# stevenrobertson/cuburn

Measured on AMD Instinct MI355X. Metric: Msamples/s into 1920x1080 histogram + DE-filter GB/s vs HBM roofline, higher is better.
Workload: dtype f32; 1 GPU; BASELINE configs[1]: 1920x1080 still, 3 xforms (linear+spherical+swirl), 2^28 samples/frame, filters yuv+bilateral+logscale+colorclip, rgba8 out; walker_waves=4, walker_slots=1024, temporal_samples=1024, samples_per_frame=268435456, accum=binned, fuse=256, nslots=1024, frames_queued_ahead=2, frames_per_gpu=1121, parallelism=frame-sharded x1, RCCL gather of device frames, 4 frames per collective

## Files before the change

### cuburn_amd/_lib.py

```python
import ctypes as C
import os

_HERE = os.path.dirname(os.path.abspath(__file__))
LIB_PATH = os.path.join(_HERE, '_lib', 'libflame_hip.so')
LIB_PATH = os.environ.get('FLAME_HIP_LIB', LIB_PATH)

(FL_OK, FL_E_INVAL, FL_E_NOMEM, FL_E_HIP, FL_E_NODEV, FL_E_UNSUPPORTED) = (0, -1, -2, -3, -4, -5)

FILT = dict(yuv=0, bilateral=1, logscale=2, colorclip=3, smearclip=4, haloclip=5, plainclip=6, logencode=7, de=8)
BUF = dict(front=0, back=1, params=2, palette=3, points=4, seeds=5, atom=6, hot=7, side=8, log=9, dir=10)
ACCUM_ATOMIC, ACCUM_BINNED = 0, 1
FL_OP_CHAOS_CDF = 11
FL_OP_OPACITY = 10
JPEG_HEADER_BYTES = 629
JPEG_SAMPLING = {'444': 0, '420': 1}
JPEG_OPTIMIZE = 1
PNG_HEADER_BYTES = 33
PNG_ADAPTIVE = 1
PNG_FILTERS = {'paeth': 0, 'adaptive': PNG_ADAPTIVE}
APNG_IDAT = 0xffffffff
EXR_PIXELS = {'half': 1, 'float': 2}
GIF_HEADER_BYTES = 779
GIF_DITHER = {'none': 0, 'ordered': 8}
WEBP_PB, WEBP_EB = 4, 6
OUT = dict(rgba8=0, rgba16=1, yuv444p=2, yuv444p10=3, yuv420p10=4, yuv444p12=5)


class fl_dim(C.Structure):
    _fields_ = [(n, C.c_uint32) for n in ('w', 'h', 'aw', 'ah', 'astride')]


_SIGS = {
    'fl_abi_version': (C.c_int, []),
    'fl_last_error': (C.c_char_p, []),
    'fl_calc_dim': (None, [C.c_uint32, C.c_uint32, C.POINTER(fl_dim)]),
    'fl_ctx_create': (C.c_int, [C.c_int, C.c_void_p, C.c_void_p, C.c_uint32, C.c_uint32, C.POINTER(C.c_void_p)]),
    'fl_ctx_destroy': (None, [C.c_void_p]),
    'fl_ctx_sync': (C.c_int, [C.c_void_p]),
    'fl_genome_create': (C.c_int, [C.c_void_p, C.c_void_p, C.c_uint32, C.c_void_p, C.c_uint32, C.c_uint32,
                                   C.POINTER(C.c_void_p)]),
    'fl_genome_destroy': (None, [C.c_void_p]),
    'fl_genome_upload': (C.c_int, [C.c_void_p, C.c_void_p, C.c_void_p, C.c_void_p, C.c_void_p, C.c_void_p, C.c_uint32]),
    'fl_interp': (C.c_int, [C.c_void_p, C.c_void_p, C.c_uint32, C.c_uint32, C.c_float, C.c_float]),
    'fl_iterate': (C.c_int, [C.c_void_p, C.c_void_p, C.c_uint32, C.c_uint32, C.c_double, C.c_uint32, C.c_int,
                             C.POINTER(C.c_uint64)]),
    'fl_filter': (C.c_int, [C.c_void_p, C.c_int, C.c_uint32, C.c_uint32, C.c_void_p, C.c_uint32]),
    'fl_resample': (C.c_int, [C.c_void_p, C.c_uint32, C.c_uint32, C.c_uint32, C.c_void_p, C.c_uint32]),
    'fl_output': (C.c_int, [C.c_void_p, C.c_uint32, C.c_uint32, C.c_int, C.c_void_p, C.c_uint64]),
    'fl_output_bytes': (C.c_size_t, [C.c_uint32, C.c_uint32, C.c_int]),
    'fl_jpeg_bound': (C.c_size_t, [C.c_uint32, C.c_uint32]),
    'fl_jpeg_encode': (C.c_int, [C.c_void_p, C.c_uint32, C.c_uint32, C.c_uint64, C.c_int, C.c_void_p, C.c_uint64, C.c_size_t]),
    'fl_output_jpeg': (C.c_int, [C.c_void_p, C.c_uint32, C.c_uint32, C.c_int, C.c_void_p, C.c_uint64, C.c_size_t]),
    'fl_jpeg_bound_s': (C.c_size_t, [C.c_uint32, C.c_uint32, C.c_int]),
    'fl_jpeg_encode_s': (C.c_int, [C.c_void_p, C.c_uint32, C.c_uint32, C.c_uint64, C.c_int, C.c_int, C.c_void_p, C.c_uint64, C.c_size_t]),
    'fl_output_jpeg_s': (C.c_int, [C.c_void_p, C.c_uint32, C.c_uint32, C.c_int, C.c_int, C.c_void_p, C.c_uint64, C.c_size_t]),
    'fl_jpeg_bound_f': (C.c_size_t, [C.c_uint32, C.c_uint32, C.c_int, C.c_uint]),
    'fl_jpeg_encode_f': (C.c_int, [C.c_void_p, C.c_uint32, C.c_uint32, C.c_uint64, C.c_int, C.c_int, C.c_uint, C.c_void_p, C.c_uint64, C.c_size_t]),
    'fl_output_jpeg_f': (C.c_int, [C.c_void_p, C.c_uint32, C.c_uint32, C.c_int, C.c_int, C.c_uint, C.c_void_p, C.c_uint64, C.c_size_t]),
    'fl_png_bound': (C.c_size_t, [C.c_uint32, C.c_uint32, C.c_int]),
    'fl_png_encode': (C.c_int, [C.c_void_p, C.c_uint32, C.c_uint32, C.c_uint64, C.c_int, C.c_void_p, C.c_uint64, C.c_size_t]),
    'fl_output_png': (C.c_int, [C.c_void_p, C.c_uint32, C.c_uint32, C.c_int, C.c_void_p, C.c_uint64, C.c_size_t]),
    'fl_png_bound_f': (C.c_size_t, [C.c_uint32, C.c_uint32, C.c_int, C.c_int, C.c_uint]),
    'fl_png_encode_f': (C.c_int, [C.c_void_p, C.c_uint32, C.c_uint32, C.c_uint64, C.c_int, C.c_int, C.c_uint, C.c_void_p, C.c_uint64, C.c_size_t]),
    'fl_output_png_f': (C.c_int, [C.c_void_p, C.c_uint32, C.c_uint32, C.c_int, C.c_int, C.c_uint, C.c_void_p, C.c_uint64, C.c_size_t]),
    'fl_apng_chunks': (C.c_uint32, [C.c_uint32, C.c_uint32, C.c_int, C.c_int]),
    'fl_apng_bound': (C.c_size_t, [C.c_uint32, C.c_uint32, C.c_int, C.c_int, C.c_uint]),
    'fl_apng_encode': (C.c_int, [C.c_void_p, C.c_uint32, C.c_uint32, C.c_uint64, C.c_int, C.c_int, C.c_uint, C.c_uint32, C.c_void_p, C.c_uint64, C.c_size_t]),
    'fl_output_apng': (C.c_int, [C.c_void_p, C.c_uint32, C.c_uint32, C.c_int, C.c_int, C.c_uint, C.c_uint32, C.c_void_p, C.c_uint64, C.c_size_t]),
    'fl_tiff_bound': (C.c_size_t, [C.c_uint32, C.c_uint32, C.c_int, C.c_int]),
    'fl_tiff_encode': (C.c_int, [C.c_void_p, C.c_uint32, C.c_uint32, C.c_uint64, C.c_int, C.c_int, C.c_void_p, C.c_uint64, C.c_size_t]),
    'fl_output_tiff': (C.c_int, [C.c_void_p, C.c_uint32, C.c_uint32, C.c_int, C.c_int, C.c_void_p, C.c_uint64, C.c_size_t]),
    'fl_exr_bound': (C.c_size_t, [C.c_uint32, C.c_uint32, C.c_int, C.c_int]),
    'fl_exr_encode': (C.c_int, [C.c_void_p, C.c_uint32, C.c_uint32, C.c_uint64, C.c_uint32, C.c_int, C.c_int, C.c_void_p, C.c_uint64, C.c_size_t]),
    'fl_output_exr': (C.c_int, [C.c_void_p, C.c_uint32, C.c_uint32, C.c_int, C.c_int, C.c_void_p, C.c_uint64, C.c_size_t]),
    'fl_gif_bound': (C.c_size_t, [C.c_uint32, C.c_uint32]),
    'fl_gif_encode': (C.c_int, [C.c_void_p, C.c_uint32, C.c_uint32, C.c_uint64, C.c_int, C.c_int, C.c_void_p, C.c_uint64, C.c_size_t]),
    'fl_output_gif': (C.c_int, [C.c_void_p, C.c_uint32, C.c_uint32, C.c_int, C.c_int, C.c_void_p, C.c_uint64, C.c_size_t]),
    'fl_webp_bound': (C.c_size_t, [C.c_uint32, C.c_uint32, C.c_int]),
    'fl_webp_encode': (C.c_int, [C.c_void_p, C.c_uint32, C.c_uint32, C.c_uint64, C.c_int, C.c_void_p, C.c_uint64, C.c_size_t]),
    'fl_output_webp': (C.c_int, [C.c_void_p, C.c_uint32, C.c_uint32, C.c_int, C.c_void_p, C.c_uint64, C.c_size_t]),
    'fl_sort_u32': (C.c_int, [C.c_void_p, C.c_uint64, C.c_uint64, C.c_uint32, C.c_uint32, C.c_uint32, C.c_int, C.c_void_p]),
    'fl_frame_begin': (C.c_int, [C.c_void_p, C.POINTER(C.c_uint32)]),
    'fl_frame_ms': (C.c_int, [C.c_void_p, C.c_uint32, C.POINTER(C.c_float)]),
    'fl_frame_query': (C.c_int, [C.c_void_p, C.c_uint32]),
    'fl_host_alloc': (C.c_void_p, [C.c_size_t]),
    'fl_host_free': (None, [C.c_void_p]),
    'fl_timings_reset': (C.c_int, [C.c_void_p]),
    'fl_timings': (C.c_int, [C.c_void_p, C.POINTER(C.c_float), C.POINTER(C.c_float), C.POINTER(C.c_float),
                             C.POINTER(C.c_uint32)]),
    'fl_timings_detail': (C.c_int, [C.c_void_p, C.POINTER(C.c_float * 6)]),
    'fl_launch_stats': (C.c_int, [C.c_void_p, C.POINTER(C.c_uint32 * 4)]),
    'fl_measure_copy': (C.c_int, [C.c_int, C.c_size_t, C.c_int, C.POINTER(C.c_float)]),
    'fl_read_buffer': (C.c_int, [C.c_void_p, C.c_void_p, C.c_int, C.c_void_p, C.c_size_t]),
    'fl_write_buffer': (C.c_int, [C.c_void_p, C.c_void_p, C.c_int, C.c_void_p, C.c_size_t]),
    'fl_buffer_ptr': (C.c_int, [C.c_void_p, C.c_void_p, C.c_int, C.POINTER(C.c_void_p), C.POINTER(C.c_size_t)]),
    'fl_buffer_ptr_async': (C.c_int, [C.c_void_p, C.c_void_p, C.c_int, C.POINTER(C.c_void_p), C.POINTER(C.c_size_t)]),
    'fl_stream_dependency': (C.c_int, [C.c_void_p, C.c_void_p, C.c_int]),
    'fl_reserve': (C.c_int, [C.c_void_p, C.c_uint32, C.c_uint32]),
    'fl_debug_iter_launch': (C.c_int, [C.c_void_p, C.c_void_p, C.c_uint32, C.c_uint32, C.c_uint32, C.c_uint32,
                                       C.c_uint32, C.c_int]),
    'fl_debug_flush': (C.c_int, [C.c_void_p, C.c_uint32, C.c_uint32]),
    'fl_debug_clear': (C.c_int, [C.c_void_p, C.c_uint32, C.c_uint32, C.c_int]),
    'fl_debug_clear_hot': (C.c_int, [C.c_void_p, C.c_uint32, C.c_uint32]),
    'fl_debug_accum': (C.c_int, [C.c_void_p, C.c_uint32, C.c_uint32, C.c_void_p, C.c_size_t, C.c_void_p, C.c_size_t,
                                 C.c_uint32, C.c_uint32, C.c_uint32, C.c_uint32, C.c_int]),
    'fl_debug_accum_check': (C.c_int, [C.c_uint32, C.c_uint32, C.c_void_p, C.c_size_t, C.c_void_p, C.c_size_t,
                                       C.c_uint32, C.c_uint32, C.c_uint32, C.c_uint32, C.c_int]),
    'fl_debug_shuffle': (C.c_int, [C.c_void_p, C.c_uint32, C.c_void_p]),
    'fl_debug_counters': (C.c_int, [C.c_void_p, C.c_void_p]),
    'fl_rtc_compile_check': (C.c_int, [C.c_void_p, C.c_uint32, C.c_void_p, C.c_uint32, C.c_int, C.c_int, C.c_int, C.c_char_p, C.c_size_t]),
    'fl_genome_prepare': (C.c_int, [C.c_void_p, C.c_void_p, C.c_uint32, C.c_uint32, C.c_int]),
    'fl_rtc_wait': (C.c_int, [C.c_void_p, C.c_void_p]),
    'fl_rtc_stats': (C.c_int, [C.POINTER(C.c_uint64 * 8)]),
    'fl_debug_rtc_hold': (C.c_int, [C.c_int]),
    'fl_debug_apply_xf': (C.c_int, [C.c_void_p, C.c_void_p, C.c_uint32, C.c_int, C.c_uint32, C.c_void_p, C.c_void_p]),
    'fl_debug_math': (C.c_int, [C.c_void_p, C.c_int, C.c_uint32, C.c_void_p, C.c_void_p, C.c_void_p]),
    'fl_debug_place': (C.c_int, [C.c_void_p, C.c_void_p, C.c_uint32, C.c_uint64, C.c_void_p, C.c_void_p]),
    'fl_debug_de_dir': (C.c_int, [C.c_void_p, C.c_uint32, C.c_uint32, C.c_int, C.c_void_p, C.c_int, C.c_int]),
}
MATH = dict((n, i) for i, n in enumerate(
    'rcp div sqrt exp2 log2 exp log pow sin cos tan atan2 sinh cosh fmod fmod_pi trunca hw_sin hw_cos'.split()))
EXPORTS = sorted(_SIGS)

_lib = None


class FlameError(RuntimeError):
    pass


def load():
    global _lib
    if _lib is not None:
        return _lib
    if not os.path.isfile(LIB_PATH):
        raise FlameError('%s not found: build it with `python __graft_entry__.py` '
                         '(make -C cuburn_amd/csrc); the HIP library is required' % LIB_PATH)
    try:
        import torch
    except Exception:
        pass
    lib = C.CDLL(LIB_PATH, mode=C.RTLD_GLOBAL)
    for name, (res, args) in _SIGS.items():
        fn = getattr(lib, name)
        fn.restype, fn.argtypes = res, args
    if lib.fl_abi_version() != 1:
        raise FlameError('libflame_hip ABI mismatch')
    _lib = lib
    return lib


def check(rc):
    if rc == FL_OK:
        return
    msg = load().fl_last_error().decode('utf-8', 'replace')
    if rc == FL_E_NOMEM:
        raise MemoryError(msg)
    if rc in (FL_E_INVAL, FL_E_UNSUPPORTED):
        raise ValueError(msg)
    raise FlameError(msg)
```

### cuburn_amd/csrc/binned.hip

```cpp
#include "flame_device.h"
#include "kernels.h"
#include <cstdlib>

__device__ __forceinline__ void spill_cell(u64 cur, uint32_t gi, float *__restrict__ out4)
{
    float yf, uf, vf, df;
    unpack_cell(cur, yf, uf, vf, df);
    float *o = out4 + 4 * (size_t)gi;
    __hip_atomic_fetch_add(o + 0, yf * FL_INV255, __ATOMIC_RELAXED, __HIP_MEMORY_SCOPE_AGENT);
    __hip_atomic_fetch_add(o + 1, uf * FL_INV255, __ATOMIC_RELAXED, __HIP_MEMORY_SCOPE_AGENT);
    __hip_atomic_fetch_add(o + 2, vf * FL_INV255, __ATOMIC_RELAXED, __HIP_MEMORY_SCOPE_AGENT);
    __hip_atomic_fetch_add(o + 3, df, __ATOMIC_RELAXED, __HIP_MEMORY_SCOPE_AGENT);
}

__device__ __forceinline__ void hot_group(u64 v, unsigned long long grp, uint32_t gi, float *__restrict__ out4)
{
#pragma unroll
    for (int sh = 1; sh < 64; sh <<= 1) {
        const uint32_t lo = (uint32_t)__shfl_xor((int)(uint32_t)v, sh), hi = (uint32_t)__shfl_xor((int)(uint32_t)(v >> 32), sh);
        v += ((u64)hi << 32) | lo;
    }
    if ((threadIdx.x & 63u) == (uint32_t)__builtin_ctzll(grp)) spill_cell(v, gi, out4);
}

__device__ __forceinline__ void hot_group_sw(u64 v, unsigned long long grp, uint32_t gi, float *__restrict__ out4)
{
#define HOT_XOR(sh) do { const uint32_t lo = (uint32_t)__builtin_amdgcn_ds_swizzle((int)(uint32_t)v, 0x1f | ((sh) << 10)), \
                                         hi = (uint32_t)__builtin_amdgcn_ds_swizzle((int)(uint32_t)(v >> 32), 0x1f | ((sh) << 10)); \
                         v += ((u64)hi << 32) | lo; } while (0)
    HOT_XOR(1); HOT_XOR(2); HOT_XOR(4); HOT_XOR(8); HOT_XOR(16);
#undef HOT_XOR
    {
        const uint32_t lo = (uint32_t)__shfl_xor((int)(uint32_t)v, 32), hi = (uint32_t)__shfl_xor((int)(uint32_t)(v >> 32), 32);
        v += ((u64)hi << 32) | lo;
    }
    if ((threadIdx.x & 63u) == (uint32_t)__builtin_ctzll(grp)) spill_cell(v, gi, out4);
}

__device__ __forceinline__ uint32_t wave_incl_scan_b(uint32_t v, uint32_t) {
    v += (uint32_t)__builtin_amdgcn_update_dpp(0, (int)v, 0x111, 0xf, 0xf, false);
    v += (uint32_t)__builtin_amdgcn_update_dpp(0, (int)v, 0x112, 0xf, 0xf, false);
    v += (uint32_t)__builtin_amdgcn_update_dpp(0, (int)v, 0x114, 0xf, 0xf, false);
    v += (uint32_t)__builtin_amdgcn_update_dpp(0, (int)v, 0x118, 0xf, 0xf, false);
    v += (uint32_t)__builtin_amdgcn_update_dpp(0, (int)v, 0x142, 0xa, 0xf, false);
    v += (uint32_t)__builtin_amdgcn_update_dpp(0, (int)v, 0x143, 0xc, 0xf, false);
    return v;
}

__device__ __forceinline__ void wave_sync() {
    __builtin_amdgcn_fence(__ATOMIC_RELEASE, "wavefront");
    __builtin_amdgcn_wave_barrier();
    __builtin_amdgcn_fence(__ATOMIC_ACQUIRE, "wavefront");
}

__device__ __forceinline__ uint32_t wave_incl_maxscan(uint32_t v) {
    v = max(v, (uint32_t)__builtin_amdgcn_update_dpp(0, (int)v, 0x111, 0xf, 0xf, false));
    v = max(v, (uint32_t)__builtin_amdgcn_update_dpp(0, (int)v, 0x112, 0xf, 0xf, false));
    v = max(v, (uint32_t)__builtin_amdgcn_update_dpp(0, (int)v, 0x114, 0xf, 0xf, false));
    v = max(v, (uint32_t)__builtin_amdgcn_update_dpp(0, (int)v, 0x118, 0xf, 0xf, false));
    v = max(v, (uint32_t)__builtin_amdgcn_update_dpp(0, (int)v, 0x142, 0xa, 0xf, false));
    v = max(v, (uint32_t)__builtin_amdgcn_update_dpp(0, (int)v, 0x143, 0xc, 0xf, false));
    return v;
}

constexpr int ACC_GATHER_AHEAD = 4;
constexpr int ACC_ADD_ILP = 8;
constexpr int ACC_ROWS_MAX = 5;
constexpr int ACC_THREADS = 1024;

template <uint32_t TWL>
__device__ __forceinline__ void add_tile_to_cells(const u64 *tile, u64 *__restrict__ atom, float *__restrict__ out4,
                                                  uint32_t tx, uint32_t ty, uint32_t astride, uint32_t aheight, uint32_t big_thr)
{
    constexpr uint32_t TW = 1u << TWL, CELLS = TW * FL_TILE_H;
    const uint32_t tid = threadIdx.x;
    for (uint32_t i0 = tid; i0 < CELLS; i0 += blockDim.x * ACC_ADD_ILP) {
        u64 old[ACC_ADD_ILP];
        uint32_t big = 0;
#pragma unroll
        for (uint32_t k = 0; k < ACC_ADD_ILP; ++k) {
            const uint32_t i = i0 + k * blockDim.x;
            old[k] = 0ull;
            if (i < CELLS) {
                const u64 v = tile[i];
                const uint32_t px = tx * TW + (i & (TW - 1u)), py = ty * FL_TILE_H + (i >> TWL);
                if (v != 0ull && px < astride && py < aheight) {
                    if ((uint32_t)(v >> 54) >= big_thr) big |= 1u << k;
                    else
                        asm volatile("global_atomic_add_x2 %0, %1, %2, off sc0" : "+v"(old[k]) : "v"(atom + py * astride + px), "v"(v) : "memory");
                }
            }
        }
        static_assert(ACC_ADD_ILP == 8 || ACC_ADD_ILP == 4, "the wait below names every result");
        if constexpr (ACC_ADD_ILP == 8)
            asm volatile("s_waitcnt vmcnt(0)" : "+v"(old[0]), "+v"(old[1]), "+v"(old[2]), "+v"(old[3]), "+v"(old[4]), "+v"(old[5]), "+v"(old[6]), "+v"(old[7]) :: "memory");
        else
            asm volatile("s_waitcnt vmcnt(0)" : "+v"(old[0]), "+v"(old[1]), "+v"(old[2]), "+v"(old[3]) :: "memory");
#pragma unroll
        for (uint32_t k = 0; k < ACC_ADD_ILP; ++k) {
            const bool full = (uint32_t)(old[k] >> 32) >= (256u << 23);
            if (full || ((big >> k) & 1u)) {
                const uint32_t i = i0 + k * blockDim.x;
                const uint32_t gi = (ty * FL_TILE_H + (i >> TWL)) * astride + tx * TW + (i & (TW - 1u));
                if (full) {
                    const u64 cur = __hip_atomic_exchange(atom + gi, 0ull, __ATOMIC_RELAXED, __HIP_MEMORY_SCOPE_AGENT);
                    if ((uint32_t)(cur >> 32) != 0u) spill_cell(cur, gi, out4);
                } else
                    spill_cell(tile[i], gi, out4);
            }
        }
    }
}

template <uint32_t TWL>
__global__ void __launch_bounds__(TWL == 7u ? ACC_THREADS : 1024, TWL == 7u ? 8 : 4) __attribute__((amdgpu_num_sgpr(80)))
k_accum_tiles(const uint32_t *__restrict__ log, const uint32_t *__restrict__ dir,
              const u64 *__restrict__ palette, u64 *__restrict__ atom, float *__restrict__ out4,
              uint32_t tiles_x, uint32_t nparts, uint32_t nbatch_total, uint32_t batch_records,
              uint32_t nslots, uint32_t astride, uint32_t aheight, uint32_t rows_cap, uint32_t big_thr, uint32_t gang, uint32_t nbins)
{
    extern __shared__ __attribute__((aligned(16))) unsigned char smem[];
    constexpr uint32_t TW = 1u << TWL, CELLS = TW * FL_TILE_H;
    constexpr int ILP = TWL == 7u ? 3 : 4;
    static_assert(FL_PAL_W == 256, "the palette column is the record's low byte, the row the mark's");
    u64 *pal = reinterpret_cast<u64 *>(smem);
    uint32_t *mk = reinterpret_cast<uint32_t *>(smem + rows_cap * FL_PAL_W * 8) + (threadIdx.x >> 6) * 64;
    u64 *tile = reinterpret_cast<u64 *>(smem + rows_cap * FL_PAL_W * 8 + blockDim.x * 4);
    const uint32_t tid = threadIdx.x, lane = tid & 63, wv = tid >> 6, nwaves = blockDim.x >> 6;
    uint32_t bin, part;
    if (gang == 0u) { bin = blockIdx.x / nparts; part = blockIdx.x % nparts; }
    else {
        const uint32_t loc = blockIdx.x >> 3, gq = (loc / gang) * 8u + (blockIdx.x & 7u);
        bin = (gq / nparts) * gang + loc % gang; part = gq % nparts;
        if (bin >= nbins) return;
    }
    const uint32_t tx = bin % tiles_x, ty = bin / tiles_x;

    const uint32_t b_lo = (uint32_t)((u64)nbatch_total * part / nparts);
    const uint32_t b_hi = (uint32_t)((u64)nbatch_total * (part + 1) / nparts);
    const uint32_t *drow = dir + (size_t)bin * nbatch_total;
    const uint32_t per_slot = nbatch_total / nslots;
    const uint32_t spr = nslots / FL_PAL_H;
    const float inv_spr = __int_as_float(__builtin_amdgcn_readfirstlane(__float_as_int(1.0f / (float)spr)));
    const float inv_ps = __int_as_float(__builtin_amdgcn_readfirstlane(__float_as_int(1.0f / (float)per_slot)));
    const uint32_t chunk_slots = (rows_cap - 1u) * spr;

    if (b_lo >= b_hi) return;
    for (uint32_t cb = b_lo; cb < b_hi;) {
    const uint32_t cs_lo = cb / per_slot;
    const uint32_t ce = min(b_hi, (cs_lo + chunk_slots) * per_slot);
    const uint32_t row_lo = cs_lo / spr, nrows = min(rows_cap, (uint32_t)FL_PAL_H - row_lo);
    u64 stagev[3];
#pragma unroll
    for (int q = 0; q < 3; ++q) {
        const uint32_t i = tid + q * blockDim.x;
        stagev[q] = i < nrows * FL_PAL_W ? palette[row_lo * FL_PAL_W + i] : 0ull;
    }
    uint32_t e_next = cb + wv * 64 + lane < ce ? drow[cb + wv * 64 + lane] : 0u;
    if (cb == b_lo) {
        for (uint32_t i = tid; i < CELLS; i += blockDim.x) tile[i] = 0ull;
        mk[lane] = 0u;
    }
    __syncthreads();
#pragma unroll
    for (int q = 0; q < 3; ++q) {
        const uint32_t i = tid + q * blockDim.x;
        if (i < nrows * FL_PAL_W) pal[i] = stagev[q];
    }
    __syncthreads();
    for (uint32_t g0v = cb + wv * 64; g0v < ce; g0v += nwaves * 64) {
        const uint32_t g0 = (uint32_t)__builtin_amdgcn_readfirstlane((int)g0v);
        const uint32_t s0 = g0 / per_slot, rem0 = g0 - s0 * per_slot;
        const uint32_t batch = g0 + lane;
        const uint32_t e = e_next;
        e_next = batch + nwaves * 64 < ce ? drow[batch + nwaves * 64] : 0u;
        const uint32_t c = e & 0xffffu, first = e >> 16;
        const uint32_t incl = wave_incl_scan_b(c, lane);
        const uint32_t excl = incl - c;
        const uint32_t total = __shfl(incl, 63);
        const uint32_t rslot_l = s0 + (uint32_t)(((float)(rem0 + lane) + 0.5f) * inv_ps);
        const uint32_t row_l = (uint32_t)(((float)rslot_l + 0.5f) * inv_spr) - row_lo;
        const uint32_t mark_l = ((lane * batch_records + first - excl + 1u) << 8) | (row_l & 255u);
        const unsigned char *gbase = reinterpret_cast<const unsigned char *>(log + (size_t)g0 * batch_records) - 4;
        uint32_t carry = 0;
        static_assert(ILP >= 2 && ILP <= 4, "up to four rows to a word");
        auto fetch = [&](const uint32_t v0, uint32_t (&rec)[ILP], uint32_t &rows) __attribute__((always_inline)) {
            unsigned char *mk8 = reinterpret_cast<unsigned char *>(mk);
            const bool starts = c != 0u && excl - v0 < 64u * ILP;
            if (starts) mk8[excl - v0] = (unsigned char)(lane + 1u);
            wave_sync();
            uint32_t mm[ILP];
#pragma unroll
            for (int k = 0; k < ILP; ++k) mm[k] = mk8[k * 64 + lane];
            wave_sync();
            if (starts) mk8[excl - v0] = 0;
#pragma unroll
            for (int k = 0; k < ILP; ++k) mm[k] = wave_incl_maxscan(mm[k]);
#pragma unroll
            for (int k = 0; k < ILP; ++k) {
                mm[k] = max(mm[k], carry);
                carry = (uint32_t)__builtin_amdgcn_readlane((int)mm[k], 63);
                mm[k] = (uint32_t)__builtin_amdgcn_ds_bpermute((int)((mm[k] - 1u) << 2), (int)mark_l);
            }
#pragma unroll
            for (int k = 0; k < ILP; ++k) {
                const uint32_t lo = v0 + k * 64, v = lo + lane;
                const uint32_t m = mm[k];
                rows = __builtin_amdgcn_perm(m, rows, k == 0 ? 0x03020104u : k == 1 ? 0x03020400u : k == 2 ? 0x03040100u : 0x04020100u);
                const uint32_t voff = v < total ? ((m >> 8) + v) << 2 : 4u;
                asm volatile("global_load_dword %0, %1, %2" : "=v"(rec[k]) : "v"(voff), "s"(gbase) : "memory");
            }
        };
        auto process = [&](const uint32_t v0, uint32_t (&rec)[ILP], const uint32_t rows) __attribute__((always_inline)) {
            bool live[ILP];
            u64 val[ILP];
            auto gather = [&](const int k) __attribute__((always_inline)) {
                val[k] = pal[__builtin_amdgcn_perm(rows, rec[k], 0x0c0c0000u | ((4u + k) << 8))];
            };
#pragma unroll
            for (int k = 0; k < ILP; ++k) {
                live[k] = v0 + k * 64 + lane < total;
                if (k < ACC_GATHER_AHEAD) gather(k);
            }
            {
                const uint32_t o0 = rec[0] >> 8;
                if (__builtin_expect(__popcll(__ballot(live[0] && o0 == (uint32_t)__builtin_amdgcn_readfirstlane((int)o0))) >= 48, 0)) {
#pragma unroll
                    for (int k = ACC_GATHER_AHEAD; k < ILP; ++k) gather(k);
#pragma unroll
                    for (int k = 0; k < ILP; ++k) {
                        const uint32_t off = rec[k] >> 8;
                        const uint32_t off0 = (uint32_t)__builtin_amdgcn_readfirstlane((int)off);
                        const bool mine = live[k] && off == off0;
                        const unsigned long long grp = __ballot(mine);
                        if (__popcll(grp) >= 16) {
                            hot_group(mine ? val[k] : 0ull, grp, (ty * FL_TILE_H + (off0 >> TWL)) * astride + tx * TW + (off0 & (TW - 1u)), out4);
                            live[k] = live[k] && !mine;
                        }
                    }
                }
            }
#pragma unroll
            for (int k = 0; k < ILP; ++k) {
                const uint32_t off = rec[k] >> 8;
                if (k + ACC_GATHER_AHEAD < ILP) gather(k + ACC_GATHER_AHEAD);
                if (!live[k]) continue;
                const u64 old = __hip_atomic_fetch_add(tile + off, val[k], __ATOMIC_RELAXED, __HIP_MEMORY_SCOPE_WORKGROUP);
                if ((uint32_t)(old >> 32) >= (128u << 23)) {
                    const u64 cur = __hip_atomic_exchange(tile + off, 0ull, __ATOMIC_RELAXED, __HIP_MEMORY_SCOPE_WORKGROUP);
                    if ((uint32_t)(cur >> 32) != 0u) {
                        const uint32_t px = tx * TW + (off & (TW - 1u)), py = ty * FL_TILE_H + (off >> TWL);
                        spill_cell(cur, py * astride + px, out4);
                    }
                }
            }
        };
#define ACC_WAIT(n, r) do { if constexpr (ILP == 4) asm volatile("s_waitcnt vmcnt(" #n ")" : "+v"(r[0]), "+v"(r[1]), "+v"(r[ILP - 2]), "+v"(r[ILP - 1]) :: "memory"); \
                            else if constexpr (ILP == 3) asm volatile("s_waitcnt vmcnt(" #n ")" : "+v"(r[0]), "+v"(r[1]), "+v"(r[ILP - 1]) :: "memory"); \
                            else asm volatile("s_waitcnt vmcnt(" #n ")" : "+v"(r[0]), "+v"(r[1]) :: "memory"); } while (0)
#define ACC_WAIT_NEWER(r) do { if constexpr (ILP == 4) ACC_WAIT(4, r); else if constexpr (ILP == 3) ACC_WAIT(3, r); else ACC_WAIT(2, r); } while (0)
        constexpr uint32_t STEP = 64 * ILP;
        uint32_t recA[ILP] = {}, recB[ILP] = {}, rowsA = 0u, rowsB = 0u;
        for (uint32_t v0 = 0; v0 < total; v0 += 2 * STEP) {
            fetch(v0, recA, rowsA);
            if (v0 != 0u) { asm volatile("; acc-guarded-block"); ACC_WAIT_NEWER(recB); process(v0 - STEP, recB, rowsB); }
            if (v0 + STEP < total) { fetch(v0 + STEP, recB, rowsB); ACC_WAIT_NEWER(recA); } else ACC_WAIT(0, recA);
            process(v0, recA, rowsA);
        }
        if (((total + STEP - 1u) / STEP & 1u) == 0u && total != 0u) {
            ACC_WAIT(0, recB);
            process((total - 1u) / STEP * STEP, recB, rowsB);
        }
#undef ACC_WAIT
#undef ACC_WAIT_NEWER
    }
    cb = ce;
    }
    __syncthreads();

    for (uint32_t i0 = tid; i0 < CELLS; i0 += blockDim.x * ACC_ADD_ILP) {
        u64 old[ACC_ADD_ILP];
        uint32_t big = 0;
#pragma unroll
        for (uint32_t k = 0; k < ACC_ADD_ILP; ++k) {
            const uint32_t i = i0 + k * blockDim.x;
            old[k] = 0ull;
            if (i < CELLS) {
                const u64 v = tile[i];
                const uint32_t px = tx * TW + (i & (TW - 1u)), py = ty * FL_TILE_H + (i >> TWL);
                if (v != 0ull && px < astride && py < aheight) {
                    if ((uint32_t)(v >> 54) >= big_thr) big |= 1u << k;
                    else
                        asm volatile("global_atomic_add_x2 %0, %1, %2, off sc0" : "+v"(old[k]) : "v"(atom + py * astride + px), "v"(v) : "memory");
                }
            }
        }
        static_assert(ACC_ADD_ILP == 8 || ACC_ADD_ILP == 4, "the wait below names every result");
        if constexpr (ACC_ADD_ILP == 8)
            asm volatile("s_waitcnt vmcnt(0)" : "+v"(old[0]), "+v"(old[1]), "+v"(old[2]), "+v"(old[3]), "+v"(old[4]), "+v"(old[5]), "+v"(old[6]), "+v"(old[7]) :: "memory");
        else
            asm volatile("s_waitcnt vmcnt(0)" : "+v"(old[0]), "+v"(old[1]), "+v"(old[2]), "+v"(old[3]) :: "memory");
#pragma unroll
        for (uint32_t k = 0; k < ACC_ADD_ILP; ++k) {
            const bool full = (uint32_t)(old[k] >> 32) >= (256u << 23);
            if (full || ((big >> k) & 1u)) {
                const uint32_t i = i0 + k * blockDim.x;
                const uint32_t gi = (ty * FL_TILE_H + (i >> TWL)) * astride + tx * TW + (i & (TW - 1u));
                if (full) {
                    const u64 cur = __hip_atomic_exchange(atom + gi, 0ull, __ATOMIC_RELAXED, __HIP_MEMORY_SCOPE_AGENT);
                    if ((uint32_t)(cur >> 32) != 0u) spill_cell(cur, gi, out4);
                } else
                    spill_cell(tile[i], gi, out4);
            }
        }
    }
}

typedef uint32_t u32x2_t __attribute__((ext_vector_type(2)));
typedef __attribute__((address_space(3))) u64 lds_u64_t;
typedef __attribute__((address_space(3))) unsigned char lds_u8_t;
__device__ __forceinline__ lds_u64_t *lds64(uint32_t byte) { return (lds_u64_t *)(uintptr_t)byte; }
__device__ __forceinline__ lds_u8_t *lds8(uint32_t byte) { return (lds_u8_t *)(uintptr_t)byte; }
constexpr uint32_t P3_MARKS = 64u, P3_PAL = 2048u, P3_TILE = P3_PAL + ACC_ROWS_MAX * FL_PAL_W * 8u, P3_LDS = P3_TILE + FL_TILE_CELLS * 8u;
static_assert(P3_MARKS + (ACC_THREADS / 64) * 64 <= P3_PAL && P3_PAL == FL_PAL_W * 8u && ACC_ROWS_MAX < 15, "marks below the rows; row + 1 is a nibble");
__global__ void __launch_bounds__(ACC_THREADS, 8) __attribute__((amdgpu_num_sgpr(80)))
k_accum_tiles_p3(const uint32_t *__restrict__ log, const uint32_t *__restrict__ dir,
                 const u64 *__restrict__ palette, u64 *__restrict__ atom, float *__restrict__ out4,
                 uint32_t tiles_x, uint32_t nparts, uint32_t nbatch_total, uint32_t batch_words,
                 uint32_t nslots, uint32_t astride, uint32_t aheight, uint32_t rows_cap, uint32_t big_thr, uint32_t gang, uint32_t nbins)
{
    extern __shared__ __attribute__((aligned(16))) unsigned char smem[];
    constexpr uint32_t TWL = 7u, TW = 1u << TWL, CELLS = TW * FL_TILE_H;
    static_assert(FL_PAL_W == 256 && FL_REC_BITS == 21, "8-bit palette column, 13-bit cell offset");
    if ((uint32_t)(uintptr_t)(lds_u8_t *)smem != 0u) __builtin_trap();
    const uint32_t tid = threadIdx.x, lane = tid & 63, wv = tid >> 6, nwaves = blockDim.x >> 6;
    uint32_t bin, part;
    if (gang == 0u) { bin = blockIdx.x / nparts; part = blockIdx.x % nparts; }
    else {
        const uint32_t loc = blockIdx.x >> 3, gq = (loc / gang) * 8u + (blockIdx.x & 7u);
        bin = (gq / nparts) * gang + loc % gang; part = gq % nparts;
        if (bin >= nbins) return;
    }
    const uint32_t tx = bin % tiles_x, ty = bin / tiles_x;
    const uint32_t b_lo = (uint32_t)((u64)nbatch_total * part / nparts);
    const uint32_t b_hi = (uint32_t)((u64)nbatch_total * (part + 1) / nparts);
    const uint32_t *drow = dir + (size_t)bin * nbatch_total;
    const uint32_t per_slot = nbatch_total / nslots;
    const uint32_t spr = nslots / FL_PAL_H;
    const float inv_spr = __int_as_float(__builtin_amdgcn_readfirstlane(__float_as_int(1.0f / (float)spr)));
    const float inv_ps = __int_as_float(__builtin_amdgcn_readfirstlane(__float_as_int(1.0f / (float)per_slot)));
    const uint32_t chunk_slots = (rows_cap - 1u) * spr;
    if (b_lo >= b_hi) return;
    const uint32_t mk8 = P3_MARKS + wv * 64u;
    const uint32_t lane8 = (lane + 1u) << 3;
    u32x2_t wA = {}, wB = {}, wC = {};
    uint32_t mA = 0u, mB = 0u, mC = 0u;

    for (uint32_t cb = b_lo; cb < b_hi;) {
    const uint32_t cs_lo = cb / per_slot;
    const uint32_t ce = min(b_hi, (cs_lo + chunk_slots) * per_slot);
    const uint32_t row_lo = cs_lo / spr, nrows = min(rows_cap, (uint32_t)FL_PAL_H - row_lo);
    u64 stagev[3];
    uint32_t tid_c = tid;
    asm volatile("" : "+v"(tid_c));
#pragma unroll
    for (int q = 0; q < 3; ++q) {
        const uint32_t i = tid_c + q * blockDim.x;
        stagev[q] = i < nrows * FL_PAL_W ? palette[row_lo * FL_PAL_W + i] : 0ull;
    }
    uint32_t e_next = cb + wv * 64 + lane < ce ? drow[cb + wv * 64 + lane] : 0u;
    if (cb == b_lo) {
        for (uint32_t i = tid; i < CELLS; i += blockDim.x) *lds64(P3_TILE + i * 8u) = 0ull;
        *lds8(mk8 + lane) = 0;
        if (tid < 2u) *lds64(tid * 8u) = 0ull;
    }
    __syncthreads();
#pragma unroll
    for (int q = 0; q < 3; ++q) {
        const uint32_t i = tid_c + q * blockDim.x;
        if (i < nrows * FL_PAL_W) *lds64(P3_PAL + i * 8u) = stagev[q];
    }
    __syncthreads();
    for (uint32_t g0v = cb + wv * 64; g0v < ce; g0v += nwaves * 64) {
        const uint32_t g0 = (uint32_t)__builtin_amdgcn_readfirstlane((int)g0v);
        const uint32_t s0 = g0 / per_slot, rem0 = g0 - s0 * per_slot;
        const uint32_t batch = g0 + lane;
        const uint32_t e = e_next;
        e_next = batch + nwaves * 64 < ce ? drow[batch + nwaves * 64] : 0u;
        const uint32_t cnt = e & 0xffffu, rfirst = e >> 16, rlast = rfirst + cnt - 1u;
        const uint32_t fw = __umul24(rfirst, 43691u) >> 17, lw = __umul24(rlast, 43691u) >> 17;
        const uint32_t c = cnt ? lw - fw + 1u : 0u;
        const uint32_t lo_mask = (7u << (rfirst - 3u * fw)) & 7u, hi_mask = 7u >> (2u - (rlast - 3u * lw));
        const uint32_t incl = wave_incl_scan_b(c, lane);
        const uint32_t excl = incl - c;
        const uint32_t total = (uint32_t)__builtin_amdgcn_readlane((int)incl, 63);
        const uint32_t rslot_l = s0 + (uint32_t)(((float)(rem0 + lane) + 0.5f) * inv_ps);
        const uint32_t row_l = (uint32_t)(((float)rslot_l + 0.5f) * inv_spr) - row_lo;
        const uint32_t w1_l = lane * batch_words + fw - excl + 1u;
        const uint32_t w2_l = ((incl - 1u) << 10) | ((row_l + 1u) << 6) | (hi_mask << 3) | lo_mask;
        const unsigned char *gbase = reinterpret_cast<const unsigned char *>(log) + (size_t)g0 * batch_words * 8u - 8u;
        uint32_t carry = 0;
        auto fetch = [&](const uint32_t v0, u32x2_t &w, uint32_t &meta) __attribute__((always_inline)) {
            uint32_t voff = 8u;
            meta = 0u;
            if (v0 < total) {
                const bool starts = cnt != 0u && excl - v0 < 64u;
                if (starts) *lds8(mk8 + excl - v0) = (unsigned char)(lane + 1u);
                wave_sync();
                const uint32_t raw = *lds8(mk8 + lane);
                wave_sync();
                if (starts) *lds8(mk8 + excl - v0) = 0;
                uint32_t mm = max(wave_incl_maxscan(raw), carry);
                carry = (uint32_t)__builtin_amdgcn_readlane((int)mm, 63);
                const int src = (int)(mm << 2) - 4;
                const uint32_t m1 = (uint32_t)__builtin_amdgcn_ds_bpermute(src, (int)w1_l);
                const uint32_t m2 = (uint32_t)__builtin_amdgcn_ds_bpermute(src, (int)w2_l);
                const uint32_t v = v0 + lane;
                const bool inside = v < total;
                const uint32_t lm = raw != 0u ? m2 : 7u, hm = (m2 >> 10) == v ? __builtin_amdgcn_ubfe(m2, 3, 3) : 7u;
                meta = (m2 & 0x3c0u) | (inside ? lm & hm : 0u);
                voff = inside ? (m1 + v) << 3 : lane8;
            }
            asm volatile("global_load_dwordx2 %0, %1, %2" : "=v"(w) : "v"(voff), "s"(gbase) : "memory");
        };
        auto process = [&](const u32x2_t w, const uint32_t meta) __attribute__((always_inline)) {
            const uint32_t wl = w.x, wh = w.y;
            const uint32_t rowbase = (meta & 0x3c0u) << 5;
            const uint32_t col8[3] = {(wl << 3) & 0x7f8u, (wl >> 18) & 0x7f8u, (wh >> 7) & 0x7f8u};
            const uint32_t cell8[3] = {(wl >> 5) & 0xfff8u, __builtin_amdgcn_alignbit(wh, wl, 26) & 0xfff8u, (wh >> 15) & 0xfff8u};
            u64 val[3];
#pragma unroll
            for (int j = 0; j < 3; ++j) {
                const uint32_t live = (uint32_t)__builtin_amdgcn_sbfe((int)meta, j, 1);
                val[j] = *lds64((col8[j] | rowbase) & live);
            }
            if (__builtin_expect((uint32_t)__popcll(__ballot(cell8[0] == (uint32_t)__builtin_amdgcn_readfirstlane((int)cell8[0]))) >= 48u, 0)) {
#pragma unroll
                for (int j = 0; j < 3; ++j) {
                    const bool live = (meta >> j & 1u) != 0u;
                    const unsigned long long lv = __ballot(live);
                    if (lv == 0ull) continue;
                    const uint32_t off0 = (uint32_t)__builtin_amdgcn_readlane((int)cell8[j], (int)__builtin_ctzll(lv)) >> 3;
                    const bool mine = live && cell8[j] >> 3 == off0;
                    const unsigned long long grp = __ballot(mine);
                    if (__popcll(grp) >= 16) {
                        hot_group_sw(mine ? val[j] : 0ull, grp, (ty * FL_TILE_H + (off0 >> TWL)) * astride + tx * TW + (off0 & (TW - 1u)), out4);
                        if (mine) val[j] = 0ull;
                    }
                }
            }
#pragma unroll
            for (int j = 0; j < 3; ++j) {
                lds_u64_t *cp = lds64(P3_TILE + cell8[j]);
                const u64 old = __hip_atomic_fetch_add(cp, val[j], __ATOMIC_RELAXED, __HIP_MEMORY_SCOPE_WORKGROUP);
                if (__builtin_expect(__ballot((uint32_t)(old >> 32) >= (128u << 23)) != 0ull, 0)) {
                    if ((uint32_t)(old >> 32) >= (128u << 23)) {
                        const u64 cur = __hip_atomic_exchange(cp, 0ull, __ATOMIC_RELAXED, __HIP_MEMORY_SCOPE_WORKGROUP);
                        if ((uint32_t)(cur >> 32) != 0u) {
                            const uint32_t off = cell8[j] >> 3, px = tx * TW + (off & (TW - 1u)), py = ty * FL_TILE_H + (off >> TWL);
                            spill_cell(cur, py * astride + px, out4);
                        }
                    }
                }
            }
        };
        const uint32_t nsteps = (total + 63u) >> 6;
#define P3_WAIT(w) asm volatile("s_waitcnt vmcnt(2)" : "+v"(w) :: "memory")
        for (uint32_t s = 0; s < nsteps + 2u; s += 3u) {
            fetch(s << 6, wA, mA);
            P3_WAIT(wB); if (s >= 2u && s - 2u < nsteps) process(wB, mB);
            fetch((s + 1u) << 6, wB, mB);
            P3_WAIT(wC); if (s >= 1u && s - 1u < nsteps) process(wC, mC);
            fetch((s + 2u) << 6, wC, mC);
            P3_WAIT(wA); if (s < nsteps) process(wA, mA);
        }
        asm volatile("s_waitcnt vmcnt(0)" : "+v"(wA), "+v"(wB), "+v"(wC) :: "memory");
#undef P3_WAIT
    }
    cb = ce;
    }
    __syncthreads();
    add_tile_to_cells<TWL>(reinterpret_cast<const u64 *>(smem + P3_TILE), atom, out4, tx, ty, astride, aheight, big_thr);
}

void launch_accum_tiles(hipStream_t st, const uint32_t *log, const uint32_t *dir, const u64 *palette,
                        u64 *atom, float *out4, uint32_t tiles_x, uint32_t nbins, uint32_t nparts,
                        uint32_t nbatch_total, uint32_t batch_records, uint32_t nslots,
                        uint32_t astride, uint32_t aheight, bool wide)
{
    const uint32_t big_thr = 1024u / nparts;
    const uint32_t spr = nslots / FL_PAL_H, slots_per_part = (nslots + nparts - 1) / nparts;
    if (batch_records > 65536u) abort();
    const uint32_t want = (slots_per_part + spr - 1) / spr + 1;
    static const int gang_env = getenv("FLAME_BIN_GANG") ? atoi(getenv("FLAME_BIN_GANG")) : -1;
    const uint32_t gang = gang_env >= 0 ? (uint32_t)gang_env : (nbins > 512u ? 32u : 0u);
    const uint32_t ngangs = gang ? ((nbins + gang - 1) / gang) * nparts : 0u;
    const uint32_t grid = gang ? ((ngangs + 7u) / 8u) * 8u * gang : nbins * nparts;
    if (wide) {
        const uint32_t rows = want < 2u ? 2u : want > 12u ? 12u : want;
        static unsigned long long attr = 0;
        ensure_max_dynamic_lds((const void *)k_accum_tiles<FL_TILE_W_WIDE_LOG2>, attr);
        hipLaunchKernelGGL((k_accum_tiles<FL_TILE_W_WIDE_LOG2>), dim3(grid), dim3(1024),
                           (FL_TILE_H << FL_TILE_W_WIDE_LOG2) * 8 + 1024 * 4 + rows * FL_PAL_W * 8, st,
                           log, dir, palette, atom, out4, tiles_x, nparts, nbatch_total, batch_records, nslots, astride, aheight, rows, big_thr, gang, nbins);
        return;
    }
    const uint32_t rows = want < 2u ? 2u : want > (uint32_t)ACC_ROWS_MAX ? (uint32_t)ACC_ROWS_MAX : want;
    static unsigned long long attr = 0;
#if FL_LOG_PACK3
    {
        static unsigned long long attr3 = 0;
        ensure_max_dynamic_lds((const void *)k_accum_tiles_p3, attr3);
        hipLaunchKernelGGL(k_accum_tiles_p3, dim3(grid), dim3(ACC_THREADS), P3_LDS, st,
                           log, dir, palette, atom, out4, tiles_x, nparts, nbatch_total, fl_pack3_words(batch_records), nslots, astride, aheight, rows, big_thr, gang, nbins);
        return;
    }
#endif
    ensure_max_dynamic_lds((const void *)k_accum_tiles<7u>, attr);
    hipLaunchKernelGGL((k_accum_tiles<7u>), dim3(grid), dim3(ACC_THREADS), FL_TILE_CELLS * 8 + ACC_THREADS * 4 + rows * FL_PAL_W * 8, st,
                       log, dir, palette, atom, out4, tiles_x, nparts, nbatch_total, batch_records, nslots, astride, aheight, rows, big_thr, gang, nbins);
}
```

### cuburn_amd/csrc/flame_abi.hip

```cpp
#include <hip/hip_runtime.h>
#include <cstdio>
#include <cstdlib>
#include <cstring>
#include <cmath>
#include <string>
#include <atomic>
#include <vector>
#include <algorithm>
#include <array>
#include "kernels.h"
#include "flame_device.h"
#include "launch_plan.h"

static thread_local std::string g_err;
static int fail(int code, const char *what, const char *file, int line, hipError_t e = hipSuccess)
{
    char buf[512];
    if (e != hipSuccess) snprintf(buf, sizeof buf, "%s: %s (%s:%d)", what, hipGetErrorString(e), file, line);
    else snprintf(buf, sizeof buf, "%s (%s:%d)", what, file, line);
    g_err = buf;
    return code;
}
static int fail_hip(hipError_t e, const char *what, const char *file, int line)
{
    return fail(e == hipErrorOutOfMemory ? FL_E_NOMEM : FL_E_HIP, what, file, line, e);
}
#define HIPCHK(x) do { hipError_t e_ = (x); if (e_ != hipSuccess) return fail_hip(e_, #x, __FILE__, __LINE__); } while (0)
#define REQUIRE(c, msg) do { if (!(c)) return fail(FL_E_INVAL, msg, __FILE__, __LINE__); } while (0)

template <class T> struct DevBuf {
    T *p = nullptr;
    size_t cap = 0;
    DevBuf() = default;
    DevBuf(const DevBuf &) = delete;
    DevBuf &operator=(const DevBuf &) = delete;
    ~DevBuf() { release(); }
    operator T *() const { return p; }
    size_t bytes() const { return cap * sizeof(T); }
    void release() { if (p) hipFree(p); p = nullptr; cap = 0; }
    template <class Quiesce> int reserve(size_t n, const char *what, Quiesce quiesce)
    {
        if (n <= cap) return FL_OK;
        if (int rc = quiesce()) return rc;
        release();
        const hipError_t e = hipMalloc(&p, n * sizeof(T));
        if (e != hipSuccess) { p = nullptr; (void)hipGetLastError(); return fail_hip(e, what, __FILE__, __LINE__); }
        cap = n;
        return FL_OK;
    }
    int reserve(size_t n, const char *what) { return reserve(n, what, [] { return (int)FL_OK; }); }
    friend void swap(DevBuf &a, DevBuf &b) { std::swap(a.p, b.p); std::swap(a.cap, b.cap); }
};

struct EvPair { hipEvent_t a, b; };

struct Bilateral { float sstd, cstd, dstd, dpow, gspeed, k7[7]; };

struct Pending {
    bool yuv = false, de = false;
    int in_mode = 0;
    Bilateral bl = {};
    DeTail tail = {};
    fl_dim dim = {0, 0, 0, 0, 0};
    void clear() { yuv = de = false; }
    void defer_yuv(const fl_dim &d) { yuv = true; dim = d; }
    void defer_bilateral(const fl_dim &d, const Bilateral &b) { in_mode = yuv ? 2 : 1; yuv = false; de = true; bl = b; tail = {}; dim = d; }
    bool try_take(int id, const float *p)
    {
        if (!de || yuv || (id == FL_FILT_LOGSCALE && tail.do_log)) return false;
        if (id == FL_FILT_LOGSCALE) { tail.do_log = 1; tail.k1 = p[0]; tail.k2 = p[1]; }
        else { tail.do_clip = 1; tail.vib = p[0]; tail.highpow = p[1]; tail.gam = p[2]; tail.lin = p[3]; tail.lingam = p[4]; }
        return true;
    }
};

struct Lane {
    hipStream_t stream = nullptr;
    DevBuf<float4> d_front, d_back, d_side;
    DevBuf<float> d_blur;
    DevBuf<u64> d_atom;
    DevBuf<uint32_t> d_hot;
    DevBuf<unsigned char> d_outpix;
    DevBuf<uint32_t> d_de_tmax;
    DevBuf<float> d_de_sinv;
    DevBuf<uint32_t> d_enc;
    DevBuf<unsigned char> d_enc_out;
    size_t nbins() const { return d_front.cap; }
    DevBuf<uint32_t> d_log[2], d_dir[2];
    hipStream_t aux = nullptr;
    hipEvent_t ev_it[2] = {nullptr, nullptr}, ev_ac[2] = {nullptr, nullptr};
    DevBuf<float> d_params;
    uint64_t params_serial = 0;
    DevBuf<u64> d_palette;
    hipEvent_t ev_interp_done = nullptr;
    hipEvent_t ev_iter_done = nullptr;
    hipEvent_t ev_out_done = nullptr;
    bool interp_rec = false, iter_rec = false, out_rec = false;
    Pending pend;

    std::array<hipEvent_t *, 7> events() { return {&ev_interp_done, &ev_iter_done, &ev_out_done, &ev_it[0], &ev_ac[0], &ev_it[1], &ev_ac[1]}; }
    int quiesce(bool with_aux)
    {
        HIPCHK(hipStreamSynchronize(stream));
        if (with_aux) HIPCHK(hipStreamSynchronize(aux));
        return FL_OK;
    }
    void release_fb()
    {
        d_front.release(); d_back.release(); d_side.release(); d_blur.release(); d_atom.release();
        d_hot.release(); d_outpix.release(); d_de_tmax.release(); d_de_sinv.release();
        pend.clear();
    }
    void release()
    {
        release_fb();
        d_params.release(); d_palette.release(); d_enc.release(); d_enc_out.release();
        for (int k = 0; k < 2; ++k) { d_log[k].release(); d_dir[k].release(); }
        if (aux) hipStreamDestroy(aux);
        for (hipEvent_t *ev : events()) if (*ev) hipEventDestroy(*ev);
    }
};

#define FL_NOUT 65536u

struct fl_ctx {
    int device = 0;
    bool own_stream = false;
    static const int kMaxLanes = 4;
    int nlanes = 2, cur = 0;
    Lane lanes[kMaxLanes];
    Lane &lane() { return lanes[cur]; }
    Lane &prev_lane() { return lanes[(cur + nlanes - 1) % nlanes]; }
    uint32_t nslots = 0;
    uint32_t sub_log2 = 0;
    uint32_t ntemporal() const { return nslots << sub_log2; }
    int nw = 4;
    uint32_t npoints() const { return nslots * (uint32_t)nw * 64u; }
    DevBuf<fl_mwc> d_rng;
    fl_mwc *rng_walk() const { return d_rng.p; }
    fl_mwc *rng_pal() const { return d_rng.p + npoints(); }
    fl_mwc *rng_out() const { return rng_pal() + FL_PAL_H * 256; }
    DevBuf<float4> d_points;
    DevBuf<u64> d_counters;
    DevBuf<uint32_t> d_sort;
    uint32_t bin_rounds = 16, bin_parts = 0;
    uint32_t launch_rounds = 0;
    uint32_t round_counter = 0;
    static const uint32_t kFrames = 8;
    hipEvent_t ev_begin_[kFrames] = {}, ev_end_[kFrames] = {};
    uint32_t frame_lane[kFrames] = {};
    uint32_t frame_seq = 0;
    std::vector<EvPair> pool, iter_ev, accum_ev, flush_ev, filt_ev, de_ev, enc_ev;
    size_t pool_used = 0;
    bool timing = true;
    static const uint32_t kDepEvents = 16;
    hipEvent_t dep_ev[kDepEvents] = {};
    uint32_t dep_next = 0;
    bool env_bin_wide = false, env_no_intra = false;
    bool use_rtc = true;
    bool rtc_async = false;
    uint32_t jpeg_ri = FL_JPEG_RI;
    uint32_t jpeg_ri_420 = FL_JPEG_RI_420;
    uint32_t gif_seg = FL_GIF_SEG;
    uint32_t n_spec_launch = 0, n_interp_launch = 0;
    BinLayout layout(const fl_dim &d) const { return bin_layout(d, nw, bin_rounds, env_bin_wide); }
};

struct fl_genome {
    uint64_t serial = 0;
    std::vector<int32_t> prog;
    IterSpec spec;
    hipFunction_t rtc_fn[5][2][4] = {};
    unsigned rtc_epoch = 0;
    bool rtc_failed = false;
    bool rtc_want[5][2][4] = {};
    uint32_t nops = 0, nrows = 0, pstride = 0;
    int32_t *d_prog = nullptr, *d_ops = nullptr;
    float *d_times = nullptr, *d_knots = nullptr, *d_ptimes = nullptr;
    float4 *d_pals = nullptr;
    uint32_t npal = 0;
    static const int kStage = 4;
    unsigned char *h_stage[kStage] = {};
    hipEvent_t ev_stage[kStage] = {};
    size_t stage_bytes = 0;
    int stage_next = 0;
};

static const int kKnownVars[] = {0,1,2,3,4,5,6,7,8,9,10,11,12,13,14,15,16,17,18,19,20,21,22,23,24,25,26,27,28,29,30,31,32,33,
    34,35,36,37,38,39,40,41,42,43,44,45,46,48,49,50,51,52,53,54,55,56,57,58,59,60,61,62,63,64,65,66,67,68,69,70,71,72,73,
    74,75,76,77,80,81,82,83,84,85,86,87,88,89,90,91,92,93,94,95,97,98};

static const size_t kMaxTimed = 8192;

static EvPair *ev_acquire(fl_ctx *c, std::vector<EvPair> &list)
{
    if (!c->timing || c->pool_used >= kMaxTimed) return nullptr;
    if (c->pool.capacity() < kMaxTimed) c->pool.reserve(kMaxTimed);
    if (c->pool_used == c->pool.size()) {
        EvPair p;
        if (hipEventCreate(&p.a) != hipSuccess || hipEventCreate(&p.b) != hipSuccess) return nullptr;
        c->pool.push_back(p);
    }
    list.push_back(c->pool[c->pool_used++]);
    return &c->pool[c->pool_used - 1];
}
static EvPair *ev_begin_on(fl_ctx *c, std::vector<EvPair> &list, hipStream_t st)
{
    EvPair *p = ev_acquire(c, list);
    if (p) hipEventRecord(p->a, st);
    return p;
}
static void ev_end_on(EvPair *p, hipStream_t st) { if (p) hipEventRecord(p->b, st); }
static EvPair *ev_begin(fl_ctx *c, std::vector<EvPair> &list) { return ev_begin_on(c, list, c->lane().stream); }
static void ev_end(fl_ctx *c, EvPair *p) { ev_end_on(p, c->lane().stream); }

#pragma GCC visibility push(default)
extern "C" {

int fl_abi_version(void) { return FL_ABI_VERSION; }
const char *fl_last_error(void) { return g_err.c_str(); }

void fl_calc_dim(uint32_t w, uint32_t h, fl_dim *o) { *o = calc_dim(w, h); }

static const float *de_norms()
{
    static const std::vector<float> t = [] { std::vector<float> v(16 * FL_DE_MAX_RADIUS + 1); de_adaptive_norms(v.data()); return v; }();
    return t.data();
}

static int ensure_fb(Lane &ln, uint32_t w, uint32_t h, fl_dim *dim)
{
    const fl_dim d = *dim = calc_dim(w, h);
    const size_t nbins = (size_t)d.ah * d.astride, ob = (size_t)d.w * d.h * 8, nsinv = 16 * FL_DE_MAX_RADIUS + 1;
    if (ln.nbins() >= nbins && ln.d_outpix.cap >= ob) return FL_OK;
    hipStreamSynchronize(ln.stream);
    ln.release_fb();
    const char *what = "framebuffer allocation";
    int rc;
    if (!(rc = ln.d_front.reserve(nbins, what)) && !(rc = ln.d_back.reserve(nbins, what)) && !(rc = ln.d_side.reserve(nbins, what)) &&
        !(rc = ln.d_blur.reserve(nbins, what)) && !(rc = ln.d_atom.reserve(nbins, what)) && !(rc = ln.d_hot.reserve(nbins / 16, what)) &&
        !(rc = ln.d_outpix.reserve(ob, what)) && !(rc = ln.d_de_tmax.reserve(nbins / 256 + 64, what)) && !(rc = ln.d_de_sinv.reserve(nsinv, what))) {
        const hipError_t e = hipMemcpyAsync(ln.d_de_sinv, de_norms(), 4 * nsinv, hipMemcpyHostToDevice, ln.stream);
        if (e != hipSuccess) { (void)hipGetLastError(); rc = fail_hip(e, what, __FILE__, __LINE__); }
    }
    if (rc) ln.release_fb();
    return rc;
}

static bool env_on(const char *name) { const char *e = getenv(name); return e && *e && strcmp(e, "0") != 0; }

int fl_ctx_create(int device, void *stream, const fl_mwc *seeds, uint32_t nseeds, uint32_t nslots, fl_ctx **out)
{
    REQUIRE(out && seeds, "null argument");
    REQUIRE(nslots_valid(nslots),
            "nslots must be a multiple of 256 in [1024, 16384] (or 512 slots of 8 waves / 256 of 16: two / four temporal samples per workgroup)");
    int ndev = 0;
    if (hipGetDeviceCount(&ndev) != hipSuccess || ndev <= 0) return fail(FL_E_NODEV, "no HIP device", __FILE__, __LINE__);
    REQUIRE(device >= 0 && device < ndev, "bad device index");
    HIPCHK(hipSetDevice(device));
    hipDeviceProp_t prop;
    HIPCHK(hipGetDeviceProperties(&prop, device));
    if (strncmp(prop.gcnArchName, "gfx950", 6) != 0)
        return fail(FL_E_NODEV, "device is not gfx950 (kernels are built for MI355X only)", __FILE__, __LINE__);
    int nw = 0;
    {
        const uint32_t fixed = FL_PAL_H * 256 + FL_NOUT;
        const uint32_t per_wave = nslots * 64u;
        if (nseeds == fixed + 16u * per_wave) nw = 16;
        else if (nseeds == fixed + 8u * per_wave) nw = 8;
        else if (nseeds == fixed + 4u * per_wave) nw = 4;
        else return fail(FL_E_INVAL, "nseeds must be nslots*64*NW + 64*256 + 65536 with NW = 4, 8 or 16", __FILE__, __LINE__);
    }
    if (nslots < FL_NTEMPORAL && (uint32_t)nw * nslots != 4u * FL_NTEMPORAL)
        return fail(FL_E_INVAL, "512 slots need 8-wave workgroups, 256 slots 16-wave ones (a temporal sample per four waves: 1024 in all)", __FILE__, __LINE__);
    fl_ctx *c = new fl_ctx;
    c->device = device;
    c->nw = nw;
    c->nslots = nslots;
    c->sub_log2 = nslots >= FL_NTEMPORAL ? 0u : nw == 8 ? 1u : 2u;
    if (const char *e = getenv("FLAME_LANES")) { const int v = atoi(e); c->nlanes = v >= 1 && v <= fl_ctx::kMaxLanes ? v : 2; }
    if (const char *e = getenv("FLAME_BIN_ROUNDS")) { int v = atoi(e); if (v >= 1 && v <= FL_BIN_R_MAX) c->bin_rounds = (uint32_t)v; }
    if (const char *e = getenv("FLAME_BIN_PARTS")) { int v = atoi(e); if (v >= 1 && v <= 64) c->bin_parts = (uint32_t)v; }
    c->env_bin_wide = env_on("FLAME_BIN_WIDE");
    if (const char *e = getenv("FLAME_RTC")) c->use_rtc = strcmp(e, "0") != 0;
    c->rtc_async = env_on("FLAME_RTC_ASYNC");
    c->gif_seg = gif_segment_pixels();
    if (const char *e = getenv("FLAME_JPEG_RI")) { const int v = atoi(e); if (v >= 1 && v <= 21) { c->jpeg_ri = (uint32_t)v; c->jpeg_ri_420 = std::min((uint32_t)v, FL_JPEG_RI_420_MAX); } }
    c->env_no_intra = env_on("FLAME_NO_INTRA_OVERLAP");
    if (const char *e = getenv("FLAME_LAUNCH_ROUNDS")) { int v = atoi(e); if (v >= 16 && v <= 4096) c->launch_rounds = (uint32_t)(v / 16 * 16); }
    if (stream) { c->lanes[0].stream = (hipStream_t)stream; c->own_stream = false; c->nlanes = 1; }
    else c->own_stream = true;
    const size_t nrng = (size_t)c->npoints() + FL_PAL_H * 256 + FL_NOUT;
    const char *what = "context allocation";
    const auto hip = [what](hipError_t e) { return e == hipSuccess ? (int)FL_OK : fail_hip(e, what, __FILE__, __LINE__); };
    int rc = FL_OK;
    for (int i = 0; i < c->nlanes && c->own_stream && !rc; ++i) rc = hip(hipStreamCreateWithFlags(&c->lanes[i].stream, hipStreamNonBlocking));
    if (!rc && !(rc = c->d_rng.reserve(nrng, what)) && !(rc = c->d_points.reserve(c->npoints(), what))) rc = c->d_counters.reserve(4, what);
    for (int i = 0; i < c->nlanes && !rc; ++i) {
        Lane &ln = c->lanes[i];
        if ((rc = ln.d_palette.reserve(FL_PAL_H * FL_PAL_W, what)) || (rc = hip(hipStreamCreateWithFlags(&ln.aux, hipStreamNonBlocking)))) break;
        for (hipEvent_t *ev : ln.events()) if ((rc = hip(hipEventCreateWithFlags(ev, hipEventDisableTiming)))) break;
    }
    if (!rc && !(rc = hip(hipMemcpy(c->d_rng, seeds, c->d_rng.bytes(), hipMemcpyHostToDevice))) &&
        !(rc = hip(hipMemsetD32(c->d_points, 0x7fc00000, (size_t)c->npoints() * 4)))) rc = hip(hipMemset(c->d_counters, 0, 32));
    for (uint32_t i = 0; i < fl_ctx::kFrames && !rc; ++i)
        if (!(rc = hip(hipEventCreate(&c->ev_begin_[i])))) rc = hip(hipEventCreate(&c->ev_end_[i]));
    if (rc) {
        fl_ctx_destroy(c);
        (void)hipGetLastError();
        return rc;
    }
    *out = c;
    return FL_OK;
}

static void sync_all(fl_ctx *c)
{
    for (int i = 0; i < c->nlanes; ++i) { hipStreamSynchronize(c->lanes[i].stream); if (c->lanes[i].aux) hipStreamSynchronize(c->lanes[i].aux); }
}

void fl_ctx_destroy(fl_ctx *c)
{
    if (!c) return;
    hipSetDevice(c->device);
    for (uint32_t i = 0; i < fl_ctx::kDepEvents; ++i) if (c->dep_ev[i]) hipEventDestroy(c->dep_ev[i]);
    for (Lane &ln : c->lanes) {
        if (ln.stream) hipStreamSynchronize(ln.stream);
        if (ln.aux) hipStreamSynchronize(ln.aux);
    }
    for (Lane &ln : c->lanes) {
        ln.release();
        if (c->own_stream && ln.stream) hipStreamDestroy(ln.stream);
    }
    for (auto &p : c->pool) { hipEventDestroy(p.a); hipEventDestroy(p.b); }
    for (uint32_t i = 0; i < fl_ctx::kFrames; ++i) {
        if (c->ev_begin_[i]) hipEventDestroy(c->ev_begin_[i]);
        if (c->ev_end_[i]) hipEventDestroy(c->ev_end_[i]);
    }
    delete c;
    (void)hipGetLastError();
}

int fl_ctx_sync(fl_ctx *c) { REQUIRE(c, "null ctx"); sync_all(c); return FL_OK; }

static int wait_other(fl_ctx *c, int what)
{
    if (c->nlanes < 2) return FL_OK;
    Lane &ln = c->lane(), &o = c->prev_lane();
    if (what == 0 && o.interp_rec) HIPCHK(hipStreamWaitEvent(ln.stream, o.ev_interp_done, 0));
    if (what == 1 && o.iter_rec) HIPCHK(hipStreamWaitEvent(ln.stream, o.ev_iter_done, 0));
    if (what == 2 && o.out_rec) HIPCHK(hipStreamWaitEvent(ln.stream, o.ev_out_done, 0));
    return FL_OK;
}

static int check_prog(const int32_t *p, uint32_t n)
{
    REQUIRE(n >= FL_PROG_HDR && p[0] == FL_PROG_MAGIC, "bad program header");
    int nxf = p[1], hf = p[2], ps = p[3], cdf = p[4], xo = p[5], xs = p[6], vs = p[7];
    REQUIRE(nxf >= 1 && nxf <= FL_MAX_XFORMS && (hf == 0 || hf == 1), "bad xform count");
    REQUIRE(ps >= 6 + nxf && ps <= FL_MAX_PSTRIDE, "bad pstride");
    REQUIRE(cdf >= 6 && cdf + nxf <= xo, "bad cdf offset");
    REQUIRE(xs >= FL_XF_HDR + vs && (xs % 4) == 0 && vs >= 2 && vs <= 64, "bad record strides");
    REQUIRE(xo + (nxf + hf) * xs <= ps, "xform records exceed the block");
    if (n > FL_PROG_HDR) {
        const int co = p[FL_PROG_HDR];
        REQUIRE(nxf <= FL_CHAOS_MAX_XFORMS, "too many xforms for a genome with chaos");
        REQUIRE(co >= xo + (nxf + hf) * xs && co <= ps && nxf * nxf <= ps - co, "bad chaos offset");
    }
    return FL_OK;
}

static int check_structure_op(const int32_t *prog, const int32_t *o)
{
    const int xs = prog[6], nxf = prog[1], nrec = nxf + prog[2], rel = o[1] - prog[5];
    if (o[0] == FL_OP_OPACITY) REQUIRE(rel >= 0 && rel / xs < nxf && rel % xs == 15, "opacity op must write word 15 of a selectable xform record");
    if (o[0] != FL_OP_CONST) return FL_OK;
    REQUIRE(rel >= 0 && rel / xs < nrec, "structure word outside the xform records");
    if (rel % xs == 14) {
        REQUIRE((o[2] >> 10) == 0, "bad structure word");
        REQUIRE(((o[2] >> 9) & 1) == 0 || rel / xs < nxf, "the final xform has no opacity");
    }
    return FL_OK;
}

static IterSpec iter_spec(const int32_t *prog, uint32_t nprog, const int32_t *ops, uint32_t nops)
{
    const int xo = prog[5], xs = prog[6], vs = prog[7], nrec = prog[1] + prog[2];
    const bool has_chaos = nprog > FL_PROG_HDR;
    IterSpec spec;
    spec.nxf = prog[1]; spec.has_final = prog[2]; spec.pstride = prog[3]; spec.cdf_off = prog[4];
    spec.xf_off = xo; spec.xf_stride = xs; spec.var_stride = vs;
    spec.chaos = has_chaos ? 1 : 0; spec.chaos_off = has_chaos ? prog[FL_PROG_HDR] : 0;
    spec.nvar.assign(nrec, 0); spec.post.assign(nrec, 0); spec.opac.assign(nrec, 0); spec.vids.assign(nrec, std::vector<int>());
    for (int pass = 0; pass < 2; ++pass)
        for (uint32_t i = 0; i < nops; ++i) {
            const int32_t *o = ops + 4 * i;
            if (o[0] != FL_OP_CONST) continue;
            const int rel = o[1] - xo, rec = rel / xs, w = rel % xs;
            if (pass == 0 && w == 14) {
                spec.nvar[rec] = o[2] & 0xff; spec.post[rec] = (o[2] >> 8) & 1; spec.opac[rec] = (o[2] >> 9) & 1;
                spec.vids[rec].assign(spec.nvar[rec], -1);
            } else if (pass == 1 && w != 14) {
                const int j = (w - FL_XF_HDR) / vs;
                if (j >= 0 && j < spec.nvar[rec]) spec.vids[rec][j] = o[2];
            }
        }
    return spec;
}

static bool known_var(int id)
{
    for (int k : kKnownVars) if (k == id) return true;
    return false;
}

int fl_genome_create(fl_ctx *c, const int32_t *prog, uint32_t nprog, const int32_t *ops, uint32_t nops,
                     uint32_t nrows, fl_genome **out)
{
    REQUIRE(c && prog && ops && out, "null argument");
    int rc = check_prog(prog, nprog);
    if (rc) return rc;
    REQUIRE(nrows >= 1 && nrows <= 4096 && nops >= 1, "bad row / op count");
    uint32_t ps = prog[3];
    const int xo = prog[5], xs = prog[6], vs = prog[7], nrec = prog[1] + prog[2];
    std::vector<int> nvar_seen(nrec, -1), opac_seen(nrec, 0), opac_ops(nrec, 0);
    const bool has_chaos = nprog > FL_PROG_HDR;
    std::vector<int> chaos_ops(has_chaos ? prog[1] : 0, 0);
    for (uint32_t i = 0; i < nops; ++i) {
        const int32_t *o = ops + 4 * i;
        REQUIRE(o[0] >= FL_OP_SPLINE && o[0] <= FL_OP_CHAOS_CDF, "bad op kind");
        REQUIRE(o[1] >= 0 && (uint32_t)o[1] < ps, "op destination out of range");
        if ((rc = check_structure_op(prog, o))) return rc;
        const int rel = o[1] - xo;
        if (o[0] != FL_OP_CONST) {
            uint32_t ndst = 1, nsrc = 1;
            switch (o[0]) {
            case FL_OP_CAMERA: ndst = 6; nsrc = 4; break;
            case FL_OP_AFFINE: ndst = 6; nsrc = 6; break;
            case FL_OP_CDF:
                REQUIRE(o[3] >= 1 && o[3] <= FL_MAX_XFORMS, "bad CDF length");
                ndst = nsrc = (uint32_t)o[3];
                break;
            case FL_OP_PERSP: ndst = 3; break;
            case FL_OP_CHAOS_CDF: {
                REQUIRE(has_chaos, "chaos op in a program without a chaos matrix");
                const int nx = prog[1], crel = o[1] - prog[FL_PROG_HDR];
                REQUIRE(o[3] >= 0 && (o[3] & 0xff) == nx, "bad chaos row length");
                REQUIRE(crel >= 0 && crel < nx * nx && crel % nx == 0, "chaos op must write a row of the chaos matrix");
                REQUIRE((uint32_t)(o[3] >> 8) + (uint32_t)nx <= nrows, "op row out of range");
                ++chaos_ops[crel / nx];
                ndst = nsrc = (uint32_t)nx;
            } break;
            default: break;
            }
            REQUIRE((uint32_t)o[1] + ndst <= ps, "op destination out of range");
            REQUIRE(o[2] >= 0 && (uint32_t)o[2] + nsrc <= nrows, "op row out of range");
            if (o[0] == FL_OP_RATIO2 || o[0] == FL_OP_PERSP) REQUIRE(o[3] >= 0 && (uint32_t)o[3] < nrows, "op row out of range");
            if (o[0] == FL_OP_OPACITY) ++opac_ops[rel / xs];
            continue;
        }
        const int w = rel % xs;
        if (w == 14) {
            const int nv = o[2] & 0xff;
            REQUIRE(FL_XF_HDR + nv * vs <= xs, "bad variation count");
            nvar_seen[rel / xs] = nv;
            opac_seen[rel / xs] = (o[2] >> 9) & 1;
        } else {
            REQUIRE(w >= FL_XF_HDR && (w - FL_XF_HDR) % vs == 0, "misplaced structure word");
            if (!known_var(o[2])) return fail(FL_E_UNSUPPORTED, "unknown variation id", __FILE__, __LINE__);
        }
    }
    for (int i = 0; i < nrec; ++i) REQUIRE(nvar_seen[i] >= 0, "xform record without a variation count");
    for (int i = 0; i < nrec; ++i) REQUIRE(opac_ops[i] == opac_seen[i], "opacity flag and opacity op do not match");
    for (int n : chaos_ops) REQUIRE(n == 1, "every row of the chaos matrix needs exactly one chaos op");
    const IterSpec spec = iter_spec(prog, nprog, ops, nops);
    for (int i = 0; i < nrec; ++i)
        for (int j = 0; j < spec.nvar[i]; ++j) REQUIRE(spec.vids[i][j] >= 0, "variation record without a variation number");
    HIPCHK(hipSetDevice(c->device));
    fl_genome *g = new fl_genome;
    { static std::atomic<uint64_t> next_serial{1}; g->serial = next_serial.fetch_add(1); }
    g->spec = spec;
    g->prog.assign(prog, prog + nprog);
    g->nops = nops; g->nrows = nrows; g->pstride = ps;
    g->stage_bytes = 2 * 4 * (size_t)nrows * FL_KNOTS + 16 * 256 * (FL_KNOTS - 1) + 4 * FL_KNOTS;
    hipError_t e = hipSuccess;
    do {
        if ((e = hipMalloc(&g->d_prog, 4 * nprog))) break;
        if ((e = hipMalloc(&g->d_ops, 16 * nops))) break;
        const size_t table = 4 * (size_t)nrows * FL_KNOTS;
        const std::vector<float> pad_times(FL_KNOTS, 1e9f);
        if ((e = hipMalloc(&g->d_times, table + 4 * FL_KNOTS))) break;
        if ((e = hipMalloc(&g->d_knots, table + 4 * FL_KNOTS))) break;
        if ((e = hipMemcpy((char *)g->d_times + table, pad_times.data(), 4 * FL_KNOTS, hipMemcpyHostToDevice))) break;
        if ((e = hipMemset((char *)g->d_knots + table, 0, 4 * FL_KNOTS))) break;
        if ((e = hipMalloc(&g->d_ptimes, 4 * FL_KNOTS))) break;
        if ((e = hipMalloc(&g->d_pals, 16 * 256 * FL_KNOTS))) break;
        if ((e = hipMemcpy(g->d_prog, prog, 4 * nprog, hipMemcpyHostToDevice))) break;
        if ((e = hipMemcpy(g->d_ops, ops, 16 * nops, hipMemcpyHostToDevice))) break;
        if ((e = hipMemset(g->d_pals, 0, 16 * 256 * FL_KNOTS))) break;
        for (int i = 0; i < fl_genome::kStage && e == hipSuccess; ++i) {
            if ((e = hipHostMalloc((void **)&g->h_stage[i], g->stage_bytes, hipHostMallocDefault))) break;
            e = hipEventCreateWithFlags(&g->ev_stage[i], hipEventDisableTiming);
        }
    } while (0);
    if (e != hipSuccess) {
        fl_genome_destroy(g);
        (void)hipGetLastError();
        return fail_hip(e, "genome allocation", __FILE__, __LINE__);
    }
    *out = g;
    return FL_OK;
}

void fl_genome_destroy(fl_genome *g)
{
    if (!g) return;
    hipFree(g->d_prog); hipFree(g->d_ops); hipFree(g->d_times); hipFree(g->d_knots);
    hipFree(g->d_ptimes); hipFree(g->d_pals);
    for (int i = 0; i < fl_genome::kStage; ++i) { if (g->h_stage[i]) hipHostFree(g->h_stage[i]); if (g->ev_stage[i]) hipEventDestroy(g->ev_stage[i]); }
    delete g;
}

int fl_genome_upload(fl_ctx *c, fl_genome *g, const float *times, const float *knots,
                     const float *pal_rgba, const float *pal_times, uint32_t npal)
{
    REQUIRE(c && g && times && knots && pal_rgba && pal_times, "null argument");
    REQUIRE(npal >= 1 && npal < FL_KNOTS, "bad palette count");
    HIPCHK(hipSetDevice(c->device));
    const size_t nb = 4 * (size_t)g->nrows * FL_KNOTS, pb = 16 * 256 * (size_t)npal, tb = 4 * FL_KNOTS;
    const int slot = g->stage_next;
    g->stage_next = (slot + 1) % fl_genome::kStage;
    HIPCHK(hipEventSynchronize(g->ev_stage[slot]));
    unsigned char *h = g->h_stage[slot];
    memcpy(h, times, nb);
    memcpy(h + nb, knots, nb);
    memcpy(h + 2 * nb, pal_rgba, pb);
    memcpy(h + 2 * nb + pb, pal_times, tb);
    { int rc = wait_other(c, 0); if (rc) return rc; }
    hipStream_t st = c->lane().stream;
    HIPCHK(hipMemcpyAsync(g->d_times, h, nb, hipMemcpyHostToDevice, st));
    HIPCHK(hipMemcpyAsync(g->d_knots, h + nb, nb, hipMemcpyHostToDevice, st));
    HIPCHK(hipMemcpyAsync(g->d_pals, h + 2 * nb, pb, hipMemcpyHostToDevice, st));
    HIPCHK(hipMemcpyAsync(g->d_ptimes, h + 2 * nb + pb, tb, hipMemcpyHostToDevice, st));
    HIPCHK(hipEventRecord(g->ev_stage[slot], st));
    g->npal = npal;
    return FL_OK;
}

int fl_frame_begin(fl_ctx *c, uint32_t *frame_id)
{
    REQUIRE(c && frame_id, "null argument");
    HIPCHK(hipSetDevice(c->device));
    const uint32_t id = c->frame_seq++;
    const uint32_t k = id % fl_ctx::kFrames;
    c->cur = (int)(id % (uint32_t)c->nlanes);
    c->frame_lane[k] = (uint32_t)c->cur;
    HIPCHK(hipEventRecord(c->ev_begin_[k], c->lane().stream));
    HIPCHK(hipEventRecord(c->ev_end_[k], c->lane().stream));
    *frame_id = id;
    return FL_OK;
}

int fl_interp(fl_ctx *c, fl_genome *g, uint32_t w, uint32_t h, float ts, float td)
{
    REQUIRE(c && g && g->npal, "genome not uploaded");
    HIPCHK(hipSetDevice(c->device));
    Lane &ln = c->lane();
    const fl_dim d = calc_dim(w, h);
    const size_t need = (size_t)c->ntemporal() * g->pstride;
    if (need > ln.d_params.cap) ln.params_serial = 0;
    int rc = ln.d_params.reserve(need, "parameter blocks", [&ln] { return ln.quiesce(false); });
    if (rc) return rc;
    if ((rc = wait_other(c, 0))) return rc;
    launch_interp_palette(ln.stream, c->rng_pal(), g->d_ptimes, g->d_pals, ts, td / FL_PAL_H, ln.d_palette);
    launch_interp_params(ln.stream, ln.d_params, g->d_times, g->d_knots, g->d_ops, g->nops, g->pstride,
                         c->ntemporal(), ts, td / (float)c->ntemporal(), d, ln.params_serial != g->serial);
    ln.params_serial = g->serial;
    HIPCHK(hipGetLastError());
    HIPCHK(hipEventRecord(ln.ev_interp_done, ln.stream));
    ln.interp_rec = true;
    return FL_OK;
}

static int do_clear(fl_ctx *c, Lane &ln, const fl_dim &d, bool reset_points)
{
    size_t nbins = (size_t)d.ah * d.astride;
    launch_clear_frame(ln.stream, ln.d_front, ln.d_atom, ln.d_hot, c->d_counters, c->d_points, (uint32_t)nbins,
                       reset_points ? c->npoints() : 0u);
    HIPCHK(hipGetLastError());
    return FL_OK;
}

static int ensure_binned(fl_ctx *c, Lane &ln, const fl_dim &d, uint32_t write_rounds, int buf, BinLayout *layout, uint32_t *nbatch_total)
{
    const BinLayout b = *layout = c->layout(d);
    if (b.nbins > FL_MAX_BINS_WIDE) return fail(FL_E_UNSUPPORTED, "image too large for the binned accumulate (> 8191 tiles of 256x64)", __FILE__, __LINE__);
    const BinSet s = bin_set(b, write_rounds, c->bin_rounds, c->nslots);
    *nbatch_total = s.nbatch;
    const auto quiesce = [&ln] { return ln.quiesce(true); };
    if (int rc = ln.d_log[buf].reserve(s.log_words, "sample log", quiesce)) return rc;
    return ln.d_dir[buf].reserve(s.dir_words, "sample log directory", quiesce);
}

static hipFunction_t rtc_variant(fl_ctx *c, fl_genome *g, bool count, int kacc, int mode, bool *pending)
{
    *pending = false;
    if (!c->use_rtc || g->rtc_failed || kacc == 2) return nullptr;
    const unsigned ep = rtc_epoch();
    if (g->rtc_epoch != ep) { memset(g->rtc_fn, 0, sizeof g->rtc_fn); g->rtc_epoch = ep; }
    const int geom = c->sub_log2 ? 2 + (int)c->sub_log2 : c->nw == 16 ? 2 : c->nw == 8 ? 1 : 0;
    hipFunction_t &slot = g->rtc_fn[geom][count ? 1 : 0][kacc];
    if (!slot) {
        std::string err;
        const int rc = rtc_iter_kernel(c->device, g->spec, c->nw, c->nslots, count, kacc, &slot, &err, c->sub_log2, mode);
        if (rc < 0) {
            g->rtc_failed = true;
            slot = nullptr;
            fprintf(stderr, "libflame_hip: per-genome kernel not available (%s); using the interpreter kernel\n", err.c_str());
        } else if (rc > 0) {
            slot = nullptr;
            *pending = true;
        }
        g->rtc_want[geom][count ? 1 : 0][kacc] = rc > 0;
    }
    return slot;
}

static int do_iter_launch(fl_ctx *c, Lane &ln, fl_genome *g, const fl_dim &d, uint32_t nrounds, uint32_t fuse, bool count, int acc = 0,
                          int buf = 0, hipStream_t drain = nullptr)
{
    if (!drain) drain = ln.stream;
    BinLayout bl = {};
    uint32_t nbatch_total = 0;
    if (acc == FL_ACCUM_BINNED) {
        if (nrounds <= fuse) return fail(FL_E_INVAL, "binned launch needs write-enabled rounds", __FILE__, __LINE__);
        int rc = ensure_binned(c, ln, d, nrounds - fuse, buf, &bl, &nbatch_total);
        if (rc) return rc;
    }
    EvPair *e = ev_acquire(c, c->iter_ev);
    const int kacc = acc == FL_ACCUM_BINNED && bl.wide ? 3 : acc;
    bool pending = false;
    const hipFunction_t fn = rtc_variant(c, g, count, kacc, c->rtc_async ? RTC_POLL : RTC_SYNC, &pending);
    (fn ? c->n_spec_launch : c->n_interp_launch) += 1;
    rtc_count_launch(fn != nullptr, pending);
    const IterLaunch il = {c->nw, count, kacc, c->nslots, g->d_prog, ln.d_params, ln.d_palette, c->rng_walk(), c->d_points,
                           ln.d_hot, ln.d_atom, (float *)ln.d_front.p, c->d_counters, d.astride, d.ah, c->round_counter, nrounds, fuse,
                           bl.tiles_x, bl.nbins, c->bin_rounds, nbatch_total, ln.d_log[buf], ln.d_dir[buf],
                           e ? e->a : nullptr, e ? e->b : nullptr, c->sub_log2, g->spec.chaos != 0};
    launch_iter(ln.stream, il, fn);
    c->round_counter += nrounds;
    HIPCHK(hipGetLastError());
    if (acc == FL_ACCUM_BINNED) {
        if (drain != ln.stream) {
            HIPCHK(hipEventRecord(ln.ev_it[buf], ln.stream));
            HIPCHK(hipStreamWaitEvent(drain, ln.ev_it[buf], 0));
        }
        EvPair *e2 = ev_begin_on(c, c->accum_ev, drain);
        launch_accum_tiles(drain, ln.d_log[buf], ln.d_dir[buf], ln.d_palette, ln.d_atom, (float *)ln.d_front.p, bl.tiles_x, bl.nbins,
                           accum_parts(bl.nbins, bl.wide, c->bin_parts), nbatch_total, c->bin_rounds * (uint32_t)c->nw * 64, c->nslots,
                           d.astride, d.ah, bl.wide);
        ev_end_on(e2, drain);
        HIPCHK(hipGetLastError());
    }
    return FL_OK;
}

static int do_flush(fl_ctx *c, Lane &ln, const fl_dim &d, bool use_hot = true, hipStream_t st = nullptr)
{
    if (!st) st = ln.stream;
    EvPair *e = ev_begin_on(c, c->flush_ev, st);
    launch_flush(st, ln.d_atom, ln.d_front, ln.d_hot, d.ah * d.astride, use_hot);
    ev_end_on(e, st);
    HIPCHK(hipGetLastError());
    return FL_OK;
}

static int flush_pending(fl_ctx *c, Lane &ln)
{
    Pending &pd = ln.pend;
    if (!pd.yuv && !pd.de) return FL_OK;
    if (pd.yuv) {
        launch_yuv_to_rgb(ln.stream, pd.dim, ln.d_back, ln.d_front);
        swap(ln.d_front, ln.d_back);
    }
    if (pd.de) {
        const Bilateral &b = pd.bl;
        const auto dir = [&](int pat, float4 *dst, const float4 *src, const DeTail *tail) {
            launch_de_dir(ln.stream, pd.dim, pat, dst, src, b.k7, b.sstd, b.cstd, b.dstd, b.dpow, b.gspeed, pd.in_mode, tail);
        };
        EvPair *e = ev_begin_on(c, c->de_ev, ln.stream);
        float4 *Na = ln.d_back, *Nb = ln.d_front;
        dir(0, Na, Nb, nullptr);
        for (int pat = 1; pat < 7; ++pat) { dir(pat, Nb, Na, nullptr); std::swap(Na, Nb); }
        dir(7, ln.d_front, Na, &pd.tail);
        ev_end_on(e, ln.stream);
    }
    pd.clear();
    HIPCHK(hipGetLastError());
    return FL_OK;
}

int fl_iterate(fl_ctx *c, fl_genome *g, uint32_t w, uint32_t h, double nsamples, uint32_t fuse,
               int accum_mode, uint64_t *nsamples_run)
{
    REQUIRE(c && g, "null argument");
    REQUIRE(accum_mode == FL_ACCUM_ATOMIC || accum_mode == FL_ACCUM_BINNED || accum_mode == 2, "bad accumulation mode");
    Lane &ln = c->lane();
    REQUIRE(ln.d_params.cap >= (size_t)c->ntemporal() * g->pstride, "fl_interp has not run for this genome");
    HIPCHK(hipSetDevice(c->device));
    fl_dim d;
    int rc = ensure_fb(ln, w, h, &d);
    if (rc) return rc;
    if ((rc = flush_pending(c, ln))) return rc;
    if ((rc = wait_other(c, 1))) return rc;
    if ((rc = do_clear(c, ln, d, true))) return rc;
    const double per_round = (double)c->npoints();
    uint64_t rounds = (uint64_t)ceil(nsamples / per_round);
    if (rounds == 0) rounds = 1;
    if (nsamples_run) *nsamples_run = (uint64_t)(rounds * per_round);
    const bool binned = accum_mode == FL_ACCUM_BINNED;
    LaunchPlan plan = binned ? launch_schedule(rounds, c->sub_log2, c->nw, c->launch_rounds) : launch_schedule_under(rounds, c->sub_log2, FL_NO_CAP);
    if (binned && !c->launch_rounds && plan.cap > launch_cap(false, c->sub_log2, c->nw)) {
        const size_t need = bin_set(c->layout(d), std::min(rounds, plan.cap), c->bin_rounds, c->nslots).bytes();
        size_t grow = 0, mfree = 0, mtotal = 0;
        for (int b = 0; b < 2; ++b) {
            const size_t have = ln.d_log[b].bytes() + ln.d_dir[b].bytes();
            if (need > have) grow += need - have;
        }
        if (grow && (hipMemGetInfo(&mfree, &mtotal) != hipSuccess || grow + (size_t(1) << 30) > mfree))
            plan = launch_schedule_under(rounds, c->sub_log2, launch_cap(false, c->sub_log2, c->nw));
    }
    const bool pipelined = binned && plan.rounds.size() > 1 && !c->env_no_intra;
    hipStream_t drain = pipelined ? ln.aux : ln.stream;
    uint32_t k = 0;
    for (const uint32_t n : plan.rounds) {
        const uint32_t f = k == 0 ? fuse : 0;
        const int buf = pipelined ? (int)(k & 1u) : 0;
        if (pipelined && k >= 2) HIPCHK(hipStreamWaitEvent(ln.stream, ln.ev_ac[buf], 0));
        if ((rc = do_iter_launch(c, ln, g, d, n + f, f, false, accum_mode, buf, drain))) return rc;
        if ((rc = do_flush(c, ln, d, !binned, drain))) return rc;
        if (pipelined) HIPCHK(hipEventRecord(ln.ev_ac[buf], drain));
        ++k;
    }
    HIPCHK(hipEventRecord(ln.ev_iter_done, ln.stream));
    ln.iter_rec = true;
    if (pipelined) {
        HIPCHK(hipStreamWaitEvent(ln.stream, ln.ev_ac[(k - 1) & 1u], 0));
        if (k >= 2) HIPCHK(hipStreamWaitEvent(ln.stream, ln.ev_ac[k & 1u], 0));
    }
    return FL_OK;
}

static void gauss7(float stdev, float *c)
{
    float s = 0.0f;
    for (int i = 0; i < 7; ++i) { float x = (float)(i - 3); c[i] = expf(x * x / (-2.0f * stdev * stdev)); s += c[i]; }
    for (int i = 0; i < 7; ++i) c[i] /= s;
}

static int check_filter(int id, const float *p, uint32_t np)
{
    static const struct { uint32_t np; const char *msg; } need[] = {
        {0, ""}, {5, "bilateral needs sstd,cstd,dstd,dpow,gspeed"}, {2, "logscale needs k1,k2"},
        {5, "colorclip needs vib,highpow,gam,lin,lingam"}, {4, "smearclip needs width,gam_m_1,lin,lingam"}, {1, "haloclip needs gam_m_1"},
        {4, "plainclip needs gam_m_1,lin,lingam,brightness"}, {1, "logencode needs degamma"}, {3, "de needs R,Rmin,curve"}};
    if (id < FL_FILT_YUV || id > FL_FILT_DE) return fail(FL_E_UNSUPPORTED, "unknown filter id", __FILE__, __LINE__);
    REQUIRE(np >= need[id].np, need[id].msg);
    REQUIRE(p || !need[id].np, "null filter scalars");
    if (id == FL_FILT_DE) {
        REQUIRE(!(p[0] > (float)FL_DE_MAX_RADIUS), "de: R above 96 px");
        REQUIRE(p[2] > 0.0f, "de: curve must be > 0");
    }
    return FL_OK;
}

int fl_filter(fl_ctx *c, int id, uint32_t w, uint32_t h, const float *p, uint32_t np)
{
    REQUIRE(c, "null ctx");
    int rc = check_filter(id, p, np);
    if (rc) return rc;
    HIPCHK(hipSetDevice(c->device));
    Lane &ln = c->lane();
    fl_dim d;
    if ((rc = ensure_fb(ln, w, h, &d))) return rc;
    hipStream_t st = ln.stream;
    float k7[7];
    EvPair *e = ev_begin(c, c->filt_ev);
    bool took = false;
    switch (id) {
    case FL_FILT_BILATERAL: if (ln.pend.de) rc = flush_pending(c, ln); break;
    case FL_FILT_LOGSCALE: if (!(took = ln.pend.try_take(id, p))) rc = flush_pending(c, ln); break;
    case FL_FILT_COLORCLIP: took = ln.pend.try_take(id, p); rc = flush_pending(c, ln); break;
    default: rc = flush_pending(c, ln); break;
    }
    if (!rc && !took) switch (id) {
    case FL_FILT_YUV: ln.pend.defer_yuv(d); break;
    case FL_FILT_BILATERAL: {
        Bilateral b = {p[0], p[1], p[2], p[3], p[4], {}};
        gauss7(1.0f, b.k7);
        ln.pend.defer_bilateral(d, b);
    } break;
    case FL_FILT_LOGSCALE: launch_logscale(st, d, ln.d_front, p[0], p[1]); break;
    case FL_FILT_COLORCLIP: launch_colorclip(st, d, ln.d_front, p[0], p[1], p[2], p[3], p[4]); break;
    case FL_FILT_SMEARCLIP:
        gauss7(p[0], k7);
        launch_gamma_full_hi(st, d, ln.d_side, ln.d_front);
        launch_full_blur(st, d, ln.d_back, ln.d_side, 2, 0, k7);
        launch_full_blur(st, d, ln.d_side, ln.d_back, 3, 0, k7);
        launch_full_blur(st, d, ln.d_back, ln.d_side, 0, 0, k7);
        launch_full_blur(st, d, ln.d_side, ln.d_back, 1, 0, k7);
        launch_smearclip(st, d, ln.d_front, ln.d_side, p[1], p[2], p[3]);
        break;
    case FL_FILT_HALOCLIP:
        gauss7(1.0f, k7);
        launch_apply_gamma(st, d, ln.d_blur, ln.d_front, 0.1f);
        launch_den_blur_1c(st, d, (float *)ln.d_side.p, ln.d_blur, 2, 0, k7);
        launch_den_blur_1c(st, d, ln.d_blur, (const float *)ln.d_side.p, 3, 0, k7);
        launch_haloclip(st, d, ln.d_front, ln.d_blur, p[0]);
        break;
    case FL_FILT_PLAINCLIP: launch_plainclip(st, d, ln.d_front, p[0], p[1], p[2], p[3]); break;
    case FL_FILT_LOGENCODE:
        launch_logencode(st, d, ln.d_back, ln.d_front, p[0]);
        swap(ln.d_front, ln.d_back);
        break;
    case FL_FILT_DE:
        if (!(p[0] > 0.0f)) break;
        launch_de_adaptive(st, d, ln.d_front, ln.d_back, ln.d_blur, ln.d_de_tmax, ln.d_de_sinv,
                           p[0], std::min(std::max(p[1], 0.0f), p[0]), p[2]);
        break;
    }
    ev_end(c, e);
    if (rc) return rc;
    HIPCHK(hipGetLastError());
    return FL_OK;
}

int fl_resample(fl_ctx *c, uint32_t w, uint32_t h, uint32_t ss, const float *taps, uint32_t ntaps)
{
    REQUIRE(c && taps && w && h, "null argument");
    REQUIRE(ss >= 1 && ss <= FL_RESAMPLE_MAX_SS, "resample: ss must be 1..4");
    REQUIRE(ntaps >= ss && ntaps <= ss + 2 * FL_GUTTER && (ntaps - ss) % 2 == 0,
            "resample: ntaps must lie in [ss, ss + 24] and have the parity of ss");
    REQUIRE(w <= 0x7fffffffu / ss && h <= 0x7fffffffu / ss, "resample: source size overflows");
    for (uint32_t i = 0; i < ntaps; ++i) REQUIRE(std::isfinite(taps[i]), "resample: non-finite tap");
    HIPCHK(hipSetDevice(c->device));
    Lane &ln = c->lane();
    fl_dim din;
    const fl_dim dout = calc_dim(w, h);
    int rc = ensure_fb(ln, ss * w, ss * h, &din);
    if (rc) return rc;
    EvPair *e = ev_begin(c, c->filt_ev);
    if (!(rc = flush_pending(c, ln))) {
        launch_resample(ln.stream, din, dout, (int)ss, ln.d_back, ln.d_front, taps, (int)ntaps);
        swap(ln.d_front, ln.d_back);
    }
    ev_end(c, e);
    if (rc) return rc;
    HIPCHK(hipGetLastError());
    return FL_OK;
}

size_t fl_output_bytes(uint32_t w, uint32_t h, int fmt)
{
    const size_t n = (size_t)w * h;
    switch (fmt) {
    case FL_OUT_RGBA8: return 4 * n;
    case FL_OUT_RGBA16: return 8 * n;
    case FL_OUT_YUV444P: return 3 * n;
    case FL_OUT_YUV444P10: case FL_OUT_YUV444P12: return 6 * n;
    case FL_OUT_YUV420P10: return 3 * n;
    default: return 0;
    }
}

static int convert_front(fl_ctx *c, Lane &ln, uint32_t w, uint32_t h, int fmt, void *dst)
{
    fl_dim d;
    int rc = ensure_fb(ln, w, h, &d);
    if (rc) return rc;
    if ((rc = flush_pending(c, ln))) return rc;
    if ((rc = wait_other(c, 2))) return rc;
    launch_f32_to_rgba(ln.stream, d, ln.d_front, c->rng_out(), FL_NOUT, fmt, dst ? dst : (void *)ln.d_outpix.p);
    HIPCHK(hipGetLastError());
    HIPCHK(hipEventRecord(ln.ev_out_done, ln.stream));
    ln.out_rec = true;
    return FL_OK;
}

static int close_frame(fl_ctx *c, Lane &ln)
{
    if (c->frame_seq) HIPCHK(hipEventRecord(c->ev_end_[(c->frame_seq - 1) % fl_ctx::kFrames], ln.stream));
    return FL_OK;
}

int fl_output(fl_ctx *c, uint32_t w, uint32_t h, int fmt, void *host_out, uint64_t dev_out)
{
    REQUIRE(c && fl_output_bytes(w, h, fmt) != 0, "bad argument");
    REQUIRE(fmt != FL_OUT_YUV420P10 || (w % 2 == 0 && h % 2 == 0), "4:2:0 needs even width and height");
    HIPCHK(hipSetDevice(c->device));
    Lane &ln = c->lane();
    void *dev = (void *)(uintptr_t)dev_out;
    if (int rc = convert_front(c, ln, w, h, fmt, dev)) return rc;
    if (host_out) HIPCHK(hipMemcpyAsync(host_out, dev ? dev : (void *)ln.d_outpix.p, fl_output_bytes(w, h, fmt), hipMemcpyDeviceToHost, ln.stream));
    return close_frame(c, ln);
}

static bool sides_ok(uint32_t w, uint32_t h, uint32_t max = 65535u) { return w >= 1 && h >= 1 && w <= max && h <= max; }

static int check_sides(const char *enc, uint32_t w, uint32_t h)
{
    if (sides_ok(w, h)) return FL_OK;
    return fail(FL_E_INVAL, (std::string(enc) + ": width and height must be 1..65535").c_str(), __FILE__, __LINE__);
}
static int check_encode(const fl_ctx *c, const char *enc, uint32_t w, uint32_t h, size_t header, const void *host_out, uint64_t dev_out, size_t cap)
{
    REQUIRE(c, "null ctx");
    if (int rc = check_sides(enc, w, h)) return rc;
    const char *bad = cap < 16 + header ? "capacity below the record and the header" : !(host_out || dev_out) ? "no destination" : nullptr;
    if (!bad) return FL_OK;
    return fail(FL_E_INVAL, (std::string(enc) + ": " + bad).c_str(), __FILE__, __LINE__);
}

extern "C++" template <class Check, class Encode, class Late = int (*)()>
static int encode_source(fl_ctx *c, uint64_t src_dev, const char *no_source, Check check, Encode encode, Late late = +[] { return (int)FL_OK; })
{
    if (int rc = check()) return rc;
    REQUIRE(src_dev, no_source);
    if (int rc = late()) return rc;
    HIPCHK(hipSetDevice(c->device));
    return encode(c->lane());
}

extern "C++" template <class Check, class Source, class Encode>
static int encode_front(fl_ctx *c, Check check, Source source, Encode encode)
{
    if (int rc = check()) return rc;
    HIPCHK(hipSetDevice(c->device));
    Lane &ln = c->lane();
    if (int rc = source(ln)) return rc;
    if (int rc = encode(ln)) return rc;
    return close_frame(c, ln);
}
extern "C++" template <class Check, class Encode>
static int encode_front(fl_ctx *c, uint32_t w, uint32_t h, int fmt, Check check, Encode encode)
{
    return encode_front(c, check, [=](Lane &ln) { return convert_front(c, ln, w, h, fmt, nullptr); }, encode);
}

extern "C++" template <class Launch>
static int encode_on(fl_ctx *c, Lane &ln, void *host_out, uint64_t dev_out, size_t cap, size_t bound, size_t scratch_words,
                     const char *what_out, const char *what_scratch, Launch launch)
{
    unsigned char *dst = (unsigned char *)(uintptr_t)dev_out;
    bool copy_back = host_out && dst;
    const size_t dcap = std::min(cap, bound);
    const auto quiesce = [&ln] { return ln.quiesce(false); };
    if (!dst) {
        hipPointerAttribute_t at = {};
        const hipError_t e = hipPointerGetAttributes(&at, host_out);
        if (e == hipSuccess && at.type == hipMemoryTypeHost && at.devicePointer) dst = (unsigned char *)at.devicePointer;
        else {
            (void)hipGetLastError();
            if (int rc = ln.d_enc_out.reserve(dcap, what_out, quiesce)) return rc;
            dst = ln.d_enc_out;
            copy_back = true;
        }
    }
    if (int rc = ln.d_enc.reserve(scratch_words, what_scratch, quiesce)) return rc;
    EvPair *e = ev_begin_on(c, c->enc_ev, ln.stream);
    launch(ln.d_enc.p, dst);
    ev_end_on(e, ln.stream);
    HIPCHK(hipGetLastError());
    if (copy_back) HIPCHK(hipMemcpyAsync(host_out, dst, dcap, hipMemcpyDeviceToHost, ln.stream));
    return FL_OK;
}

size_t fl_jpeg_bound_s(uint32_t w, uint32_t h, int sampling)
{
    if (!sides_ok(w, h) || (sampling != FL_JPEG_444 && sampling != FL_JPEG_420)) return 0;
    if (sampling == FL_JPEG_420) return 16 + FL_JPEG_HEADER_BYTES + (size_t)((w + 15u) / 16u) * ((h + 15u) / 16u) * 2492u;
    return 16 + FL_JPEG_HEADER_BYTES + (size_t)((w + 7u) / 8u) * ((h + 7u) / 8u) * 1248u;
}

size_t fl_jpeg_bound(uint32_t w, uint32_t h) { return fl_jpeg_bound_s(w, h, FL_JPEG_444); }

static uint64_t jpeg_blocks(uint32_t w, uint32_t h, int sampling)
{
    return sampling == FL_JPEG_420 ? (uint64_t)((w + 15u) / 16u) * ((h + 15u) / 16u) * 6u : (uint64_t)((w + 7u) / 8u) * ((h + 7u) / 8u) * 3u;
}

size_t fl_jpeg_bound_f(uint32_t w, uint32_t h, int sampling, unsigned flags)
{
    if (!flags) return fl_jpeg_bound_s(w, h, sampling);
    if (flags != FL_JPEG_OPTIMIZE || !fl_jpeg_bound_s(w, h, sampling) || jpeg_blocks(w, h, sampling) > FL_JPEG_OPT_MAX_BLOCKS) return 0;
    if (sampling == FL_JPEG_420) return 16 + FL_JPEG_HEADER_BYTES + (size_t)((w + 15u) / 16u) * ((h + 15u) / 16u) * 2494u;
    return 16 + FL_JPEG_HEADER_BYTES + (size_t)((w + 7u) / 8u) * ((h + 7u) / 8u) * 1248u;
}

static int check_jpeg(const fl_ctx *c, uint32_t w, uint32_t h, int quality, int sampling, unsigned flags, const void *host_out, uint64_t dev_out, size_t cap)
{
    if (int rc = check_encode(c, "jpeg", w, h, FL_JPEG_HEADER_BYTES, host_out, dev_out, cap)) return rc;
    REQUIRE(quality >= 1 && quality <= 100, "jpeg: quality must be 1..100");
    REQUIRE(sampling == FL_JPEG_444 || sampling == FL_JPEG_420, "jpeg: sampling must be FL_JPEG_444 or FL_JPEG_420");
    REQUIRE(!(flags & ~(unsigned)FL_JPEG_OPTIMIZE), "jpeg: unknown flag");
    if (flags && jpeg_blocks(w, h, sampling) > FL_JPEG_OPT_MAX_BLOCKS) return fail(FL_E_UNSUPPORTED, "jpeg: FL_JPEG_OPTIMIZE takes frames of at most 2^24 blocks", __FILE__, __LINE__);
    return FL_OK;
}

static int jpeg_encode_on(fl_ctx *c, Lane &ln, uint32_t w, uint32_t h, const unsigned char *src, int quality, int sampling, unsigned flags,
                          void *host_out, uint64_t dev_out, size_t cap)
{
    const uint32_t ri = sampling == FL_JPEG_420 ? c->jpeg_ri_420 : c->jpeg_ri;
    const bool optimize = flags & FL_JPEG_OPTIMIZE;
    return encode_on(c, ln, host_out, dev_out, cap, fl_jpeg_bound_f(w, h, sampling, flags), jpeg_layout(w, h, ri, sampling).words, "jpeg stream", "jpeg scratch",
                     [=, st = ln.stream](uint32_t *scratch, unsigned char *dst) { launch_jpeg_encode(st, src, w, h, quality, ri, sampling, optimize, scratch, dst, cap); });
}

int fl_jpeg_encode_f(fl_ctx *c, uint32_t w, uint32_t h, uint64_t src_dev, int quality, int sampling, unsigned flags, void *host_out, uint64_t dev_out,
                     size_t cap)
{
    return encode_source(c, src_dev, "jpeg: null source planes", [&] { return check_jpeg(c, w, h, quality, sampling, flags, host_out, dev_out, cap); },
                         [&](Lane &ln) { return jpeg_encode_on(c, ln, w, h, (const unsigned char *)(uintptr_t)src_dev, quality, sampling, flags, host_out, dev_out, cap); });
}

int fl_jpeg_encode_s(fl_ctx *c, uint32_t w, uint32_t h, uint64_t src_dev, int quality, int sampling, void *host_out, uint64_t dev_out, size_t cap)
{
    return fl_jpeg_encode_f(c, w, h, src_dev, quality, sampling, 0u, host_out, dev_out, cap);
}

int fl_jpeg_encode(fl_ctx *c, uint32_t w, uint32_t h, uint64_t src_dev, int quality, void *host_out, uint64_t dev_out, size_t cap)
{
    return fl_jpeg_encode_s(c, w, h, src_dev, quality, FL_JPEG_444, host_out, dev_out, cap);
}

int fl_output_jpeg_f(fl_ctx *c, uint32_t w, uint32_t h, int quality, int sampling, unsigned flags, void *host_out, uint64_t dev_out, size_t cap)
{
    return encode_front(c, w, h, FL_OUT_YUV444P, [&] { return check_jpeg(c, w, h, quality, sampling, flags, host_out, dev_out, cap); },
                        [&](Lane &ln) { return jpeg_encode_on(c, ln, w, h, ln.d_outpix, quality, sampling, flags, host_out, dev_out, cap); });
}

int fl_output_jpeg_s(fl_ctx *c, uint32_t w, uint32_t h, int quality, int sampling, void *host_out, uint64_t dev_out, size_t cap)
{
    return fl_output_jpeg_f(c, w, h, quality, sampling, 0u, host_out, dev_out, cap);
// ... 91 lines not shown
                          uint32_t seq, void *host_out, uint64_t dev_out, size_t cap)
{
    const uint32_t seg = png_segment_bytes();
    return encode_on(c, ln, host_out, dev_out, cap, fl_apng_bound(w, h, channels, bits, flags), png_layout(w, h, channels, seg, bits, flags).words,
                     "apng frame block", "png scratch", [=, st = ln.stream](uint32_t *scratch, unsigned char *dst) {
                         launch_apng_encode(st, src, w, h, channels, bits, flags, seg, seq, scratch, dst, cap);
                     });
}

int fl_apng_encode(fl_ctx *c, uint32_t w, uint32_t h, uint64_t src_dev, int channels, int bits, unsigned flags, uint32_t seq, void *host_out,
                   uint64_t dev_out, size_t cap)
{
    return encode_source(c, src_dev, "png: null source pixels", [&] { return check_png(c, w, h, channels, host_out, dev_out, cap, 0); },
                         [&](Lane &ln) { return apng_encode_on(c, ln, w, h, (const unsigned char *)(uintptr_t)src_dev, channels, bits, flags, seq, host_out, dev_out, cap); },
                         [&] { return check_apng_f(w, h, channels, bits, flags, seq); });
}

int fl_output_apng(fl_ctx *c, uint32_t w, uint32_t h, int channels, int bits, unsigned flags, uint32_t seq, void *host_out, uint64_t dev_out,
                   size_t cap)
{
    return encode_front(c, w, h, bits == 16 ? FL_OUT_RGBA16 : FL_OUT_RGBA8,
                        [&] { const int rc = check_png(c, w, h, channels, host_out, dev_out, cap, 0); return rc ? rc : check_apng_f(w, h, channels, bits, flags, seq); },
                        [&](Lane &ln) { return apng_encode_on(c, ln, w, h, ln.d_outpix, channels, bits, flags, seq, host_out, dev_out, cap); });
}

size_t fl_tiff_bound(uint32_t w, uint32_t h, int channels, int bits)
{
    if (!sides_ok(w, h) || (channels != 3 && channels != 4) || (bits != 8 && bits != 16)) return 0;
    const TiffLayout l = tiff_layout(w, h, channels, bits);
    const uint64_t n = 16u + l.H + (uint64_t)l.nt * (l.tile_bytes + 5u + 6u + 1u);
    return n > 0xffffffffull ? 0 : (size_t)n;
}

static int check_tiff(const fl_ctx *c, uint32_t w, uint32_t h, int channels, int bits, const void *host_out, uint64_t dev_out, size_t cap)
{
    REQUIRE(c, "null ctx");
    REQUIRE(channels == 3 || channels == 4, "tiff: channels must be 3 or 4");
    REQUIRE(bits == 8 || bits == 16, "tiff: bits must be 8 or 16");
    if (int rc = check_sides("tiff", w, h)) return rc;
    if (int rc = check_encode(c, "tiff", w, h, (size_t)tiff_layout(w, h, channels, bits).H, host_out, dev_out, cap)) return rc;
    REQUIRE(fl_tiff_bound(w, h, channels, bits) != 0, "tiff: the file could pass 2^32 - 1 bytes");
    return FL_OK;
}

static int tiff_encode_on(fl_ctx *c, Lane &ln, uint32_t w, uint32_t h, const unsigned char *src, int channels, int bits, void *host_out,
                          uint64_t dev_out, size_t cap)
{
    return encode_on(c, ln, host_out, dev_out, cap, fl_tiff_bound(w, h, channels, bits), tiff_layout(w, h, channels, bits).words, "tiff file",
                     "tiff scratch", [=, st = ln.stream](uint32_t *scratch, unsigned char *dst) {
                         launch_tiff_encode(st, src, w, h, channels, bits, scratch, dst, cap);
                     });
}

int fl_tiff_encode(fl_ctx *c, uint32_t w, uint32_t h, uint64_t src_dev, int channels, int bits, void *host_out, uint64_t dev_out, size_t cap)
{
    return encode_source(c, src_dev, "tiff: null source pixels", [&] { return check_tiff(c, w, h, channels, bits, host_out, dev_out, cap); },
                         [&](Lane &ln) { return tiff_encode_on(c, ln, w, h, (const unsigned char *)(uintptr_t)src_dev, channels, bits, host_out, dev_out, cap); });
}

int fl_output_tiff(fl_ctx *c, uint32_t w, uint32_t h, int channels, int bits, void *host_out, uint64_t dev_out, size_t cap)
{
    return encode_front(c, w, h, bits == 16 ? FL_OUT_RGBA16 : FL_OUT_RGBA8, [&] { return check_tiff(c, w, h, channels, bits, host_out, dev_out, cap); },
                        [&](Lane &ln) { return tiff_encode_on(c, ln, w, h, ln.d_outpix, channels, bits, host_out, dev_out, cap); });
}

size_t fl_exr_bound(uint32_t w, uint32_t h, int channels, int pixel)
{
    if (!sides_ok(w, h) || (channels != 3 && channels != 4) || (pixel != FL_EXR_HALF && pixel != FL_EXR_FLOAT)) return 0;
    const ExrLayout l = exr_layout(w, h, channels, pixel);
    const uint64_t n = 16u + l.H + 20ull * l.nt + l.raw;
    return n > 0xffffffffull ? 0 : (size_t)n;
}

static int check_exr(const fl_ctx *c, uint32_t w, uint32_t h, int channels, int pixel, const void *host_out, uint64_t dev_out, size_t cap)
{
    REQUIRE(c, "null ctx");
    REQUIRE(channels == 3 || channels == 4, "exr: channels must be 3 or 4");
    REQUIRE(pixel == FL_EXR_HALF || pixel == FL_EXR_FLOAT, "exr: pixel must be FL_EXR_HALF or FL_EXR_FLOAT");
    if (int rc = check_sides("exr", w, h)) return rc;
    if (int rc = check_encode(c, "exr", w, h, (size_t)exr_layout(w, h, channels, pixel).H, host_out, dev_out, cap)) return rc;
    REQUIRE(fl_exr_bound(w, h, channels, pixel) != 0, "exr: the file could pass 2^32 - 1 bytes");
    return FL_OK;
}

static int exr_encode_on(fl_ctx *c, Lane &ln, uint32_t w, uint32_t h, const float4 *src, uint32_t src_stride, int channels, int pixel,
                         void *host_out, uint64_t dev_out, size_t cap)
{
    return encode_on(c, ln, host_out, dev_out, cap, fl_exr_bound(w, h, channels, pixel), exr_layout(w, h, channels, pixel).words, "exr file",
                     "exr scratch", [=, st = ln.stream](uint32_t *scratch, unsigned char *dst) {
                         launch_exr_encode(st, src, src_stride, w, h, channels, pixel, scratch, dst, cap);
                     });
}

int fl_exr_encode(fl_ctx *c, uint32_t w, uint32_t h, uint64_t src_dev, uint32_t src_stride, int channels, int pixel, void *host_out,
                  uint64_t dev_out, size_t cap)
{
    return encode_source(c, src_dev, "exr: null source pixels", [&] { return check_exr(c, w, h, channels, pixel, host_out, dev_out, cap); },
                         [&](Lane &ln) { return exr_encode_on(c, ln, w, h, (const float4 *)(uintptr_t)src_dev, src_stride, channels, pixel, host_out, dev_out, cap); },
                         [&]() -> int { REQUIRE(src_stride >= w, "exr: the source's stride is below the width"); return FL_OK; });
}

int fl_output_exr(fl_ctx *c, uint32_t w, uint32_t h, int channels, int pixel, void *host_out, uint64_t dev_out, size_t cap)
{
    fl_dim d;
    return encode_front(c, [&] { return check_exr(c, w, h, channels, pixel, host_out, dev_out, cap); },
                        [&](Lane &ln) { const int rc = ensure_fb(ln, w, h, &d); return rc ? rc : flush_pending(c, ln); },
                        [&](Lane &ln) {
                            const float4 *src = (const float4 *)ln.d_front.p + (size_t)d.astride * FL_GUTTER + FL_GUTTER;
                            return exr_encode_on(c, ln, w, h, src, d.astride, channels, pixel, host_out, dev_out, cap);
                        });
}

size_t fl_gif_bound(uint32_t w, uint32_t h)
{
    if (!sides_ok(w, h) || (uint64_t)w * h > (1ull << 24)) return 0;
    const uint64_t n = (uint64_t)w * h, T = (3u * n + 1u) / 2u + 11u * ((n + 255u) / 256u);
    return (size_t)(16u + FL_GIF_HEADER_BYTES + T + (T + 254u) / 255u + 1u);
}

static int check_gif(const fl_ctx *c, uint32_t w, uint32_t h, int colors, int amp, const void *host_out, uint64_t dev_out, size_t cap)
{
    if (int rc = check_encode(c, "gif", w, h, FL_GIF_HEADER_BYTES, host_out, dev_out, cap)) return rc;
    REQUIRE(colors >= 2 && colors <= 256, "gif: colors must be 2..256");
    REQUIRE(amp >= 0 && amp <= 64, "gif: dither_amp must be 0..64");
    REQUIRE(fl_gif_bound(w, h) != 0, "gif: the frame has more than 2^24 pixels");
    return FL_OK;
}

static int gif_encode_on(fl_ctx *c, Lane &ln, uint32_t w, uint32_t h, const unsigned char *src, int colors, int amp, void *host_out,
                         uint64_t dev_out, size_t cap)
{
    const uint32_t seg = c->gif_seg;
    return encode_on(c, ln, host_out, dev_out, cap, fl_gif_bound(w, h), gif_layout(w, h, seg).words, "gif block", "gif scratch",
                     [=, st = ln.stream](uint32_t *scratch, unsigned char *dst) { launch_gif_encode(st, src, w, h, colors, amp, seg, scratch, dst, cap); });
}

int fl_gif_encode(fl_ctx *c, uint32_t w, uint32_t h, uint64_t src_dev, int colors, int dither_amp, void *host_out, uint64_t dev_out, size_t cap)
{
    return encode_source(c, src_dev, "gif: null source pixels", [&] { return check_gif(c, w, h, colors, dither_amp, host_out, dev_out, cap); },
                         [&](Lane &ln) { return gif_encode_on(c, ln, w, h, (const unsigned char *)(uintptr_t)src_dev, colors, dither_amp, host_out, dev_out, cap); });
}

int fl_output_gif(fl_ctx *c, uint32_t w, uint32_t h, int colors, int dither_amp, void *host_out, uint64_t dev_out, size_t cap)
{
    return encode_front(c, w, h, FL_OUT_RGBA8, [&] { return check_gif(c, w, h, colors, dither_amp, host_out, dev_out, cap); },
                        [&](Lane &ln) { return gif_encode_on(c, ln, w, h, ln.d_outpix, colors, dither_amp, host_out, dev_out, cap); });
}

size_t fl_webp_bound(uint32_t w, uint32_t h, int channels)
{
    if (!sides_ok(w, h, 16384u) || (channels != 3 && channels != 4)) return 0;
    const uint64_t n = 16u + 8u + (webp_bound_bits(w, h) + 7u) / 8u + 1u;
    return n > 0xffffffffull ? 0 : (size_t)n;
}

static int check_webp(const fl_ctx *c, uint32_t w, uint32_t h, int channels, const void *host_out, uint64_t dev_out, size_t cap)
{
    if (int rc = check_encode(c, "webp", w, h, FL_WEBP_HEADER_BYTES, host_out, dev_out, cap)) return rc;
    REQUIRE(channels == 3 || channels == 4, "webp: channels must be 3 or 4");
    REQUIRE(sides_ok(w, h, 16384u), "webp: width and height must be 1..16384");
    REQUIRE(fl_webp_bound(w, h, channels) != 0, "webp: the block could pass 2^32 - 1 bytes");
    return FL_OK;
}

static int webp_encode_on(fl_ctx *c, Lane &ln, uint32_t w, uint32_t h, const unsigned char *src, int channels, void *host_out, uint64_t dev_out,
                          size_t cap)
{
    const size_t bound = fl_webp_bound(w, h, channels);
    return encode_on(c, ln, host_out, dev_out, cap, bound, webp_layout(w, h).words, "webp block", "webp scratch",
                     [=, st = ln.stream](uint32_t *scratch, unsigned char *dst) { launch_webp_encode(st, src, w, h, channels, scratch, dst, cap, bound); });
}

int fl_webp_encode(fl_ctx *c, uint32_t w, uint32_t h, uint64_t src_dev, int channels, void *host_out, uint64_t dev_out, size_t cap)
{
    return encode_source(c, src_dev, "webp: null source pixels", [&] { return check_webp(c, w, h, channels, host_out, dev_out, cap); },
                         [&](Lane &ln) { return webp_encode_on(c, ln, w, h, (const unsigned char *)(uintptr_t)src_dev, channels, host_out, dev_out, cap); });
}

int fl_output_webp(fl_ctx *c, uint32_t w, uint32_t h, int channels, void *host_out, uint64_t dev_out, size_t cap)
{
    return encode_front(c, w, h, FL_OUT_RGBA8, [&] { return check_webp(c, w, h, channels, host_out, dev_out, cap); },
                        [&](Lane &ln) { return webp_encode_on(c, ln, w, h, ln.d_outpix, channels, host_out, dev_out, cap); });
}

int fl_sort_u32(fl_ctx *c, uint64_t dst_dev, uint64_t src_dev, uint32_t n, uint32_t lo_bit, uint32_t nbits, int ignore_max,
                uint32_t *nvalid)
{
    REQUIRE(c && dst_dev && src_dev && dst_dev != src_dev, "null or aliased key arrays");
    REQUIRE(nbits >= 1 && nbits <= 10 && lo_bit + nbits <= 32, "a pass sorts 1..10 bits inside the 32-bit key");
    HIPCHK(hipSetDevice(c->device));
    if (n == 0) { if (nvalid) *nvalid = 0; return FL_OK; }
    size_t chunk_words = 0;
    const size_t hist_words = sort_scratch_words(n, nbits, &chunk_words);
    hipStream_t sst = c->lanes[0].stream;
    if (int rc = c->d_sort.reserve(hist_words + chunk_words, "sort scratch", [c] { sync_all(c); return (int)FL_OK; })) return rc;
    uint32_t *chunk_tot = c->d_sort + hist_words, *total_dev = chunk_tot + (chunk_words - 1);
    launch_sort_pass(sst, (uint32_t *)(uintptr_t)dst_dev, (const uint32_t *)(uintptr_t)src_dev, n, lo_bit, nbits,
                     ignore_max, c->d_sort, chunk_tot, total_dev);
    HIPCHK(hipGetLastError());
    if (nvalid) {
        HIPCHK(hipMemcpyAsync(nvalid, total_dev, 4, hipMemcpyDeviceToHost, sst));
        HIPCHK(hipStreamSynchronize(sst));
    }
    return FL_OK;
}

int fl_frame_ms(fl_ctx *c, uint32_t frame_id, float *ms)
{
    REQUIRE(c && ms, "null argument");
    REQUIRE(frame_id < c->frame_seq && c->frame_seq - frame_id <= fl_ctx::kFrames, "frame id no longer tracked");
    const uint32_t k = frame_id % fl_ctx::kFrames;
    HIPCHK(hipEventSynchronize(c->ev_end_[k]));
    HIPCHK(hipEventElapsedTime(ms, c->ev_begin_[k], c->ev_end_[k]));
    return FL_OK;
}

int fl_frame_query(fl_ctx *c, uint32_t frame_id)
{
    REQUIRE(c, "null ctx");
    REQUIRE(frame_id < c->frame_seq && c->frame_seq - frame_id <= fl_ctx::kFrames, "frame id no longer tracked");
    hipError_t e = hipEventQuery(c->ev_end_[frame_id % fl_ctx::kFrames]);
    if (e == hipSuccess) return 1;
    if (e == hipErrorNotReady) { (void)hipGetLastError(); return 0; }
    return fail(FL_E_HIP, "hipEventQuery", __FILE__, __LINE__, e);
}

void *fl_host_alloc(size_t nbytes)
{
    void *p = nullptr;
    if (hipHostMalloc(&p, nbytes, hipHostMallocDefault) != hipSuccess) { (void)hipGetLastError(); return nullptr; }
    return p;
}

void fl_host_free(void *p) { if (p) hipHostFree(p); }

static float sum_ms(std::vector<EvPair> &v)
{
    float t = 0.0f;
    for (auto &p : v) { float ms = 0.0f; if (hipEventElapsedTime(&ms, p.a, p.b) == hipSuccess) t += ms; }
    return t;
}

int fl_timings_reset(fl_ctx *c)
{
    REQUIRE(c, "null ctx");
    sync_all(c);
    c->iter_ev.clear(); c->accum_ev.clear(); c->flush_ev.clear(); c->filt_ev.clear(); c->de_ev.clear(); c->enc_ev.clear(); c->pool_used = 0;
    c->n_spec_launch = c->n_interp_launch = 0;
    return FL_OK;
}

int fl_timings_detail(fl_ctx *c, float ms[6])
{
    REQUIRE(c && ms, "null argument");
    sync_all(c);
    ms[0] = sum_ms(c->iter_ev); ms[1] = sum_ms(c->accum_ev); ms[2] = sum_ms(c->flush_ev);
    ms[3] = sum_ms(c->filt_ev); ms[4] = sum_ms(c->de_ev); ms[5] = sum_ms(c->enc_ev);
    return FL_OK;
}

int fl_launch_stats(fl_ctx *c, uint32_t out[4])
{
    REQUIRE(c && out, "null argument");
    out[0] = c->n_spec_launch; out[1] = c->n_interp_launch; out[2] = c->nslots; out[3] = (uint32_t)c->nw;
    return FL_OK;
}

int fl_measure_copy(int device, size_t nbytes, int iters, float *ms)
{
    REQUIRE(ms && iters > 0 && nbytes >= 16, "bad argument");
    HIPCHK(hipSetDevice(device));
    if (launch_measure_copy(nbytes, iters, ms)) return fail(FL_E_HIP, "copy measurement (allocation of 2 x nbytes, or the launch)", __FILE__, __LINE__);
    return FL_OK;
}

int fl_timings(fl_ctx *c, float *iter_ms, float *flush_ms, float *filter_ms, uint32_t *nlaunch)
{
    REQUIRE(c, "null ctx");
    sync_all(c);
    if (iter_ms) *iter_ms = sum_ms(c->iter_ev);
    if (flush_ms) *flush_ms = sum_ms(c->accum_ev) + sum_ms(c->flush_ev);
    if (filter_ms) *filter_ms = sum_ms(c->filt_ev);
    if (nlaunch) *nlaunch = (uint32_t)c->iter_ev.size();
    return FL_OK;
}

static int buf_ptr(fl_ctx *c, int which, void **p, size_t *cap)
{
    Lane &ln = c->lane();
    if (int rc = flush_pending(c, ln)) return rc;
    const auto is = [&](auto &b) { *p = b.p; *cap = b.bytes(); };
    switch (which) {
    case FL_BUF_FRONT: is(ln.d_front); break;
    case FL_BUF_BACK: is(ln.d_back); break;
    case FL_BUF_SIDE: is(ln.d_side); break;
    case FL_BUF_PARAMS: is(ln.d_params); break;
    case FL_BUF_PALETTE: is(ln.d_palette); break;
    case FL_BUF_POINTS: is(c->d_points); break;
    case FL_BUF_SEEDS: is(c->d_rng); break;
    case FL_BUF_ATOM: is(ln.d_atom); break;
    case FL_BUF_HOT: is(ln.d_hot); break;
    case FL_BUF_LOG: is(ln.d_log[0]); break;
    case FL_BUF_DIR: is(ln.d_dir[0]); break;
    default: return fail(FL_E_INVAL, "unknown buffer", __FILE__, __LINE__);
    }
    if (!*p) return fail(FL_E_INVAL, "buffer not allocated yet", __FILE__, __LINE__);
    return FL_OK;
}

int fl_buffer_ptr_async(fl_ctx *c, fl_genome *g, int which, void **dev_ptr, size_t *nbytes)
{
    REQUIRE(c && dev_ptr && nbytes, "null argument");
    HIPCHK(hipSetDevice(c->device));
    return buf_ptr(c, which, dev_ptr, nbytes);
}

int fl_buffer_ptr(fl_ctx *c, fl_genome *g, int which, void **dev_ptr, size_t *nbytes)
{
    const int rc = fl_buffer_ptr_async(c, g, which, dev_ptr, nbytes);
    if (rc == FL_OK) sync_all(c);
    return rc;
}

static int host_copy(fl_ctx *c, int which, void *host, size_t nbytes, bool to_device)
{
    REQUIRE(c && host, "null argument");
    HIPCHK(hipSetDevice(c->device));
    void *p; size_t cap;
    int rc = buf_ptr(c, which, &p, &cap);
    if (rc) return rc;
    REQUIRE(nbytes <= cap, to_device ? "write larger than buffer" : "read larger than buffer");
    sync_all(c);
    if (to_device) HIPCHK(hipMemcpy(p, host, nbytes, hipMemcpyHostToDevice));
    else HIPCHK(hipMemcpy(host, p, nbytes, hipMemcpyDeviceToHost));
    return FL_OK;
}

int fl_read_buffer(fl_ctx *c, fl_genome *g, int which, void *dst, size_t nbytes) { return host_copy(c, which, dst, nbytes, false); }

int fl_reserve(fl_ctx *c, uint32_t w, uint32_t h)
{
    REQUIRE(c && w && h, "bad argument");
    HIPCHK(hipSetDevice(c->device));
    fl_dim d;
    return ensure_fb(c->lane(), w, h, &d);
}

int fl_stream_dependency(fl_ctx *c, void *stream, int ctx_waits)
{
    REQUIRE(c, "null ctx");
    HIPCHK(hipSetDevice(c->device));
    Lane &ln = c->lane();
    hipStream_t other = (hipStream_t)stream;
    hipEvent_t &ev = c->dep_ev[c->dep_next++ % fl_ctx::kDepEvents];
    if (!ev) HIPCHK(hipEventCreateWithFlags(&ev, hipEventDisableTiming));
    if (ctx_waits) {
        HIPCHK(hipEventRecord(ev, other));
        HIPCHK(hipStreamWaitEvent(ln.stream, ev, 0));
    } else {
        if (int rc = flush_pending(c, ln)) return rc;
        HIPCHK(hipEventRecord(ev, ln.stream));
        HIPCHK(hipStreamWaitEvent(other, ev, 0));
    }
    return FL_OK;
}

int fl_write_buffer(fl_ctx *c, fl_genome *g, int which, const void *src, size_t nbytes)
{
    const int rc = host_copy(c, which, const_cast<void *>(src), nbytes, true);
    if (rc == FL_OK && which == FL_BUF_PARAMS) c->lane().params_serial = 0;
    return rc;
}

int fl_debug_clear(fl_ctx *c, uint32_t w, uint32_t h, int reset_points)
{
    REQUIRE(c, "null ctx");
    HIPCHK(hipSetDevice(c->device));
    Lane &ln = c->lane();
    fl_dim d;
    int rc = ensure_fb(ln, w, h, &d);
    if (rc) return rc;
    if ((rc = flush_pending(c, ln))) return rc;
    return do_clear(c, ln, d, reset_points != 0);
}

int fl_debug_iter_launch(fl_ctx *c, fl_genome *g, uint32_t w, uint32_t h, uint32_t round0,
                         uint32_t nrounds, uint32_t fuse, int accum_mode)
{
    REQUIRE(c && g && (accum_mode == FL_ACCUM_ATOMIC || accum_mode == FL_ACCUM_BINNED), "bad argument");
    Lane &ln = c->lane();
    REQUIRE(ln.d_params.cap >= (size_t)c->ntemporal() * g->pstride, "fl_interp has not run for this genome");
    HIPCHK(hipSetDevice(c->device));
    fl_dim d;
    int rc = ensure_fb(ln, w, h, &d);
    if (rc) return rc;
    c->round_counter = round0;
    HIPCHK(hipMemsetAsync(c->d_counters, 0, 32, ln.stream));
    return do_iter_launch(c, ln, g, d, nrounds, fuse, true, accum_mode);
}

int fl_debug_flush(fl_ctx *c, uint32_t w, uint32_t h)
{
    REQUIRE(c, "null ctx");
    Lane &ln = c->lane();
    fl_dim d;
    int rc = ensure_fb(ln, w, h, &d);
    if (rc) return rc;
    if ((rc = flush_pending(c, ln))) return rc;
    return do_flush(c, ln, d);
}

int fl_debug_accum_check(uint32_t w, uint32_t h, const uint32_t *log, size_t log_words, const uint32_t *dir, size_t dir_words,
                          uint32_t nbatch_total, uint32_t batch_records, uint32_t nslots, uint32_t nparts, int wide)
{
    fl_dim d;
    BinLayout b;
    const char *why = accum_log_check(w, h, log, log_words, dir, dir_words, nbatch_total, batch_records, nslots, nparts, wide, &d, &b);
    return why ? fail(FL_E_INVAL, why, __FILE__, __LINE__) : (int)FL_OK;
}

int fl_debug_accum(fl_ctx *c, uint32_t w, uint32_t h, const uint32_t *log, size_t log_words, const uint32_t *dir, size_t dir_words,
                   uint32_t nbatch_total, uint32_t batch_records, uint32_t nslots, uint32_t nparts, int wide)
{
    REQUIRE(c, "null ctx");
    fl_dim d;
    BinLayout bl;
    if (const char *why = accum_log_check(w, h, log, log_words, dir, dir_words, nbatch_total, batch_records, nslots, nparts, wide, &d, &bl))
        return fail(FL_E_INVAL, why, __FILE__, __LINE__);
    HIPCHK(hipSetDevice(c->device));
    Lane &ln = c->lane();
    int rc = ensure_fb(ln, w, h, &d);
    if (rc) return rc;
    if ((rc = flush_pending(c, ln))) return rc;
    const auto quiesce = [&ln] { return ln.quiesce(true); };
    if ((rc = ln.d_log[0].reserve(log_words, "sample log", quiesce))) return rc;
    if ((rc = ln.d_dir[0].reserve(dir_words, "sample log directory", quiesce))) return rc;
    if ((rc = quiesce())) return rc;
    HIPCHK(hipMemcpy(ln.d_log[0], log, 4 * log_words, hipMemcpyHostToDevice));
    HIPCHK(hipMemcpy(ln.d_dir[0], dir, 4 * dir_words, hipMemcpyHostToDevice));
    launch_accum_tiles(ln.stream, ln.d_log[0], ln.d_dir[0], ln.d_palette, ln.d_atom, (float *)ln.d_front.p, bl.tiles_x, bl.nbins,
                       nparts, nbatch_total, batch_records, nslots, d.astride, d.ah, bl.wide);
    HIPCHK(hipGetLastError());
    return FL_OK;
}

int fl_debug_clear_hot(fl_ctx *c, uint32_t w, uint32_t h)
{
    REQUIRE(c && c->lane().d_hot, "null ctx");
    const fl_dim d = calc_dim(w, h);
    HIPCHK(hipMemsetAsync(c->lane().d_hot, 0, 4 * ((size_t)d.ah * d.astride / 16), c->lane().stream));
    return FL_OK;
}

int fl_debug_shuffle(fl_ctx *c, uint32_t round, uint32_t *out256)
{
    REQUIRE(c && out256, "null argument");
    HIPCHK(hipSetDevice(c->device));
    DevBuf<uint32_t> d; const size_t n = (size_t)c->nw * 64;
    if (int rc = d.reserve(n, "shuffle tap scratch")) return rc;
    launch_shuffle_tap(c->lane().stream, c->nw, d, round);
    HIPCHK(hipStreamSynchronize(c->lane().stream));
    HIPCHK(hipMemcpy(out256, d, 4 * n, hipMemcpyDeviceToHost));
    return FL_OK;
}

int fl_debug_apply_xf(fl_ctx *c, fl_genome *g, uint32_t ts, int xfi, uint32_t n, float *xyzw, fl_mwc *rng)
{
    REQUIRE(c && g && xyzw && rng && n > 0 && ts < c->ntemporal(), "bad argument");
    REQUIRE(xfi >= 0 && xfi < g->prog[1] + g->prog[2], "xform index out of range");
    Lane &ln = c->lane();
    REQUIRE(ln.d_params.cap >= (size_t)c->ntemporal() * g->pstride, "fl_interp has not run for this genome");
    HIPCHK(hipSetDevice(c->device));
    DevBuf<float4> dp; DevBuf<fl_mwc> dr;
    int rc;
    if ((rc = dp.reserve(n, "xform tap scratch")) || (rc = dr.reserve(n, "xform tap scratch"))) return rc;
    HIPCHK(hipMemcpy(dp, xyzw, dp.bytes(), hipMemcpyHostToDevice));
    HIPCHK(hipMemcpy(dr, rng, dr.bytes(), hipMemcpyHostToDevice));
    launch_apply_xf_tap(ln.stream, g->d_prog, ln.d_params, ts, xfi, n, dp, dr);
    HIPCHK(hipStreamSynchronize(ln.stream));
    HIPCHK(hipMemcpy(xyzw, dp, dp.bytes(), hipMemcpyDeviceToHost));
    HIPCHK(hipMemcpy(rng, dr, dr.bytes(), hipMemcpyDeviceToHost));
    return FL_OK;
}

int fl_debug_math(fl_ctx *c, int fn, uint32_t n, const float *a, const float *b, uint32_t *out_bits)
{
    REQUIRE(c && a && b && out_bits, "null argument");
    REQUIRE(n > 0, "no elements");
    REQUIRE(fn >= 0 && fn < FL_MATH_COUNT, "unknown math helper");
    Lane &ln = c->lane();
    HIPCHK(hipSetDevice(c->device));
    DevBuf<float> da, db; DevBuf<uint32_t> dout;
    int rc;
    if ((rc = da.reserve(n, "math tap scratch")) || (rc = db.reserve(n, "math tap scratch")) || (rc = dout.reserve(n, "math tap scratch"))) return rc;
    HIPCHK(hipMemcpy(da, a, da.bytes(), hipMemcpyHostToDevice));
    HIPCHK(hipMemcpy(db, b, db.bytes(), hipMemcpyHostToDevice));
    launch_math_tap(ln.stream, fn, n, da, db, dout);
    HIPCHK(hipStreamSynchronize(ln.stream));
    HIPCHK(hipMemcpy(out_bits, dout, dout.bytes(), hipMemcpyDeviceToHost));
    return FL_OK;
}

int fl_debug_place(fl_ctx *c, const uint32_t *lens, uint32_t n, uint64_t front, uint64_t *offs_out, uint64_t *total_out)
{
    REQUIRE(c && lens && offs_out && total_out, "null argument");
    REQUIRE(n > 0, "no elements");
    Lane &ln = c->lane();
    HIPCHK(hipSetDevice(c->device));
    DevBuf<uint32_t> dl; DevBuf<u64> doffs;
    int rc;
    if ((rc = dl.reserve(n, "placement tap scratch")) || (rc = doffs.reserve((size_t)n + 1u, "placement tap scratch"))) return rc;
    HIPCHK(hipMemcpy(dl, lens, dl.bytes(), hipMemcpyHostToDevice));
    launch_debug_place(ln.stream, dl, n, front, doffs, doffs.p + n);
    HIPCHK(hipStreamSynchronize(ln.stream));
    HIPCHK(hipMemcpy(offs_out, doffs, 8 * (size_t)n, hipMemcpyDeviceToHost));
    HIPCHK(hipMemcpy(total_out, doffs.p + n, 8, hipMemcpyDeviceToHost));
    return FL_OK;
}

int fl_debug_de_dir(fl_ctx *c, uint32_t w, uint32_t h, int pattern, const float *scalars, int in_mode, int order)
{
    REQUIRE(c && scalars, "null argument");
    REQUIRE(pattern >= 0 && pattern <= 7, "de direction must be 0..7");
    REQUIRE(order >= -1 && order <= 2, "tile order must be -1 (the table's) or 0..2");
    REQUIRE(pattern != 0 || in_mode == 1 || in_mode == 2, "direction 0 reads the raw accumulator: in_mode 1, or 2 (YUV)");
    REQUIRE(w && h, "empty frame");
    HIPCHK(hipSetDevice(c->device));
    Lane &ln = c->lane();
    fl_dim d;
    int rc = ensure_fb(ln, w, h, &d);
    if (rc) return rc;
    if ((rc = flush_pending(c, ln))) return rc;
    float k7[7];
    gauss7(1.0f, k7);
    HIPCHK(hipMemsetAsync(ln.d_back, 0xff, 16 * (size_t)d.ah * d.astride, ln.stream));
    const DeTail none = {};
    launch_de_dir(ln.stream, d, pattern, ln.d_back, ln.d_front, k7, scalars[0], scalars[1], scalars[2], scalars[3], scalars[4],
                  in_mode, pattern == 7 ? &none : nullptr, order);
    swap(ln.d_front, ln.d_back);
    HIPCHK(hipGetLastError());
    return FL_OK;
}

int fl_rtc_compile_check(const int32_t *prog, uint32_t nprog, const int32_t *ops, uint32_t nops, int nw, int count, int acc,
                         char *log, size_t log_bytes)
{
    REQUIRE(prog && ops && nprog >= FL_PROG_HDR && (nw == 4 || nw == 8 || nw == 16) && acc >= 0 && acc <= 3, "bad argument");
    int rc = check_prog(prog, nprog);
    if (rc) return rc;
    for (uint32_t i = 0; i < nops; ++i) if ((rc = check_structure_op(prog, ops + 4 * i))) return rc;
    IterSpec spec = iter_spec(prog, nprog, ops, nops);
    for (std::vector<int> &v : spec.vids) for (int &id : v) if (id < 0) id = 0;
    std::vector<char> code;
    std::string err;
    rc = rtc_compile(spec, nw, (count & 1) != 0, acc, &code, &err, nullptr, (count & 2) == 0 ? 0u : nw == 8 ? 1u : nw == 16 ? 2u : 0u);
    if (log && log_bytes) { snprintf(log, log_bytes, "%s", rc ? err.c_str() : "ok"); }
    if (rc) return fail(rtc_available() ? FL_E_HIP : FL_E_UNSUPPORTED, "per-genome kernel did not compile", __FILE__, __LINE__);
    return (int)(code.size() > 0 ? FL_OK : FL_E_HIP);
}

int fl_genome_prepare(fl_ctx *c, fl_genome *g, uint32_t w, uint32_t h, int accum_mode)
{
    REQUIRE(c && g, "null argument");
    REQUIRE(accum_mode == FL_ACCUM_ATOMIC || accum_mode == FL_ACCUM_BINNED || accum_mode == 2, "bad accumulation mode");
    HIPCHK(hipSetDevice(c->device));
    const int kacc = accum_mode == FL_ACCUM_BINNED && c->layout(calc_dim(w, h)).wide ? 3 : accum_mode;
    bool pending = false;
    (void)rtc_variant(c, g, false, kacc, c->rtc_async ? RTC_POLL : RTC_SYNC, &pending);
    return FL_OK;
}

int fl_rtc_wait(fl_ctx *c, fl_genome *g)
{
    REQUIRE(c && g, "null argument");
    HIPCHK(hipSetDevice(c->device));
    const int geom = c->sub_log2 ? 2 + (int)c->sub_log2 : c->nw == 16 ? 2 : c->nw == 8 ? 1 : 0;
    for (int count = 0; count < 2; ++count)
        for (int kacc = 0; kacc < 4; ++kacc) {
            if (!g->rtc_want[geom][count][kacc]) continue;
            REQUIRE(!rtc_held(), "the worker is held (fl_debug_rtc_hold): its jobs cannot finish");
            bool pending = false;
            (void)rtc_variant(c, g, count != 0, kacc, RTC_WAIT, &pending);
        }
    return FL_OK;
}

int fl_rtc_stats(uint64_t out[8])
{
    REQUIRE(out, "null argument");
    rtc_stats(out);
    return FL_OK;
}

int fl_debug_rtc_hold(int on) { rtc_hold(on != 0); return FL_OK; }

int fl_debug_counters(fl_ctx *c, uint64_t out4[4])
{
    REQUIRE(c && out4, "null argument");
    sync_all(c);
    HIPCHK(hipMemcpy(out4, c->d_counters, 32, hipMemcpyDeviceToHost));
    return FL_OK;
}

}
#pragma GCC visibility pop
```

### cuburn_amd/csrc/iter.hip

```cpp
#include "variations.h"
#ifndef FL_RTC
#include "kernels.h"
#include <hip/hip_ext.h>
#endif

#define FL_CNT_SETS 3
#define FL_CNT_SETS_BIG 2
#define FL_SCATTER_DEPTH 4
#ifndef FL_ITER_MERGE_MAX_XF
#define FL_ITER_MERGE_MAX_XF 4
#endif
#ifndef FL_SORT_FULL_COPY
#define FL_SORT_FULL_COPY 1
#endif
#ifndef FL_SORT_LOCAL_TID
#define FL_SORT_LOCAL_TID 1
#endif

template <int NW>
__device__ __forceinline__ uint32_t shuffle_dest(uint32_t w, uint32_t l, uint32_t phase) {
    uint32_t sh = l + (phase == 1 ? l / NW : 0u) + (phase == 2 ? l / (NW * NW) : 0u);
    return ((w + sh) % NW) * 64u + l;
}

// ... 552 lines not shown
                    if constexpr (OPAC) { if (any_opac && k == bg.nbins) return false; }
                    return k != 0xffffffffu;
                };
#pragma unroll
                for (int q = 0; q < FL_BIN_R_MAX; ++q) {
                    const bool have = (uint32_t)q < staged;
                    r2[q] = have ? stage[q * NT + tid] : 0u;
                    k2[q] = !have ? 0xffffffffu : WIDE ? (uint32_t)skey[q * NT + tid] : r2[q] >> PAY_BITS;
                }
                const uint32_t nchunk = (bg.nbins + 64u) >> 6;
                if (nchunk <= 8u) {
                    if (w == 0) {
                        uint32_t running = 0;
                        for (uint32_t c0 = 0; c0 <= bg.nbins; c0 += 64) {
                            const uint32_t b = c0 + l;
                            uint32_t vs[SETS], v = 0;
#pragma unroll
                            for (int t = 0; t < SETS; ++t) { vs[t] = b <= bg.nbins ? cnt[t * CNTW + b] : 0u; v += vs[t]; }
                            const uint32_t incl = wave_incl_scan(v, l);
                            const uint32_t excl = incl - v + running;
                            if (b <= bg.nbins) {
                                uint32_t at = excl;
#pragma unroll
                                for (int t = 0; t < SETS; ++t) { cnt[t * CNTW + b] = at; at += vs[t]; }
                            }
                            if (b < bg.nbins) bin_dir[(size_t)b * bg.nbatch_total + batch_id] = (excl << 16) | v;
                            if (b == bg.nbins) *s_nvalid = excl;
                            running += (uint32_t)__builtin_amdgcn_readlane((int)incl, 63);
                        }
                    }
                } else {
                for (uint32_t c = w; c < nchunk; c += NW) {
                    const uint32_t b = c * 64u + l;
                    uint32_t v = 0;
#pragma unroll
                    for (int t = 0; t < SETS; ++t) v += b <= bg.nbins ? cnt[t * CNTW + b] : 0u;
                    const uint32_t incl = wave_incl_scan(v, l);
                    if (l == 63u) tot[c] = incl;
                }
                __syncthreads();
                {
                    const uint32_t t0 = l < nchunk ? tot[l] : 0u, t1 = 64u + l < nchunk ? tot[64u + l] : 0u;
                    const uint32_t i0 = wave_incl_scan(t0, l);
                    const uint32_t i1 = wave_incl_scan(t1, l) + (uint32_t)__builtin_amdgcn_readlane((int)i0, 63);
                    for (uint32_t cv = w; cv < nchunk; cv += NW) {
                        const uint32_t c = (uint32_t)__builtin_amdgcn_readfirstlane((int)cv);
                        const uint32_t base = c < 64u ? (uint32_t)__builtin_amdgcn_readlane((int)(i0 - t0), c)
                                                      : (uint32_t)__builtin_amdgcn_readlane((int)(i1 - t1), c - 64u);
                        const uint32_t b = c * 64u + l;
                        uint32_t vs[SETS], v = 0;
#pragma unroll
                        for (int t = 0; t < SETS; ++t) { vs[t] = b <= bg.nbins ? cnt[t * CNTW + b] : 0u; v += vs[t]; }
                        const uint32_t excl = wave_incl_scan(v, l) - v + base;
                        if (b <= bg.nbins) {
                            uint32_t at = excl;
#pragma unroll
                            for (int t = 0; t < SETS; ++t) { cnt[t * CNTW + b] = at; at += vs[t]; }
                            if (b < bg.nbins) bin_dir[(size_t)b * bg.nbatch_total + batch_id] = (excl << 16) | v;
                            else *s_nvalid = excl;
                        }
                    }
                }
                }
                __syncthreads();
#pragma unroll
                for (int q0 = 0; q0 < FL_BIN_R_MAX; q0 += FL_SCATTER_DEPTH) {
                    if ((uint32_t)q0 >= staged) break;
                    uint32_t pos[FL_SCATTER_DEPTH];
#pragma unroll
                    for (int q = 0; q < FL_SCATTER_DEPTH; ++q)
                        if (has_record(k2[q0 + q]))
                            pos[q] = __hip_atomic_fetch_add(my_cnt + k2[q0 + q], 1u, __ATOMIC_RELAXED, __HIP_MEMORY_SCOPE_WORKGROUP);
#pragma unroll
                    for (int q = 0; q < FL_SCATTER_DEPTH; ++q)
                        if (has_record(k2[q0 + q])) stage[pos[q]] = r2[q0 + q] & ((1u << PAY_BITS) - 1u);
                }
                __syncthreads();
                const uint32_t nvalid = *s_nvalid;
                if constexpr (PACK3) {
                    typedef uint32_t u32x2_ __attribute__((ext_vector_type(2)));
                    u32x2_ *d2 = reinterpret_cast<u32x2_ *>(bin_log) + (size_t)batch_id * fl_pack3_words(bg.rounds * NT);
                    const uint32_t nwords = (nvalid + 2u) / 3u;
                    for (uint32_t i = tid; i < nwords; i += NT) {
                        const uint32_t a = stage[3u * i], b = stage[3u * i + 1u], c3 = stage[3u * i + 2u];
                        u32x2_ o;
                        o.x = a | (b << 21); o.y = (b >> 11) | (c3 << 10);
                        __builtin_nontemporal_store(o, d2 + i);
                    }
                } else {
                uint4 *dst = reinterpret_cast<uint4 *>(bin_log + (size_t)batch_id * bg.rounds * NT);
                {
                    typedef uint32_t u32x4_ __attribute__((ext_vector_type(4)));
                    const u32x4_ *s4 = reinterpret_cast<const u32x4_ *>(stage);
                    u32x4_ *d4 = reinterpret_cast<u32x4_ *>(dst);
                    for (uint32_t i = tid; i * 4 < nvalid; i += NT) __builtin_nontemporal_store(s4[i], d4 + i);
                }
                }
                for (uint32_t i = tid; i < SETS * CNTW; i += NT) cnt[i] = 0;
                ++batch_in_slot;
                __syncthreads();
            };
#if FL_SORT_FULL_COPY
            if (blen == (uint32_t)FL_BIN_R_MAX) sort_batch((uint32_t)FL_BIN_R_MAX); else
#endif
            sort_batch(blen);
    }
    }

    if (ACC == 0) drain_if_full(pend_ok, pend_old, pend_gi, pend_mult, atom, out4, n_spill);
    else if (pend_old == 0x123456789abcdefull) atom[0] = pend_old;
    {
        uint32_t tid_end = threadIdx.x;
        asm volatile("" : "+v"(tid_end));
        const size_t wj = (size_t)slot * NT + tid_end;
        points[wj] = make_float4(x, y, color, CHAOS ? (float)nx : 0.0f);
        rng[wj].mul = rctx.mul; rng[wj].state = rctx.state; rng[wj].carry = rctx.carry;
    }

    if (COUNT) {
        atomicAdd(counters + 0, (u64)n_acc);
        atomicAdd(counters + 1, (u64)n_oob);
        atomicAdd(counters + 2, (u64)n_drop);
        atomicAdd(counters + 3, (u64)n_spill);
    }
}

#define FL_ITER_ARGS const int32_t *__restrict__ prog, const float *__restrict__ params, \
       const u64 *__restrict__ palette, fl_mwc *__restrict__ rng, float4 *__restrict__ points, \
       const uint32_t *__restrict__ hot, u64 *__restrict__ atom, float *__restrict__ out4, \
       u64 *__restrict__ counters, uint32_t astride, uint32_t aheight, \
       uint32_t round0, uint32_t nrounds, uint32_t fuse, BinGeom bg, \
       uint32_t *__restrict__ bin_log, uint32_t *__restrict__ bin_dir
#define FL_ITER_PASS prog, params, palette, rng, points, hot, atom, out4, counters, astride, aheight, round0, nrounds, fuse, bg, bin_log, bin_dir

#ifdef FL_RTC
extern "C" __global__ void __launch_bounds__(FL_SPEC_NW * 64) k_iter_spec(FL_ITER_ARGS)
{
    extern __shared__ __attribute__((aligned(16))) unsigned char smem[];
    iter_body<FL_SPEC_NW, FL_SPEC_COUNT != 0, FL_SPEC_ACC, true, FL_SPEC_CHAOS != 0>(smem, FL_ITER_PASS);
}
#else
template <int NW, bool COUNT, int ACC, bool CHAOS = false>
__global__ void __launch_bounds__(NW * 64, NW == 4 ? (CHAOS ? 5 : 6) : NW == 8 ? 3 : 1) k_iter(FL_ITER_ARGS)
{
    extern __shared__ __attribute__((aligned(16))) unsigned char smem[];
    iter_body<NW, COUNT, ACC, false, CHAOS>(smem, FL_ITER_PASS);
}

__global__ void __launch_bounds__(256)
k_apply_xf_tap(const int32_t *__restrict__ prog, const float *__restrict__ params, uint32_t ts, int xfi,
               uint32_t n, float4 *__restrict__ pts, fl_mwc *__restrict__ rng)
{
    const uint32_t i = blockIdx.x * 256u + threadIdx.x;
    if (i >= n) return;
    const float *__restrict__ P = params + (size_t)ts * prog[3];
    mwc_t r = {rng[i].mul, rng[i].state, rng[i].carry};
    float4 p = pts[i];
    const float *__restrict__ xf = P + prog[5] + xfi * prog[6];
    const XfHead h = load_head(xf);
    xf_apply(h, xf, XfInterp<false>(h, prog[7], false), p.x, p.y, p.z, r);
    pts[i] = p;
    rng[i].mul = r.mul; rng[i].state = r.state; rng[i].carry = r.carry;
}

void launch_apply_xf_tap(hipStream_t st, const int32_t *prog, const float *params, uint32_t ts, int xfi,
                         uint32_t n, float4 *pts, fl_mwc *rng)
{
    hipLaunchKernelGGL(k_apply_xf_tap, dim3((n + 255) / 256), dim3(256), 0, st, prog, params, ts, xfi, n, pts, rng);
}

__global__ void __launch_bounds__(256)
k_math_tap(int fn, uint32_t n, const float *__restrict__ a, const float *__restrict__ b, uint32_t *__restrict__ out)
{
    const uint32_t i = blockIdx.x * 256u + threadIdx.x;
    if (i >= n) return;
    const float x = a[i], y = b[i];
    float r = 0.0f;
    switch (fn) {
    case FL_MATH_RCP: r = frcp(x); break;
    case FL_MATH_DIV: r = fdiv(x, y); break;
    case FL_MATH_SQRT: r = fsqrt(x); break;
    case FL_MATH_EXP2: r = fexp2(x); break;
    case FL_MATH_LOG2: r = flog2(x); break;
    case FL_MATH_EXP: r = fexp(x); break;
    case FL_MATH_LOG: r = flog(x); break;
    case FL_MATH_POW: r = fpow(x, y); break;
    case FL_MATH_SIN: r = fsin(x); break;
    case FL_MATH_COS: r = fcos(x); break;
    case FL_MATH_TAN: r = ftan(x); break;
    case FL_MATH_ATAN2: r = v_atan2(x, y); break;
    case FL_MATH_SINH: r = v_sinh(x); break;
    case FL_MATH_COSH: r = v_cosh(x); break;
    case FL_MATH_FMOD: r = v_fmod(x, y); break;
    case FL_MATH_FMOD_PI: r = v_fmod_pi(x); break;
    case FL_MATH_TRUNCA: out[i] = trunca(x); return;
    case FL_MATH_HW_SIN: r = __builtin_amdgcn_sinf(x); break;
    case FL_MATH_HW_COS: r = __builtin_amdgcn_cosf(x); break;
    default: break;
    }
    out[i] = __float_as_uint(r);
}

void launch_math_tap(hipStream_t st, int fn, uint32_t n, const float *a, const float *b, uint32_t *out)
{
    hipLaunchKernelGGL(k_math_tap, dim3((n + 255) / 256), dim3(256), 0, st, fn, n, a, b, out);
}

template <int NW>
__global__ void __launch_bounds__(NW * 64) k_shuffle_tap(uint32_t *out, uint32_t round)
{
    __shared__ uint32_t s[NW * 64];
    const uint32_t tid = threadIdx.x;
    s[shuffle_dest<NW>(tid >> 6, tid & 63, round % 3u)] = tid;
    __syncthreads();
    out[tid] = s[tid];
}

__global__ void __launch_bounds__(256)
k_flush(u64 *__restrict__ atom, float4 *__restrict__ out, uint32_t *__restrict__ hot, uint32_t nbins, int use_hot)
{
    const uint32_t gi = blockIdx.x * 256u + threadIdx.x;
    if (gi >= nbins) return;
    const uint32_t sh = (gi & 15u) << 1;
    const uint32_t flag = use_hot ? (hot[gi >> 4] >> sh) & 3u : 0u;
    const float mult = hot_mult(flag);
    const u64 cell = __builtin_nontemporal_load(atom + gi);
    __builtin_nontemporal_store(0ull, atom + gi);
    float yf, uf, vf, df;
    unpack_cell(cell, yf, uf, vf, df);
    float4 o = out[gi];
    const float m255 = mult * FL_INV255;
    o.w = fmaf(df, mult, o.w);
    o.x = fmaf(yf, m255, o.x);
    o.y = fmaf(uf, m255, o.y);
    o.z = fmaf(vf, m255, o.z);
    out[gi] = o;
    uint32_t nf = (uint32_t)(o.w > 128.0f) + (uint32_t)(o.w > 512.0f) + (uint32_t)(o.w > 2048.0f);
    uint32_t word = nf << sh;
    word |= __shfl_xor(word, 1);
    word |= __shfl_xor(word, 2);
    word |= __shfl_xor(word, 4);
    word |= __shfl_xor(word, 8);
    if ((gi & 15u) == 0) hot[gi >> 4] = word;
}

static size_t iter_lds_bytes(int nw, int acc, uint32_t rounds, uint32_t nbins, uint32_t sub_log2, bool chaos)
{
    size_t nt = (size_t)nw * 64, b = 2 * (chaos ? 4 : 3) * nt * 4;
    if (acc == 1 || acc == 3) b += (size_t)rounds * nt * (acc == 3 ? 6 : 4) + (nw == 4 ? FL_CNT_SETS : FL_CNT_SETS_BIG) * (size_t)((nbins + 1 + 3) & ~3u) * 4 + 16
             + 128 * 4;
    else b += FL_PAL_W * 8;
    return b + ((size_t)FL_XTAB_BYTES << sub_log2);
}

void launch_iter(hipStream_t st, const IterLaunch &L, hipFunction_t fn)
{
    const int nw = L.nw;
    if (L.sub_log2 != 0u && (4 << L.sub_log2) != nw) abort();
    BinGeom bg = {L.tiles_x, L.nbins, L.rounds_per_batch, L.nbatch_total, L.sub_log2};
    const size_t lds = iter_lds_bytes(nw, L.acc, L.rounds_per_batch, L.nbins, L.sub_log2, L.chaos);
    if (fn) {
        IterLaunch a = L;
        void *args[] = {&a.prog, &a.params, &a.palette, &a.rng, &a.points, &a.hot, &a.atom, &a.out4, &a.counters, &a.astride, &a.aheight,
                        &a.round0, &a.nrounds, &a.fuse, &bg, &a.log, &a.dir};
        (void)hipExtModuleLaunchKernel(fn, L.nslots * (uint32_t)nw * 64, 1, 1, (uint32_t)nw * 64, 1, 1, lds, st, args, nullptr, L.ev_start, L.ev_stop, 0);
        return;
    }
#define LAUNCH_X(NW, C, A, X) do { \
        static unsigned long long attr_done = 0; \
        ensure_max_dynamic_lds((const void *)k_iter<NW, C, A, X>, attr_done); \
         \
        hipExtLaunchKernelGGL((k_iter<NW, C, A, X>), dim3(L.nslots), dim3(NW * 64), lds, st, L.ev_start, L.ev_stop, 0, L.prog, L.params, L.palette, \
        L.rng, L.points, L.hot, L.atom, L.out4, L.counters, L.astride, L.aheight, L.round0, L.nrounds, L.fuse, bg, L.log, L.dir); } while (0)
#define LAUNCH(NW, C, A) do { if (L.chaos) LAUNCH_X(NW, C, A, true); else LAUNCH_X(NW, C, A, false); } while (0)
#define LAUNCH_NW(C, A) do { if (nw == 4) LAUNCH(4, C, A); else if (nw == 8) LAUNCH(8, C, A); else LAUNCH(16, C, A); } while (0)
    if (L.acc == 2) LAUNCH_NW(false, 2);
    else if (L.acc == 1) { if (L.count) LAUNCH_NW(true, 1); else LAUNCH_NW(false, 1); }
    else if (L.acc == 3) { if (L.count) LAUNCH_NW(true, 3); else LAUNCH_NW(false, 3); }
    else { if (L.count) LAUNCH_NW(true, 0); else LAUNCH_NW(false, 0); }
#undef LAUNCH_NW
#undef LAUNCH
#undef LAUNCH_X
}

void launch_flush(hipStream_t st, u64 *atom, float4 *out, uint32_t *hot, uint32_t nbins, bool use_hot)
{
    hipLaunchKernelGGL(k_flush, dim3((nbins + 255) / 256), dim3(256), 0, st, atom, out, hot, nbins, use_hot ? 1 : 0);
}

__global__ void __launch_bounds__(256)
k_clear_frame(float4 *__restrict__ front, u64 *__restrict__ atom, uint32_t *__restrict__ hot, u64 *__restrict__ counters,
              float4 *__restrict__ points, uint32_t nbins, uint32_t npoints)
{
    const uint32_t i = blockIdx.x * 256u + threadIdx.x;
    if (i < nbins) {
        front[i] = make_float4(0.0f, 0.0f, 0.0f, 0.0f);
        atom[i] = 0ull;
        if ((i & 15u) == 0u) hot[i >> 4] = 0u;
    }
    if (i < npoints) {
        const float nanf_ = __uint_as_float(0x7fc00000u);
        points[i] = make_float4(nanf_, nanf_, nanf_, nanf_);
    }
    if (i < 4u) counters[i] = 0ull;
}

void launch_clear_frame(hipStream_t st, float4 *front, u64 *atom, uint32_t *hot, u64 *counters, float4 *points,
                        uint32_t nbins, uint32_t npoints)
{
    const uint32_t n = nbins > npoints ? nbins : npoints;
    hipLaunchKernelGGL(k_clear_frame, dim3((n + 255) / 256), dim3(256), 0, st, front, atom, hot, counters, points, nbins, npoints);
}

void launch_shuffle_tap(hipStream_t st, int nw, uint32_t *out, uint32_t round)
{
    if (nw == 4) hipLaunchKernelGGL(k_shuffle_tap<4>, dim3(1), dim3(256), 0, st, out, round);
    else if (nw == 8) hipLaunchKernelGGL(k_shuffle_tap<8>, dim3(1), dim3(512), 0, st, out, round);
    else hipLaunchKernelGGL(k_shuffle_tap<16>, dim3(1), dim3(1024), 0, st, out, round);
}
#endif
```

### cuburn_amd/csrc/kernels.h

```cpp
#pragma once
#include <hip/hip_runtime.h>
#include <stdint.h>
#include "../../include/flame_hip.h"

typedef unsigned long long u64;

static inline void ensure_max_dynamic_lds(const void *fn, unsigned long long &done)
{
    int dev = 0;
    if (hipGetDevice(&dev) != hipSuccess || dev < 0 || dev > 63) dev = 63;
    if (done >> dev & 1ull) return;
    hipFuncSetAttribute(fn, hipFuncAttributeMaxDynamicSharedMemorySize, 160 * 1024);
    if (dev != 63) done |= 1ull << dev;
}

struct IterLaunch {
    int nw; bool count; int acc; uint32_t nslots;
    const int32_t *prog; const float *params; const u64 *palette; fl_mwc *rng; float4 *points;
    const uint32_t *hot; u64 *atom; float *out4; u64 *counters;
    uint32_t astride, aheight, round0, nrounds, fuse;
    uint32_t tiles_x, nbins, rounds_per_batch, nbatch_total;
    uint32_t *log, *dir;
    hipEvent_t ev_start, ev_stop;
    uint32_t sub_log2;
    bool chaos;
};
void launch_iter(hipStream_t st, const IterLaunch &launch, hipFunction_t fn);
void launch_flush(hipStream_t st, u64 *atom, float4 *out, uint32_t *hot, uint32_t nbins, bool use_hot);
void launch_clear_frame(hipStream_t st, float4 *front, u64 *atom, uint32_t *hot, u64 *counters, float4 *points,
                        uint32_t nbins, uint32_t npoints);
void launch_shuffle_tap(hipStream_t st, int nw, uint32_t *out, uint32_t round);
void launch_apply_xf_tap(hipStream_t st, const int32_t *prog, const float *params, uint32_t ts, int xfi,
                         uint32_t n, float4 *pts, fl_mwc *rng);
void launch_math_tap(hipStream_t st, int fn, uint32_t n, const float *a, const float *b, uint32_t *out);

#include <string>
#include <vector>
struct IterSpec {
    int nxf = 0, has_final = 0, pstride = 0, cdf_off = 0, xf_off = 0, xf_stride = 0, var_stride = 0;
    int chaos = 0, chaos_off = 0;
    std::vector<int> nvar, post, opac;
    std::vector<std::vector<int>> vids;
};
bool rtc_available();
unsigned rtc_epoch();
int rtc_compile(const IterSpec &spec, int nw, bool count, int acc, std::vector<char> *code, std::string *err, const char *extra_opt = nullptr, uint32_t sub_log2 = 0);
enum { RTC_SYNC = 0, RTC_POLL = 1, RTC_WAIT = 2 };
int rtc_iter_kernel(int device, const IterSpec &spec, int nw, uint32_t nslots, bool count, int acc, hipFunction_t *fn, std::string *err, uint32_t sub_log2 = 0,
                    int mode = RTC_SYNC);
void rtc_stats(uint64_t out[8]);
void rtc_count_launch(bool spec, bool pending);
void rtc_hold(bool on);
bool rtc_held();

void launch_accum_tiles(hipStream_t st, const uint32_t *log, const uint32_t *dir, const u64 *palette,
                        u64 *atom, float *out4, uint32_t tiles_x, uint32_t nbins, uint32_t nparts,
                        uint32_t nbatch_total, uint32_t batch_records, uint32_t nslots,
                        uint32_t astride, uint32_t aheight, bool wide);

void launch_interp_palette(hipStream_t st, fl_mwc *rng_pal, const float *ptimes, const float4 *pals,
                           float ts, float tstep, u64 *out);
void launch_interp_params(hipStream_t st, float *params, const float *times, const float *knots,
                          const int32_t *ops, uint32_t nops, uint32_t pstride, uint32_t nts, float ts, float tstep,
                          fl_dim dim, bool zero_first);

void launch_yuv_to_rgb(hipStream_t st, fl_dim d, float4 *dst, const float4 *src);
void launch_den_blur_1c(hipStream_t st, fl_dim d, float *dst, const float *src, int pattern, int upsample, const float *coefs7);
void launch_full_blur(hipStream_t st, fl_dim d, float4 *dst, const float4 *src, int pattern, int upsample, const float *coefs7);
void launch_logscale(hipStream_t st, fl_dim d, float4 *buf, float k1, float k2);
void launch_colorclip(hipStream_t st, fl_dim d, float4 *buf, float vib, float highpow, float gam, float lin, float lingam);
void launch_gamma_full_hi(hipStream_t st, fl_dim d, float4 *dst, const float4 *src);
void launch_smearclip(hipStream_t st, fl_dim d, float4 *buf, const float4 *smear, float gam_m_1, float lin, float lingam);
void launch_apply_gamma(hipStream_t st, fl_dim d, float *dst, const float4 *src, float gamma);
void launch_haloclip(hipStream_t st, fl_dim d, float4 *buf, const float *den, float gam_m_1);
void launch_plainclip(hipStream_t st, fl_dim d, float4 *buf, float gam_m_1, float lin, float lingam, float brightness);
void launch_logencode(hipStream_t st, fl_dim d, float4 *dst, const float4 *src, float degamma);

struct DeTail { int do_log; float k1, k2; int do_clip; float vib, highpow, gam, lin, lingam; int order; };
void launch_de_dir(hipStream_t st, fl_dim d, int pattern, float4 *Nout, const float4 *N, const float *coefs7,
                   float sstd, float cstd, float dstd, float dpow, float gspeed, int in_mode = 1, const DeTail *tail = nullptr,
                   int order_override = -1);

void launch_de_adaptive(hipStream_t st, fl_dim d, float4 *buf, float4 *stage_c, float *stage_a, uint32_t *tmax,
                        const float *sinv, float R, float Rmin, float curve);
size_t de_adaptive_tiles(fl_dim d);
void de_adaptive_norms(float *out);

void launch_resample(hipStream_t st, fl_dim din, fl_dim dout, int ss, float4 *dst, const float4 *src, const float *taps, int ntaps);

void launch_f32_to_rgba(hipStream_t st, fl_dim d, const float4 *src, fl_mwc *rng, uint32_t nrng, int fmt, void *dst);

#define FL_JPEG_RI 8u
#define FL_JPEG_RI_420 4u
#define FL_JPEG_RI_420_MAX 10u
#define FL_JPEG_OPT_MAX_BLOCKS (1u << 24)
struct JpegLayout { uint32_t mw, nmcu, nint; size_t coef, offs, lens, acbits, info, counts, huff, words; };
JpegLayout jpeg_layout(uint32_t w, uint32_t h, uint32_t ri, int sampling);
void launch_jpeg_encode(hipStream_t st, const unsigned char *src, uint32_t w, uint32_t h, int quality, uint32_t ri, int sampling, bool optimize,
                        uint32_t *scratch, unsigned char *out, size_t cap);
void launch_debug_place(hipStream_t st, const uint32_t *lens, uint32_t n, u64 front, u64 *offs, u64 *total);

#define FL_PNG_SEG 32768u
struct PngLayout { uint32_t rowlen, nseg, stride, per; uint64_t F; size_t filt, segbuf, offs, lens, adl, info, types, words; };
uint32_t png_segment_bytes();
PngLayout png_layout(uint32_t w, uint32_t h, int channels, uint32_t seg, int bits, unsigned flags);
void launch_png_encode(hipStream_t st, const unsigned char *src, uint32_t w, uint32_t h, int channels, int bits, unsigned flags, uint32_t seg,
                       uint32_t *scratch, unsigned char *out, size_t cap);
void launch_apng_encode(hipStream_t st, const unsigned char *src, uint32_t w, uint32_t h, int channels, int bits, unsigned flags, uint32_t seg,
                        uint32_t seq, uint32_t *scratch, unsigned char *out, size_t cap);

void launch_deflate_tiles(hipStream_t st, const unsigned char *bytes, uint32_t tile_bytes, uint32_t ntiles, unsigned char *segbuf, uint32_t stride,
                          uint32_t *lens, uint32_t *adl);

#define FL_TIFF_TILE_LENGTH 64u
struct TiffLayout { uint32_t tw, tiles_x, nt, tile_bytes, stride, entries, fixed; uint64_t H, F; size_t tiled, segbuf, offs, lens, adl, info, words; };
TiffLayout tiff_layout(uint32_t w, uint32_t h, int channels, int bits);
void launch_tiff_encode(hipStream_t st, const unsigned char *src, uint32_t w, uint32_t h, int channels, int bits, uint32_t *scratch,
                        unsigned char *out, size_t cap);

void launch_deflate_pieces(hipStream_t st, const unsigned char *bytes, uint32_t tile_bytes, uint32_t ntiles, unsigned char *segbuf, uint32_t stride,
                           uint32_t *lens, uint32_t *adl);

#define FL_EXR_TILE_WIDTH 64u
#define FL_EXR_TILE_ROWS_HALF 64u
#define FL_EXR_TILE_ROWS_FLOAT 32u
struct ExrLayout { uint32_t th, tiles_x, nt, tile_bytes, stride, header; uint64_t H, raw; size_t staged, segbuf, offs, lens, adl, info, words; };
ExrLayout exr_layout(uint32_t w, uint32_t h, int channels, int pixel);
void launch_exr_encode(hipStream_t st, const float4 *src, uint32_t src_stride, uint32_t w, uint32_t h, int channels, int pixel, uint32_t *scratch,
                       unsigned char *out, size_t cap);

#define FL_GIF_SEG 1024u
#define FL_GIF_LZW_TABLE_BYTES 32768u
struct GifLayout { uint32_t npix, seg, nseg, stride, slots_log2, lanes; size_t hist, ccnt, pal, lut, idx, segbuf, offs, lens, info, words; };
uint32_t gif_segment_pixels();
GifLayout gif_layout(uint32_t w, uint32_t h, uint32_t seg);
void launch_gif_encode(hipStream_t st, const unsigned char *src, uint32_t w, uint32_t h, int colors, int amp, uint32_t seg, uint32_t *scratch,
                       unsigned char *out, size_t cap);

struct WebpLayout { uint32_t ptx, pty, gx, gy, G, NR, subwords; size_t asmwords, modes, codes, hdr, cnt, off, sub, subinfo, info, asmb, words; };
uint64_t webp_bound_bits(uint32_t w, uint32_t h);
WebpLayout webp_layout(uint32_t w, uint32_t h);
void launch_webp_encode(hipStream_t st, const unsigned char *src, uint32_t w, uint32_t h, int channels, uint32_t *scratch, unsigned char *out,
                        size_t cap, size_t bound);

int launch_measure_copy(size_t nbytes, int iters, float *ms);

int launch_sort_pass(hipStream_t st, uint32_t *dst, const uint32_t *src, uint32_t n, uint32_t lo_bit, uint32_t nbits,
                     int ignore_max, uint32_t *hist, uint32_t *chunk_tot, uint32_t *total_dev);
size_t sort_scratch_words(uint32_t n, uint32_t nbits, size_t *chunk_words);
```

### include/flame_hip.h

```cpp
#ifndef FLAME_HIP_H
#define FLAME_HIP_H

#ifndef __HIPCC_RTC__
#include <stdint.h>
#include <stddef.h>
#endif

#ifdef __cplusplus
extern "C" {
#endif

#define FL_ABI_VERSION 1

enum {
    FL_OK = 0,
    FL_E_INVAL = -1,
    FL_E_NOMEM = -2,
    FL_E_HIP = -3,
    FL_E_NODEV = -4,
    FL_E_UNSUPPORTED = -5
};

typedef struct fl_dim {
    uint32_t w, h, aw, ah, astride;
} fl_dim;

typedef struct fl_mwc {
    uint32_t mul, state, carry;
} fl_mwc;

#define FL_KNOTS 32
#define FL_NTEMPORAL 1024
#define FL_PAL_W 256
#define FL_PAL_H 64
#define FL_GUTTER 12

#define FL_PROG_MAGIC 0x464c5032
#define FL_PROG_HDR 8
#define FL_MAX_XFORMS 64
#define FL_CHAOS_MAX_XFORMS 32
#define FL_MAX_PSTRIDE 4096
#define FL_XF_HDR 16

enum {
    FL_OP_SPLINE = 0,
    FL_OP_SPLINE_MAG = 1,
    FL_OP_CAMERA = 2,
    FL_OP_AFFINE = 3,
    FL_OP_CDF = 4,
    FL_OP_RATIO2 = 5,
    FL_OP_INVSQ = 6,
    FL_OP_PERSP = 7,
    FL_OP_INVSQ_MAX = 8,
    FL_OP_CONST = 9,
    FL_OP_OPACITY = 10,
    FL_OP_CHAOS_CDF = 11,
};


typedef struct fl_ctx fl_ctx;
typedef struct fl_genome fl_genome;

int fl_abi_version(void);
const char *fl_last_error(void);

void fl_calc_dim(uint32_t w, uint32_t h, fl_dim *out);

int fl_ctx_create(int device, void *stream, const fl_mwc *seeds, uint32_t nseeds, uint32_t nslots, fl_ctx **out);
void fl_ctx_destroy(fl_ctx *ctx);
int fl_ctx_sync(fl_ctx *ctx);

int fl_genome_create(fl_ctx *ctx, const int32_t *prog, uint32_t nprog,
                     const int32_t *ops, uint32_t nops, uint32_t nrows, fl_genome **out);
void fl_genome_destroy(fl_genome *g);

int fl_genome_upload(fl_ctx *ctx, fl_genome *g, const float *times, const float *knots,
                     const float *pal_rgba, const float *pal_times, uint32_t npal);

int fl_interp(fl_ctx *ctx, fl_genome *g, uint32_t w, uint32_t h, float ts, float td);

enum {
    FL_ACCUM_ATOMIC = 0,
    FL_ACCUM_BINNED = 1
};

int fl_iterate(fl_ctx *ctx, fl_genome *g, uint32_t w, uint32_t h, double nsamples,
               uint32_t fuse, int accum_mode, uint64_t *nsamples_run);

enum {
    FL_FILT_YUV = 0,
    FL_FILT_BILATERAL = 1,
    FL_FILT_LOGSCALE = 2,
    FL_FILT_COLORCLIP = 3,
    FL_FILT_SMEARCLIP = 4,
    FL_FILT_HALOCLIP = 5,
    FL_FILT_PLAINCLIP = 6,
    FL_FILT_LOGENCODE = 7,
    FL_FILT_DE = 8
};
#define FL_DE_MAX_RADIUS 96
int fl_filter(fl_ctx *ctx, int filter_id, uint32_t w, uint32_t h, const float *params, uint32_t nparams);

#define FL_RESAMPLE_MAX_SS 4
#define FL_RESAMPLE_MAX_TAPS (FL_RESAMPLE_MAX_SS + 2 * FL_GUTTER)
int fl_resample(fl_ctx *ctx, uint32_t w, uint32_t h, uint32_t ss, const float *taps, uint32_t ntaps);

enum {
    FL_OUT_RGBA8 = 0,
    FL_OUT_RGBA16 = 1,
    FL_OUT_YUV444P = 2,
    FL_OUT_YUV444P10 = 3,
    FL_OUT_YUV420P10 = 4,
    FL_OUT_YUV444P12 = 5
};
size_t fl_output_bytes(uint32_t w, uint32_t h, int fmt);
int fl_output(fl_ctx *ctx, uint32_t w, uint32_t h, int fmt, void *host_out, uint64_t dev_out);

#define FL_JPEG_HEADER_BYTES 629
size_t fl_jpeg_bound(uint32_t w, uint32_t h);
int fl_jpeg_encode(fl_ctx *ctx, uint32_t w, uint32_t h, uint64_t src_dev, int quality, void *host_out, uint64_t dev_out, size_t cap);
int fl_output_jpeg(fl_ctx *ctx, uint32_t w, uint32_t h, int quality, void *host_out, uint64_t dev_out, size_t cap);

enum { FL_JPEG_444 = 0, FL_JPEG_420 = 1 };
size_t fl_jpeg_bound_s(uint32_t w, uint32_t h, int sampling);
int fl_jpeg_encode_s(fl_ctx *ctx, uint32_t w, uint32_t h, uint64_t src_dev, int quality, int sampling,
                     void *host_out, uint64_t dev_out, size_t cap);
int fl_output_jpeg_s(fl_ctx *ctx, uint32_t w, uint32_t h, int quality, int sampling,
                     void *host_out, uint64_t dev_out, size_t cap);

enum { FL_JPEG_OPTIMIZE = 1 };
size_t fl_jpeg_bound_f(uint32_t w, uint32_t h, int sampling, unsigned flags);
int fl_jpeg_encode_f(fl_ctx *ctx, uint32_t w, uint32_t h, uint64_t src_dev, int quality, int sampling, unsigned flags,
                     void *host_out, uint64_t dev_out, size_t cap);
int fl_output_jpeg_f(fl_ctx *ctx, uint32_t w, uint32_t h, int quality, int sampling, unsigned flags,
                     void *host_out, uint64_t dev_out, size_t cap);

#define FL_PNG_HEADER_BYTES 33
size_t fl_png_bound(uint32_t w, uint32_t h, int channels);
int fl_png_encode(fl_ctx *ctx, uint32_t w, uint32_t h, uint64_t src_dev, int channels, void *host_out, uint64_t dev_out, size_t cap);
int fl_output_png(fl_ctx *ctx, uint32_t w, uint32_t h, int channels, void *host_out, uint64_t dev_out, size_t cap);

enum { FL_PNG_ADAPTIVE = 1 };
size_t fl_png_bound_f(uint32_t w, uint32_t h, int channels, int bits, unsigned flags);
int fl_png_encode_f(fl_ctx *ctx, uint32_t w, uint32_t h, uint64_t src_dev, int channels, int bits, unsigned flags,
                    void *host_out, uint64_t dev_out, size_t cap);
int fl_output_png_f(fl_ctx *ctx, uint32_t w, uint32_t h, int channels, int bits, unsigned flags,
                    void *host_out, uint64_t dev_out, size_t cap);

enum { FL_APNG_IDAT = 0xffffffffu };
uint32_t fl_apng_chunks(uint32_t w, uint32_t h, int channels, int bits);
size_t fl_apng_bound(uint32_t w, uint32_t h, int channels, int bits, unsigned flags);
int fl_apng_encode(fl_ctx *ctx, uint32_t w, uint32_t h, uint64_t src_dev, int channels, int bits, unsigned flags, uint32_t seq,
                   void *host_out, uint64_t dev_out, size_t cap);
int fl_output_apng(fl_ctx *ctx, uint32_t w, uint32_t h, int channels, int bits, unsigned flags, uint32_t seq,
                   void *host_out, uint64_t dev_out, size_t cap);

size_t fl_tiff_bound(uint32_t w, uint32_t h, int channels, int bits);
int fl_tiff_encode(fl_ctx *ctx, uint32_t w, uint32_t h, uint64_t src_dev, int channels, int bits,
                   void *host_out, uint64_t dev_out, size_t cap);
int fl_output_tiff(fl_ctx *ctx, uint32_t w, uint32_t h, int channels, int bits, void *host_out, uint64_t dev_out, size_t cap);

enum { FL_EXR_HALF = 1, FL_EXR_FLOAT = 2 };
size_t fl_exr_bound(uint32_t w, uint32_t h, int channels, int pixel);
int fl_exr_encode(fl_ctx *ctx, uint32_t w, uint32_t h, uint64_t src_dev, uint32_t src_stride, int channels, int pixel,
                  void *host_out, uint64_t dev_out, size_t cap);
int fl_output_exr(fl_ctx *ctx, uint32_t w, uint32_t h, int channels, int pixel, void *host_out, uint64_t dev_out, size_t cap);

#define FL_GIF_HEADER_BYTES 779
size_t fl_gif_bound(uint32_t w, uint32_t h);
int fl_gif_encode(fl_ctx *ctx, uint32_t w, uint32_t h, uint64_t src_dev, int colors, int dither_amp,
                  void *host_out, uint64_t dev_out, size_t cap);
int fl_output_gif(fl_ctx *ctx, uint32_t w, uint32_t h, int colors, int dither_amp, void *host_out, uint64_t dev_out, size_t cap);

#define FL_WEBP_PB 4
#define FL_WEBP_EB 6
#define FL_WEBP_HEADER_BYTES 8
size_t fl_webp_bound(uint32_t w, uint32_t h, int channels);
int fl_webp_encode(fl_ctx *ctx, uint32_t w, uint32_t h, uint64_t src_dev, int channels, void *host_out, uint64_t dev_out, size_t cap);
int fl_output_webp(fl_ctx *ctx, uint32_t w, uint32_t h, int channels, void *host_out, uint64_t dev_out, size_t cap);

int fl_sort_u32(fl_ctx *ctx, uint64_t dst_dev, uint64_t src_dev, uint32_t n, uint32_t lo_bit, uint32_t nbits, int ignore_max,
                uint32_t *nvalid);

int fl_frame_begin(fl_ctx *ctx, uint32_t *frame_id);
int fl_frame_ms(fl_ctx *ctx, uint32_t frame_id, float *ms);
int fl_frame_query(fl_ctx *ctx, uint32_t frame_id);

void *fl_host_alloc(size_t nbytes);
void fl_host_free(void *p);

int fl_timings_reset(fl_ctx *ctx);
int fl_timings(fl_ctx *ctx, float *iter_ms, float *flush_ms, float *filter_ms, uint32_t *niter_launches);
int fl_timings_detail(fl_ctx *ctx, float ms[6]);
int fl_launch_stats(fl_ctx *ctx, uint32_t out[4]);
int fl_measure_copy(int device, size_t nbytes, int iters, float *ms);

enum {
    FL_BUF_FRONT = 0,
    FL_BUF_BACK = 1,
    FL_BUF_PARAMS = 2,
    FL_BUF_PALETTE = 3,
    FL_BUF_POINTS = 4,
    FL_BUF_SEEDS = 5,
    FL_BUF_ATOM = 6,
    FL_BUF_HOT = 7,
    FL_BUF_SIDE = 8,
    FL_BUF_LOG = 9,
    FL_BUF_DIR = 10
};
int fl_read_buffer(fl_ctx *ctx, fl_genome *g, int which, void *host_dst, size_t nbytes);
int fl_write_buffer(fl_ctx *ctx, fl_genome *g, int which, const void *host_src, size_t nbytes);

int fl_buffer_ptr(fl_ctx *ctx, fl_genome *g, int which, void **dev_ptr, size_t *nbytes);
int fl_buffer_ptr_async(fl_ctx *ctx, fl_genome *g, int which, void **dev_ptr, size_t *nbytes);
int fl_stream_dependency(fl_ctx *ctx, void *stream, int ctx_waits);
int fl_reserve(fl_ctx *ctx, uint32_t w, uint32_t h);

int fl_debug_iter_launch(fl_ctx *ctx, fl_genome *g, uint32_t w, uint32_t h, uint32_t round0,
                         uint32_t nrounds, uint32_t fuse, int accum_mode);
int fl_debug_flush(fl_ctx *ctx, uint32_t w, uint32_t h);
int fl_debug_clear(fl_ctx *ctx, uint32_t w, uint32_t h, int reset_points);
int fl_debug_clear_hot(fl_ctx *ctx, uint32_t w, uint32_t h);
int fl_debug_accum(fl_ctx *ctx, uint32_t w, uint32_t h, const uint32_t *log, size_t log_words, const uint32_t *dir, size_t dir_words,
                   uint32_t nbatch_total, uint32_t batch_records, uint32_t nslots, uint32_t nparts, int wide);
int fl_debug_accum_check(uint32_t w, uint32_t h, const uint32_t *log, size_t log_words, const uint32_t *dir, size_t dir_words,
                         uint32_t nbatch_total, uint32_t batch_records, uint32_t nslots, uint32_t nparts, int wide);
int fl_debug_shuffle(fl_ctx *ctx, uint32_t round, uint32_t *out256);
int fl_debug_apply_xf(fl_ctx *ctx, fl_genome *g, uint32_t ts, int xfi, uint32_t n, float *xyzw, fl_mwc *rng);
enum {
    FL_MATH_RCP = 0, FL_MATH_DIV, FL_MATH_SQRT, FL_MATH_EXP2, FL_MATH_LOG2, FL_MATH_EXP, FL_MATH_LOG, FL_MATH_POW,
    FL_MATH_SIN, FL_MATH_COS, FL_MATH_TAN,
    FL_MATH_ATAN2, FL_MATH_SINH, FL_MATH_COSH, FL_MATH_FMOD, FL_MATH_FMOD_PI,
    FL_MATH_TRUNCA,
    FL_MATH_HW_SIN, FL_MATH_HW_COS,
    FL_MATH_COUNT
};
int fl_debug_math(fl_ctx *ctx, int fn, uint32_t n, const float *a, const float *b, uint32_t *out_bits);
int fl_debug_place(fl_ctx *ctx, const uint32_t *lens, uint32_t n, uint64_t front, uint64_t *offs_out, uint64_t *total_out);
int fl_debug_de_dir(fl_ctx *ctx, uint32_t w, uint32_t h, int pattern, const float scalars[5], int in_mode, int order);
int fl_rtc_compile_check(const int32_t *prog, uint32_t nprog, const int32_t *ops, uint32_t nops, int nw, int count, int acc,
                         char *log, size_t log_bytes);
int fl_genome_prepare(fl_ctx *ctx, fl_genome *g, uint32_t w, uint32_t h, int accum_mode);
int fl_rtc_wait(fl_ctx *ctx, fl_genome *g);
int fl_rtc_stats(uint64_t out[8]);
int fl_debug_rtc_hold(int on);
int fl_debug_counters(fl_ctx *ctx, uint64_t out4[4]);


#ifdef __cplusplus
}
#endif
#endif
```

Before: 220,300 Msamples/s.

## Fuse per-tile atom drain into accumulate kernel via last-block tickets

```diff
diff --git a/cuburn_amd/_lib.py b/cuburn_amd/_lib.py
--- a/cuburn_amd/_lib.py
+++ b/cuburn_amd/_lib.py
@@ -8,7 +8,7 @@
 (FL_OK, FL_E_INVAL, FL_E_NOMEM, FL_E_HIP, FL_E_NODEV, FL_E_UNSUPPORTED) = (0, -1, -2, -3, -4, -5)
 
 FILT = dict(yuv=0, bilateral=1, logscale=2, colorclip=3, smearclip=4, haloclip=5, plainclip=6, logencode=7, de=8)
-BUF = dict(front=0, back=1, params=2, palette=3, points=4, seeds=5, atom=6, hot=7, side=8, log=9, dir=10)
+BUF = dict(front=0, back=1, params=2, palette=3, points=4, seeds=5, atom=6, hot=7, side=8, log=9, dir=10, ticket=11)
 ACCUM_ATOMIC, ACCUM_BINNED = 0, 1
 FL_OP_CHAOS_CDF = 11
 FL_OP_OPACITY = 10
@@ -104,6 +104,8 @@
     'fl_debug_clear_hot': (C.c_int, [C.c_void_p, C.c_uint32, C.c_uint32]),
     'fl_debug_accum': (C.c_int, [C.c_void_p, C.c_uint32, C.c_uint32, C.c_void_p, C.c_size_t, C.c_void_p, C.c_size_t,
                                  C.c_uint32, C.c_uint32, C.c_uint32, C.c_uint32, C.c_int]),
+    'fl_debug_accum_drain': (C.c_int, [C.c_void_p, C.c_uint32, C.c_uint32, C.c_void_p, C.c_size_t, C.c_void_p, C.c_size_t,
+                                       C.c_uint32, C.c_uint32, C.c_uint32, C.c_uint32, C.c_int]),
     'fl_debug_accum_check': (C.c_int, [C.c_uint32, C.c_uint32, C.c_void_p, C.c_size_t, C.c_void_p, C.c_size_t,
                                        C.c_uint32, C.c_uint32, C.c_uint32, C.c_uint32, C.c_int]),
     'fl_debug_shuffle': (C.c_int, [C.c_void_p, C.c_uint32, C.c_void_p]),
diff --git a/cuburn_amd/csrc/binned.hip b/cuburn_amd/csrc/binned.hip
--- a/cuburn_amd/csrc/binned.hip
+++ b/cuburn_amd/csrc/binned.hip
@@ -113,11 +113,48 @@
 }
 
 template <uint32_t TWL>
+__device__ __forceinline__ void drain_tile_if_last(uint32_t *flag, u64 *__restrict__ atom, float *__restrict__ out4, uint32_t *__restrict__ ticket,
+                                                   uint32_t bin, uint32_t nparts, uint32_t tx, uint32_t ty, uint32_t astride, uint32_t aheight)
+{
+    constexpr uint32_t TW = 1u << TWL, CELLS = TW * FL_TILE_H;
+    const uint32_t tid = threadIdx.x;
+    asm volatile("s_waitcnt vmcnt(0)" ::: "memory");
+    __syncthreads();
+    if (tid == 0u) {
+        __builtin_amdgcn_fence(__ATOMIC_RELEASE, "agent");
+        asm volatile("s_waitcnt vmcnt(0)" ::: "memory");
+        const bool last = __hip_atomic_fetch_add(ticket + bin, 1u, __ATOMIC_RELAXED, __HIP_MEMORY_SCOPE_AGENT) == nparts - 1u;
+        if (last) {
+            __hip_atomic_store(ticket + bin, 0u, __ATOMIC_RELAXED, __HIP_MEMORY_SCOPE_AGENT);
+            __builtin_amdgcn_fence(__ATOMIC_ACQUIRE, "agent");
+        }
+        *flag = last ? 1u : 0u;
+    }
+    __syncthreads();
+    if (*flag == 0u) return;
+    for (uint32_t i0 = tid; i0 < CELLS; i0 += blockDim.x * ACC_ADD_ILP) {
+        u64 cur[ACC_ADD_ILP];
+        uint32_t gi[ACC_ADD_ILP];
+#pragma unroll
+        for (uint32_t k = 0; k < ACC_ADD_ILP; ++k) {
+            const uint32_t i = min(i0 + k * blockDim.x, CELLS - 1u);
+            const uint32_t px = min(tx * TW + (i & (TW - 1u)), astride - 1u), py = min(ty * FL_TILE_H + (i >> TWL), aheight - 1u);
+            gi[k] = py * astride + px;
+            cur[k] = __hip_atomic_exchange(atom + gi[k], 0ull, __ATOMIC_RELAXED, __HIP_MEMORY_SCOPE_AGENT);
+        }
+#pragma unroll
+        for (uint32_t k = 0; k < ACC_ADD_ILP; ++k)
+            if (cur[k] != 0ull) spill_cell(cur[k], gi[k], out4);
+    }
+}
+
+template <uint32_t TWL>
 __global__ void __launch_bounds__(TWL == 7u ? ACC_THREADS : 1024, TWL == 7u ? 8 : 4) __attribute__((amdgpu_num_sgpr(80)))
 k_accum_tiles(const uint32_t *__restrict__ log, const uint32_t *__restrict__ dir,
               const u64 *__restrict__ palette, u64 *__restrict__ atom, float *__restrict__ out4,
               uint32_t tiles_x, uint32_t nparts, uint32_t nbatch_total, uint32_t batch_records,
-              uint32_t nslots, uint32_t astride, uint32_t aheight, uint32_t rows_cap, uint32_t big_thr, uint32_t gang, uint32_t nbins)
+              uint32_t nslots, uint32_t astride, uint32_t aheight, uint32_t rows_cap, uint32_t big_thr, uint32_t gang, uint32_t nbins,
+              uint32_t *__restrict__ ticket)
 {
     extern __shared__ __attribute__((aligned(16))) unsigned char smem[];
     constexpr uint32_t TW = 1u << TWL, CELLS = TW * FL_TILE_H;
@@ -145,7 +182,10 @@
     const float inv_ps = __int_as_float(__builtin_amdgcn_readfirstlane(__float_as_int(1.0f / (float)per_slot)));
     const uint32_t chunk_slots = (rows_cap - 1u) * spr;
 
-    if (b_lo >= b_hi) return;
+    if (b_lo >= b_hi) {
+        if (ticket) drain_tile_if_last<TWL>(reinterpret_cast<uint32_t *>(tile), atom, out4, ticket, bin, nparts, tx, ty, astride, aheight);
+        return;
+    }
     for (uint32_t cb = b_lo; cb < b_hi;) {
     const uint32_t cs_lo = cb / per_slot;
     const uint32_t ce = min(b_hi, (cs_lo + chunk_slots) * per_slot);
@@ -314,6 +354,7 @@
             }
         }
     }
+    if (ticket) drain_tile_if_last<TWL>(reinterpret_cast<uint32_t *>(tile), atom, out4, ticket, bin, nparts, tx, ty, astride, aheight);
 }
 
 typedef uint32_t u32x2_t __attribute__((ext_vector_type(2)));
@@ -327,7 +368,8 @@
 k_accum_tiles_p3(const uint32_t *__restrict__ log, const uint32_t *__restrict__ dir,
                  const u64 *__restrict__ palette, u64 *__restrict__ atom, float *__restrict__ out4,
                  uint32_t tiles_x, uint32_t nparts, uint32_t nbatch_total, uint32_t batch_words,
-                 uint32_t nslots, uint32_t astride, uint32_t aheight, uint32_t rows_cap, uint32_t big_thr, uint32_t gang, uint32_t nbins)
+                 uint32_t nslots, uint32_t astride, uint32_t aheight, uint32_t rows_cap, uint32_t big_thr, uint32_t gang, uint32_t nbins,
+                 uint32_t *__restrict__ ticket)
 {
     extern __shared__ __attribute__((aligned(16))) unsigned char smem[];
     constexpr uint32_t TWL = 7u, TW = 1u << TWL, CELLS = TW * FL_TILE_H;
@@ -350,7 +392,10 @@
     const float inv_spr = __int_as_float(__builtin_amdgcn_readfirstlane(__float_as_int(1.0f / (float)spr)));
     const float inv_ps = __int_as_float(__builtin_amdgcn_readfirstlane(__float_as_int(1.0f / (float)per_slot)));
     const uint32_t chunk_slots = (rows_cap - 1u) * spr;
-    if (b_lo >= b_hi) return;
+    if (b_lo >= b_hi) {
+        if (ticket) drain_tile_if_last<TWL>(reinterpret_cast<uint32_t *>(smem + P3_TILE), atom, out4, ticket, bin, nparts, tx, ty, astride, aheight);
+        return;
+    }
     const uint32_t mk8 = P3_MARKS + wv * 64u;
     const uint32_t lane8 = (lane + 1u) << 3;
     u32x2_t wA = {}, wB = {}, wC = {};
@@ -481,12 +526,13 @@
     }
     __syncthreads();
     add_tile_to_cells<TWL>(reinterpret_cast<const u64 *>(smem + P3_TILE), atom, out4, tx, ty, astride, aheight, big_thr);
+    if (ticket) drain_tile_if_last<TWL>(reinterpret_cast<uint32_t *>(smem + P3_TILE), atom, out4, ticket, bin, nparts, tx, ty, astride, aheight);
 }
 
 void launch_accum_tiles(hipStream_t st, const uint32_t *log, const uint32_t *dir, const u64 *palette,
                         u64 *atom, float *out4, uint32_t tiles_x, uint32_t nbins, uint32_t nparts,
                         uint32_t nbatch_total, uint32_t batch_records, uint32_t nslots,
-                        uint32_t astride, uint32_t aheight, bool wide)
+                        uint32_t astride, uint32_t aheight, bool wide, uint32_t *ticket)
 {
     const uint32_t big_thr = 1024u / nparts;
     const uint32_t spr = nslots / FL_PAL_H, slots_per_part = (nslots + nparts - 1) / nparts;
@@ -502,7 +548,7 @@
         ensure_max_dynamic_lds((const void *)k_accum_tiles<FL_TILE_W_WIDE_LOG2>, attr);
         hipLaunchKernelGGL((k_accum_tiles<FL_TILE_W_WIDE_LOG2>), dim3(grid), dim3(1024),
                            (FL_TILE_H << FL_TILE_W_WIDE_LOG2) * 8 + 1024 * 4 + rows * FL_PAL_W * 8, st,
-                           log, dir, palette, atom, out4, tiles_x, nparts, nbatch_total, batch_records, nslots, astride, aheight, rows, big_thr, gang, nbins);
+                           log, dir, palette, atom, out4, tiles_x, nparts, nbatch_total, batch_records, nslots, astride, aheight, rows, big_thr, gang, nbins, ticket);
         return;
     }
     const uint32_t rows = want < 2u ? 2u : want > (uint32_t)ACC_ROWS_MAX ? (uint32_t)ACC_ROWS_MAX : want;
@@ -512,11 +558,11 @@
         static unsigned long long attr3 = 0;
         ensure_max_dynamic_lds((const void *)k_accum_tiles_p3, attr3);
         hipLaunchKernelGGL(k_accum_tiles_p3, dim3(grid), dim3(ACC_THREADS), P3_LDS, st,
-                           log, dir, palette, atom, out4, tiles_x, nparts, nbatch_total, fl_pack3_words(batch_records), nslots, astride, aheight, rows, big_thr, gang, nbins);
+                           log, dir, palette, atom, out4, tiles_x, nparts, nbatch_total, fl_pack3_words(batch_records), nslots, astride, aheight, rows, big_thr, gang, nbins, ticket);
         return;
     }
 #endif
     ensure_max_dynamic_lds((const void *)k_accum_tiles<7u>, attr);
     hipLaunchKernelGGL((k_accum_tiles<7u>), dim3(grid), dim3(ACC_THREADS), FL_TILE_CELLS * 8 + ACC_THREADS * 4 + rows * FL_PAL_W * 8, st,
-                       log, dir, palette, atom, out4, tiles_x, nparts, nbatch_total, batch_records, nslots, astride, aheight, rows, big_thr, gang, nbins);
-}
+                       log, dir, palette, atom, out4, tiles_x, nparts, nbatch_total, batch_records, nslots, astride, aheight, rows, big_thr, gang, nbins, ticket);
+}
diff --git a/cuburn_amd/csrc/flame_abi.hip b/cuburn_amd/csrc/flame_abi.hip
--- a/cuburn_amd/csrc/flame_abi.hip
+++ b/cuburn_amd/csrc/flame_abi.hip
@@ -87,6 +87,7 @@
     DevBuf<unsigned char> d_enc_out;
     size_t nbins() const { return d_front.cap; }
     DevBuf<uint32_t> d_log[2], d_dir[2];
+    DevBuf<uint32_t> d_ticket;
     hipStream_t aux = nullptr;
     hipEvent_t ev_it[2] = {nullptr, nullptr}, ev_ac[2] = {nullptr, nullptr};
     DevBuf<float> d_params;
@@ -116,6 +117,7 @@
         release_fb();
         d_params.release(); d_palette.release(); d_enc.release(); d_enc_out.release();
         for (int k = 0; k < 2; ++k) { d_log[k].release(); d_dir[k].release(); }
+        d_ticket.release();
         if (aux) hipStreamDestroy(aux);
         for (hipEvent_t *ev : events()) if (*ev) hipEventDestroy(*ev);
     }
@@ -582,11 +584,11 @@
     return FL_OK;
 }
 
-static int do_clear(fl_ctx *c, Lane &ln, const fl_dim &d, bool reset_points)
+static int do_clear(fl_ctx *c, Lane &ln, const fl_dim &d, bool reset_points, bool own = true, bool shared = true)
 {
     size_t nbins = (size_t)d.ah * d.astride;
-    launch_clear_frame(ln.stream, ln.d_front, ln.d_atom, ln.d_hot, c->d_counters, c->d_points, (uint32_t)nbins,
-                       reset_points ? c->npoints() : 0u);
+    launch_clear_frame(ln.stream, ln.d_front, ln.d_atom, ln.d_hot, shared ? c->d_counters.p : nullptr, c->d_points,
+                       own ? (uint32_t)nbins : 0u, shared && reset_points ? c->npoints() : 0u);
     HIPCHK(hipGetLastError());
     return FL_OK;
 }
@@ -600,6 +602,14 @@
     const auto quiesce = [&ln] { return ln.quiesce(true); };
     if (int rc = ln.d_log[buf].reserve(s.log_words, "sample log", quiesce)) return rc;
     return ln.d_dir[buf].reserve(s.dir_words, "sample log directory", quiesce);
+}
+
+static int ensure_tickets(Lane &ln, uint32_t ntiles)
+{
+    if (ln.d_ticket.cap >= ntiles) return FL_OK;
+    if (int rc = ln.d_ticket.reserve(ntiles, "accumulate tickets", [&ln] { return ln.quiesce(true); })) return rc;
+    HIPCHK(hipMemsetAsync(ln.d_ticket, 0, ln.d_ticket.bytes(), ln.stream));
+    return FL_OK;
 }
 
 static hipFunction_t rtc_variant(fl_ctx *c, fl_genome *g, bool count, int kacc, int mode, bool *pending)
@@ -627,7 +637,7 @@
 }
 
 static int do_iter_launch(fl_ctx *c, Lane &ln, fl_genome *g, const fl_dim &d, uint32_t nrounds, uint32_t fuse, bool count, int acc = 0,
-                          int buf = 0, hipStream_t drain = nullptr)
+                          int buf = 0, hipStream_t drain = nullptr, bool drain_cells = false)
 {
     if (!drain) drain = ln.stream;
     BinLayout bl = {};
@@ -635,7 +645,7 @@
     if (acc == FL_ACCUM_BINNED) {
         if (nrounds <= fuse) return fail(FL_E_INVAL, "binned launch needs write-enabled rounds", __FILE__, __LINE__);
         int rc = ensure_binned(c, ln, d, nrounds - fuse, buf, &bl, &nbatch_total);
-        if (rc) return rc;
+        if (rc || (drain_cells && (rc = ensure_tickets(ln, bl.nbins)))) return rc;
     }
     EvPair *e = ev_acquire(c, c->iter_ev);
     const int kacc = acc == FL_ACCUM_BINNED && bl.wide ? 3 : acc;
@@ -658,19 +668,18 @@
         EvPair *e2 = ev_begin_on(c, c->accum_ev, drain);
         launch_accum_tiles(drain, ln.d_log[buf], ln.d_dir[buf], ln.d_palette, ln.d_atom, (float *)ln.d_front.p, bl.tiles_x, bl.nbins,
                            accum_parts(bl.nbins, bl.wide, c->bin_parts), nbatch_total, c->bin_rounds * (uint32_t)c->nw * 64, c->nslots,
-                           d.astride, d.ah, bl.wide);
+                           d.astride, d.ah, bl.wide, drain_cells ? ln.d_ticket.p : nullptr);
         ev_end_on(e2, drain);
         HIPCHK(hipGetLastError());
     }
     return FL_OK;
 }
 
-static int do_flush(fl_ctx *c, Lane &ln, const fl_dim &d, bool use_hot = true, hipStream_t st = nullptr)
-{
-    if (!st) st = ln.stream;
-    EvPair *e = ev_begin_on(c, c->flush_ev, st);
-    launch_flush(st, ln.d_atom, ln.d_front, ln.d_hot, d.ah * d.astride, use_hot);
-    ev_end_on(e, st);
+static int do_flush(fl_ctx *c, Lane &ln, const fl_dim &d)
+{
+    EvPair *e = ev_begin_on(c, c->flush_ev, ln.stream);
+    launch_flush(ln.stream, ln.d_atom, ln.d_front, ln.d_hot, d.ah * d.astride, true);
+    ev_end_on(e, ln.stream);
     HIPCHK(hipGetLastError());
     return FL_OK;
 }
@@ -712,8 +721,10 @@
     int rc = ensure_fb(ln, w, h, &d);
     if (rc) return rc;
     if ((rc = flush_pending(c, ln))) return rc;
+    const bool split_clear = c->nlanes > 1;
+    if (split_clear && (rc = do_clear(c, ln, d, false, true, false))) return rc;
     if ((rc = wait_other(c, 1))) return rc;
-    if ((rc = do_clear(c, ln, d, true))) return rc;
+    if ((rc = do_clear(c, ln, d, true, !split_clear, true))) return rc;
     const double per_round = (double)c->npoints();
     uint64_t rounds = (uint64_t)ceil(nsamples / per_round);
     if (rounds == 0) rounds = 1;
@@ -737,8 +748,8 @@
         const uint32_t f = k == 0 ? fuse : 0;
         const int buf = pipelined ? (int)(k & 1u) : 0;
         if (pipelined && k >= 2) HIPCHK(hipStreamWaitEvent(ln.stream, ln.ev_ac[buf], 0));
-        if ((rc = do_iter_launch(c, ln, g, d, n + f, f, false, accum_mode, buf, drain))) return rc;
-        if ((rc = do_flush(c, ln, d, !binned, drain))) return rc;
+        if ((rc = do_iter_launch(c, ln, g, d, n + f, f, false, accum_mode, buf, drain, true))) return rc;
+        if (!binned && (rc = do_flush(c, ln, d))) return rc;
         if (pipelined) HIPCHK(hipEventRecord(ln.ev_ac[buf], drain));
         ++k;
     }
@@ -1436,6 +1447,7 @@
     case FL_BUF_HOT: is(ln.d_hot); break;
     case FL_BUF_LOG: is(ln.d_log[0]); break;
     case FL_BUF_DIR: is(ln.d_dir[0]); break;
+    case FL_BUF_TICKET: is(ln.d_ticket); break;
     default: return fail(FL_E_INVAL, "unknown buffer", __FILE__, __LINE__);
     }
     if (!*p) return fail(FL_E_INVAL, "buffer not allocated yet", __FILE__, __LINE__);
@@ -1553,8 +1565,8 @@
     return why ? fail(FL_E_INVAL, why, __FILE__, __LINE__) : (int)FL_OK;
 }
 
-int fl_debug_accum(fl_ctx *c, uint32_t w, uint32_t h, const uint32_t *log, size_t log_words, const uint32_t *dir, size_t dir_words,
-                   uint32_t nbatch_total, uint32_t batch_records, uint32_t nslots, uint32_t nparts, int wide)
+static int debug_accum(fl_ctx *c, uint32_t w, uint32_t h, const uint32_t *log, size_t log_words, const uint32_t *dir, size_t dir_words,
+                       uint32_t nbatch_total, uint32_t batch_records, uint32_t nslots, uint32_t nparts, int wide, bool drain_cells)
 {
     REQUIRE(c, "null ctx");
     fl_dim d;
@@ -1569,13 +1581,26 @@
     const auto quiesce = [&ln] { return ln.quiesce(true); };
     if ((rc = ln.d_log[0].reserve(log_words, "sample log", quiesce))) return rc;
     if ((rc = ln.d_dir[0].reserve(dir_words, "sample log directory", quiesce))) return rc;
+    if (drain_cells && (rc = ensure_tickets(ln, bl.nbins))) return rc;
     if ((rc = quiesce())) return rc;
     HIPCHK(hipMemcpy(ln.d_log[0], log, 4 * log_words, hipMemcpyHostToDevice));
     HIPCHK(hipMemcpy(ln.d_dir[0], dir, 4 * dir_words, hipMemcpyHostToDevice));
     launch_accum_tiles(ln.stream, ln.d_log[0], ln.d_dir[0], ln.d_palette, ln.d_atom, (float *)ln.d_front.p, bl.tiles_x, bl.nbins,
-                       nparts, nbatch_total, batch_records, nslots, d.astride, d.ah, bl.wide);
+                       nparts, nbatch_total, batch_records, nslots, d.astride, d.ah, bl.wide, drain_cells ? ln.d_ticket.p : nullptr);
     HIPCHK(hipGetLastError());
     return FL_OK;
+}
+
+int fl_debug_accum(fl_ctx *c, uint32_t w, uint32_t h, const uint32_t *log, size_t log_words, const uint32_t *dir, size_t dir_words,
+                   uint32_t nbatch_total, uint32_t batch_records, uint32_t nslots, uint32_t nparts, int wide)
+{
+    return debug_accum(c, w, h, log, log_words, dir, dir_words, nbatch_total, batch_records, nslots, nparts, wide, false);
+}
+
+int fl_debug_accum_drain(fl_ctx *c, uint32_t w, uint32_t h, const uint32_t *log, size_t log_words, const uint32_t *dir, size_t dir_words,
+                         uint32_t nbatch_total, uint32_t batch_records, uint32_t nslots, uint32_t nparts, int wide)
+{
+    return debug_accum(c, w, h, log, log_words, dir, dir_words, nbatch_total, batch_records, nslots, nparts, wide, true);
 }
 
 int fl_debug_clear_hot(fl_ctx *c, uint32_t w, uint32_t h)
diff --git a/cuburn_amd/csrc/iter.hip b/cuburn_amd/csrc/iter.hip
--- a/cuburn_amd/csrc/iter.hip
+++ b/cuburn_amd/csrc/iter.hip
@@ -878,13 +878,13 @@
         const float nanf_ = __uint_as_float(0x7fc00000u);
         points[i] = make_float4(nanf_, nanf_, nanf_, nanf_);
     }
-    if (i < 4u) counters[i] = 0ull;
+    if (counters && i < 4u) counters[i] = 0ull;
 }
 
 void launch_clear_frame(hipStream_t st, float4 *front, u64 *atom, uint32_t *hot, u64 *counters, float4 *points,
                         uint32_t nbins, uint32_t npoints)
 {
-    const uint32_t n = nbins > npoints ? nbins : npoints;
+    const uint32_t n = nbins > npoints ? nbins : npoints > 4u ? npoints : 4u;
     hipLaunchKernelGGL(k_clear_frame, dim3((n + 255) / 256), dim3(256), 0, st, front, atom, hot, counters, points, nbins, npoints);
 }
 
diff --git a/cuburn_amd/csrc/kernels.h b/cuburn_amd/csrc/kernels.h
--- a/cuburn_amd/csrc/kernels.h
+++ b/cuburn_amd/csrc/kernels.h
@@ -56,7 +56,7 @@
 void launch_accum_tiles(hipStream_t st, const uint32_t *log, const uint32_t *dir, const u64 *palette,
                         u64 *atom, float *out4, uint32_t tiles_x, uint32_t nbins, uint32_t nparts,
                         uint32_t nbatch_total, uint32_t batch_records, uint32_t nslots,
-                        uint32_t astride, uint32_t aheight, bool wide);
+                        uint32_t astride, uint32_t aheight, bool wide, uint32_t *ticket);
 
 void launch_interp_palette(hipStream_t st, fl_mwc *rng_pal, const float *ptimes, const float4 *pals,
                            float ts, float tstep, u64 *out);
diff --git a/include/flame_hip.h b/include/flame_hip.h
--- a/include/flame_hip.h
+++ b/include/flame_hip.h
@@ -206,7 +206,8 @@
     FL_BUF_HOT = 7,
     FL_BUF_SIDE = 8,
     FL_BUF_LOG = 9,
-    FL_BUF_DIR = 10
+    FL_BUF_DIR = 10,
+    FL_BUF_TICKET = 11
 };
 int fl_read_buffer(fl_ctx *ctx, fl_genome *g, int which, void *host_dst, size_t nbytes);
 int fl_write_buffer(fl_ctx *ctx, fl_genome *g, int which, const void *host_src, size_t nbytes);
@@ -224,6 +225,8 @@
 int fl_debug_accum(fl_ctx *ctx, uint32_t w, uint32_t h, const uint32_t *log, size_t log_words, const uint32_t *dir, size_t dir_words,
                    uint32_t nbatch_total, uint32_t batch_records, uint32_t nslots, uint32_t nparts, int wide);
 int fl_debug_accum_check(uint32_t w, uint32_t h, const uint32_t *log, size_t log_words, const uint32_t *dir, size_t dir_words,
+                         uint32_t nbatch_total, uint32_t batch_records, uint32_t nslots, uint32_t nparts, int wide);
+int fl_debug_accum_drain(fl_ctx *ctx, uint32_t w, uint32_t h, const uint32_t *log, size_t log_words, const uint32_t *dir, size_t dir_words,
                          uint32_t nbatch_total, uint32_t batch_records, uint32_t nslots, uint32_t nparts, int wide);
 int fl_debug_shuffle(fl_ctx *ctx, uint32_t round, uint32_t *out256);
 int fl_debug_apply_xf(fl_ctx *ctx, fl_genome *g, uint32_t ts, int xfi, uint32_t n, float *xyzw, fl_mwc *rng);
```

After: 126,600 Msamples/s. -42.5%, worse.
